# CoderLSF/fast-llama

Measured on AMD Instinct MI355X. Metric: decode tokens/s LLaMA2-7B int8, higher is better.
Workload: dtype int8; 1 GPU; LLaMA2-7B int8 .flm-layout synthetic weights (portable splitmix64 checkpoint, norm weights 1.0), single-stream greedy decode, prompt 9 tokens, positions 14..928, fp32 KV cache, max_seq 1024; parallelism=single-gpu

## Files before the change

### fast-llama_amd/csrc/flm_attn.h

```cpp
#pragma once
#include "flm_math.h"
#include "flm_gemv.h"
#pragma clang fp contract(off)

namespace flm {

struct AttnArgs {
    const float* q;
    const float* kcache;
    const float* vcache;
    float* out;
    const int* pos_ptr;
    const int* halt;
    int hs, max_seq;
    int kv_rows;
    unsigned long long* trace;
    void* oq; float* os; int oqt;
    int G; float* sc_global; unsigned* flag_sc; unsigned epoch; int* err;
    float* out_peer[7]; int n_peer;
    unsigned long long* gout; unsigned long long* gout_peer[7];
    const unsigned long long* qg; const unsigned long long* kg; const unsigned long long* vg;
};

#ifndef FLM_V_LATE_NS
// ... 718 lines not shown
        const int k = tid & 7, p = (tid >> 3) & 63, jh = (tid >> 9) * 4;
        for (int s = 0; s < nt; ++s) {
            float* cur = (s & 1) ? tile1 : tile0;
            park(cur, ring);
            __syncthreads();
            request(rK, s + 1, ring);
            const float* kp = cur + p * rs + k;
            const float* q0 = qs + (jh + 0) * hs + k; const float* q1 = qs + (jh + 1) * hs + k;
            const float* q2 = qs + (jh + 2) * hs + k; const float* q3 = qs + (jh + 3) * hs + k;
            float l0 = 0.f, l1 = 0.f, l2 = 0.f, l3 = 0.f;
#pragma unroll 8
            for (int i = 0; i < hs; i += 8) {
                const float kv = kp[i];
                l0 = __fmaf_rn(kv, q0[i], l0); l1 = __fmaf_rn(kv, q1[i], l1); l2 = __fmaf_rn(kv, q2[i], l2); l3 = __fmaf_rn(kv, q3[i], l3);
            }
            const int t = s * kAttnTile + p;
            auto fold = [&](float l, int j) {
                const int li = __float_as_int(l);
                float tot = __fadd_rn(0.f, l);
                tot = __fadd_rn(tot, __int_as_float(__builtin_amdgcn_update_dpp(0, li, 0x101 , 0xF, 0xF, true)));
                tot = __fadd_rn(tot, __int_as_float(__builtin_amdgcn_update_dpp(0, li, 0x102, 0xF, 0xF, true)));
                tot = __fadd_rn(tot, __int_as_float(__builtin_amdgcn_update_dpp(0, li, 0x103, 0xF, 0xF, true)));
                tot = __fadd_rn(tot, __int_as_float(__builtin_amdgcn_update_dpp(0, li, 0x104, 0xF, 0xF, true)));
                tot = __fadd_rn(tot, __int_as_float(__builtin_amdgcn_update_dpp(0, li, 0x105, 0xF, 0xF, true)));
                tot = __fadd_rn(tot, __int_as_float(__builtin_amdgcn_update_dpp(0, li, 0x106, 0xF, 0xF, true)));
                tot = __fadd_rn(tot, __int_as_float(__builtin_amdgcn_update_dpp(0, li, 0x107, 0xF, 0xF, true)));
                if (k == 0 && j < nq && t < pos0 + i0 + j + 1) sc[j * scs + t] = __fmul_rn(tot, scale);
            };
            fold(l0, jh + 0); fold(l1, jh + 1); fold(l2, jh + 2); fold(l3, jh + 3);
        }
    }
    }
    request(rV, 0, ring);
    __syncthreads();
    if (wave < nq) {
        const int T = pos0 + i0 + wave + 1;
        float* row = sc + wave * scs;
        float m = -INFINITY;
        for (int t = lane; t < T; t += 64) m = fmaxf(m, row[t]);
        m = wave_max(m);
        for (int t = lane; t < T; t += 64) row[t] = expf_ref(__fsub_rn(row[t], m));
        float sum = 0.f;
        if (lane == 0) {
            int t = 0;
            if (T >= 16) {
                const float4* r4 = reinterpret_cast<const float4*>(row);
                float4 a0 = r4[0], a1 = r4[1], a2 = r4[2], a3 = r4[3];
#define FLM_ADD4(q) sum = __fadd_rn(sum, q.x); sum = __fadd_rn(sum, q.y); sum = __fadd_rn(sum, q.z); sum = __fadd_rn(sum, q.w);
                for (; t + 32 <= T; t += 16) {
                    const float4 b0 = r4[t / 4 + 4], b1 = r4[t / 4 + 5], b2 = r4[t / 4 + 6], b3 = r4[t / 4 + 7];
                    FLM_ADD4(a0) FLM_ADD4(a1) FLM_ADD4(a2) FLM_ADD4(a3)
                    a0 = b0; a1 = b1; a2 = b2; a3 = b3;
                }
                FLM_ADD4(a0) FLM_ADD4(a1) FLM_ADD4(a2) FLM_ADD4(a3)
#undef FLM_ADD4
                t += 16;
            }
            for (; t < T; ++t) sum = __fadd_rn(sum, row[t]);
        }
        sum = __uint_as_float(__builtin_amdgcn_readfirstlane(__float_as_uint(sum)));
        for (int t = lane; t < T; t += 64) { const float w = __fdiv_rn(row[t], sum); row[t] = (t > 0 && fabsf(w) <= 1e-15f) ? 0.f : w; }
    }
    const int tpq = hs <= 64 ? 64 : 128;
    const int j = tid / tpq, d = tid - j * tpq;
    const bool mine = j < nq && d < hs;
    const int Tj = pos0 + i0 + j + 1;
    float o = 0.f;
    for (int i = 0; i < nt; ++i) {
        float* cur = (i & 1) ? tile1 : tile0;
        park(cur, ring);
        __syncthreads();
        request(rV, i + 1, ring);
        if (mine) {
            const float* vp = cur + d;
            const float* wp = sc + j * scs + i * kAttnTile;
            int np = Tj - i * kAttnTile; np = np < 0 ? 0 : (np > kAttnTile ? kAttnTile : np);
            int p = 0;
            if (i == 0 && np > 0) { o = __fmul_rn(vp[0], wp[0]); p = 1; }
            const float wl = lane < np ? wp[lane] : 1.f;
            if (__all(wl != 0.f)) {
                for (; p < np && (p & 7); ++p) o = __fmaf_rn(vp[p * rs], wp[p], o);
                for (; p + 8 <= np; p += 8) {
                    const float* vq = vp + p * rs;
                    const float4 wa = *reinterpret_cast<const float4*>(wp + p), wb = *reinterpret_cast<const float4*>(wp + p + 4);
                    const float a0 = vq[0], a1 = vq[rs], a2 = vq[2 * rs], a3 = vq[3 * rs], a4 = vq[4 * rs], a5 = vq[5 * rs], a6 = vq[6 * rs], a7 = vq[7 * rs];
                    o = __fmaf_rn(a0, wa.x, o); o = __fmaf_rn(a1, wa.y, o); o = __fmaf_rn(a2, wa.z, o); o = __fmaf_rn(a3, wa.w, o);
                    o = __fmaf_rn(a4, wb.x, o); o = __fmaf_rn(a5, wb.y, o); o = __fmaf_rn(a6, wb.z, o); o = __fmaf_rn(a7, wb.w, o);
                }
                for (; p < np; ++p) o = __fmaf_rn(vp[p * rs], wp[p], o);
            } else {
                for (; p < np; ++p) { const float w = wp[p]; o = w == 0.f ? o : __fmaf_rn(vp[p * rs], w, o); }
            }
        }
    }
    if (mine) a.out[(size_t)(i0 + j) * row_stride + (size_t)h * hs + d] = o;
}
template <bool PRE>
__global__ void __launch_bounds__(kAttnBlock) k_attn_prefill_mq(const AttnArgs a, int pos0, int row_stride, int B) {
    extern __shared__ __attribute__((aligned(16))) char lds[];
    const int i0 = blockIdx.y * kMqQueries, nq = B - i0 < kMqQueries ? B - i0 : kMqQueries;
    if (a.hs <= 64) attn_prefill_mq<1, PRE>(a, blockIdx.x, lds, pos0, i0, nq, row_stride, B); else attn_prefill_mq<2, PRE>(a, blockIdx.x, lds, pos0, i0, nq, row_stride, B);
}

constexpr int kQkQ = 16;
template <int NS>
__global__ void __launch_bounds__(256) k_qk_mfma(const AttnArgs a, int pos0, int row_stride, int B) {
    typedef float v4f __attribute__((ext_vector_type(4)));
    const int hs = a.hs, tid = threadIdx.x, lane = tid & 63, wave = tid >> 6;
    const int h = blockIdx.x, q0 = blockIdx.y * kQkQ;
    const int Tmax = pos0 + (q0 + kQkQ < B ? q0 + kQkQ : B);
    const int nt = (Tmax + 15) >> 4;
    const float* K = a.kcache + (size_t)h * (a.kv_rows ? a.kv_rows : a.max_seq) * hs;
    const __amdgpu_buffer_rsrc_t rK = __builtin_amdgcn_make_buffer_rsrc(const_cast<float*>(K), 0, Tmax * hs * 4, 0x00020000);
    const float scale = (float)(1.0 / (double)__builtin_sqrtf((float)hs));
    const int li = lane & 15, c = lane >> 4;
    v4f qa[NS][2];
    {
        const float* qp = a.q + (size_t)(q0 + li) * row_stride + (size_t)h * hs;
#pragma unroll
        for (int sp = 0; sp < NS; ++sp) {
            const int e = 8 * (4 * sp + c);
            if (q0 + li < B) { qa[sp][0] = *reinterpret_cast<const v4f*>(qp + e); qa[sp][1] = *reinterpret_cast<const v4f*>(qp + e + 4); }
            else { qa[sp][0] = v4f{0.f, 0.f, 0.f, 0.f}; qa[sp][1] = v4f{0.f, 0.f, 0.f, 0.f}; }
        }
    }
    v4f kb[2][NS][2];
    auto request = [&](int tile, v4f (&r)[NS][2]) {
        const unsigned base = (unsigned)(((tile * 16 + li) * hs + 8 * c) * 4);
#pragma unroll
        for (int sp = 0; sp < NS; ++sp) {
            r[sp][0] = __builtin_bit_cast(v4f, __builtin_amdgcn_raw_buffer_load_b128(rK, (int)(base + sp * 128), 0, 0));
            r[sp][1] = __builtin_bit_cast(v4f, __builtin_amdgcn_raw_buffer_load_b128(rK, (int)(base + sp * 128 + 16), 0, 0));
        }
    };
    auto tile_scores = [&](int tile, const v4f (&kr)[NS][2]) {
        v4f acc[8];
#pragma unroll
        for (int r = 0; r < 8; ++r) acc[r] = v4f{0.f, 0.f, 0.f, 0.f};
#pragma unroll
        for (int sp = 0; sp < NS; ++sp) {
#pragma unroll
            for (int r = 0; r < 8; ++r)
                acc[r] = __builtin_amdgcn_mfma_f32_16x16x4f32(qa[sp][r >> 2][r & 3], kr[sp][r >> 2][r & 3], acc[r], 0, 0, 0);
        }
        const int t = tile * 16 + li;
#pragma unroll
        for (int reg = 0; reg < 4; ++reg) {
            const int q = q0 + 4 * c + reg;
            float tot = __fadd_rn(0.f, acc[0][reg]);
#pragma unroll
            for (int r = 1; r < 8; ++r) tot = __fadd_rn(tot, acc[r][reg]);
            if (q < B && t < pos0 + q + 1) a.sc_global[((size_t)h * B + q) * a.max_seq + t] = __fmul_rn(tot, scale);
        }
    };
    request(wave, kb[0]);
    for (int tile = wave; tile < nt; tile += 8) {
        request(tile + 4, kb[1]);
        tile_scores(tile, kb[0]);
        request(tile + 8, kb[0]);
        if (tile + 4 < nt) tile_scores(tile + 4, kb[1]);
    }
}
constexpr int kPvQ = 16, kPvRing = 4;
__host__ __device__ inline int pv_row_stride(int tmax) { return ((((tmax + 15) & ~15) + 63) & ~63) + 4; }
__host__ inline size_t pv_mfma_lds_bytes(int tmax, int qw = kPvQ) { return ((size_t)qw * pv_row_stride(tmax) + 16) * 4; }
__host__ inline int pv_mfma_queries(int tmax, size_t lds_max) { int qw = kPvQ; while (qw > 1 && pv_mfma_lds_bytes(tmax, qw) > lds_max) qw >>= 1; return qw; }
inline __global__ void __launch_bounds__(256) k_attn_pv_mfma(const AttnArgs a, int pos0, int row_stride, int B, int qw) {
    typedef float v4f __attribute__((ext_vector_type(4)));
    typedef float v2f __attribute__((ext_vector_type(2)));
    extern __shared__ __attribute__((aligned(16))) char lds[];
    const int hs = a.hs, tid = threadIdx.x, lane = tid & 63, wave = tid >> 6;
    const int h = blockIdx.x, q0 = blockIdx.y * qw, nq = B - q0 < qw ? B - q0 : qw;
    const int S = pv_row_stride(pos0 + B);
    float* E = reinterpret_cast<float*>(lds);
    float* sums = E + qw * S;
    const int Tmax = pos0 + q0 + nq, Tp = (Tmax + 15) & ~15, nblk = Tp >> 4;
    {
        const int q = 4 * wave + (lane >> 4), l16 = lane & 15;
        const int Tq = q < nq ? pos0 + q0 + q + 1 : 0;
        const float* src = a.sc_global + ((size_t)h * B + (q0 + (q < nq ? q : 0))) * a.max_seq;
        float* row = E + q * S;
        const int Tr = q < qw ? Tp : 0;
        float m = -INFINITY;
        for (int t = l16 * 4; t < Tr; t += 64) {
            float4 v = make_float4(-INFINITY, -INFINITY, -INFINITY, -INFINITY);
            if (t + 3 < Tq) v = *reinterpret_cast<const float4*>(src + t);
            else { if (t < Tq) v.x = src[t]; if (t + 1 < Tq) v.y = src[t + 1]; if (t + 2 < Tq) v.z = src[t + 2]; }
            *reinterpret_cast<float4*>(row + t) = v;
            m = fmaxf(m, fmaxf(fmaxf(v.x, v.y), fmaxf(v.z, v.w)));
        }
        m = row16_max(m);
        for (int t = l16 * 4; t < Tr; t += 64) {
            float4 v = *reinterpret_cast<const float4*>(row + t);
            v.x = t < Tq ? expf_ref(__fsub_rn(v.x, m)) : 0.f; v.y = t + 1 < Tq ? expf_ref(__fsub_rn(v.y, m)) : 0.f;
            v.z = t + 2 < Tq ? expf_ref(__fsub_rn(v.z, m)) : 0.f; v.w = t + 3 < Tq ? expf_ref(__fsub_rn(v.w, m)) : 0.f;
            *reinterpret_cast<float4*>(row + t) = v;
        }
    }
    __syncthreads();
    if (tid < qw) {
        const float4* r4 = reinterpret_cast<const float4*>(E + tid * S);
        float sum = 0.f;
#pragma unroll 4
        for (int i = 0; i < Tp / 4; ++i) { const float4 v = r4[i]; sum = __fadd_rn(sum, v.x); sum = __fadd_rn(sum, v.y); sum = __fadd_rn(sum, v.z); sum = __fadd_rn(sum, v.w); }
        sums[tid] = sum;
    }
    __syncthreads();
    for (int bidx = tid; bidx < qw * nblk; bidx += 256) {
        const int q = bidx / nblk, bi = bidx - q * nblk;
        float* blk = E + q * S + bi * 16;
        const float sum = sums[q];
        float w[16];
#pragma unroll
        for (int i = 0; i < 4; ++i) { const float4 v = *reinterpret_cast<const float4*>(blk + 4 * i); w[4 * i] = v.x; w[4 * i + 1] = v.y; w[4 * i + 2] = v.z; w[4 * i + 3] = v.w; }
#pragma unroll
        for (int i = 0; i < 16; ++i) {
            const float x = q < nq ? __fdiv_rn(w[i], sum) : 0.f;
            w[i] = (bi * 16 + i > 0 && fabsf(x) <= 1e-15f) ? 0.f : x;
        }
#pragma unroll
        for (int c = 0; c < 4; ++c) *reinterpret_cast<float4*>(blk + 4 * c) = make_float4(w[c], w[4 + c], w[8 + c], w[12 + c]);
    }
    __syncthreads();
    const int li = lane & 15, c = lane >> 4, d0 = 32 * wave + 2 * li;
    if (32 * wave >= hs) return;
    const float* V = a.vcache + (size_t)h * (a.kv_rows ? a.kv_rows : a.max_seq) * hs;
    const __amdgpu_buffer_rsrc_t rV = __builtin_amdgcn_make_buffer_rsrc(const_cast<float*>(V), 0, Tmax * hs * 4, 0x00020000);
    unsigned voff = d0 < hs ? (unsigned)((c * hs + d0) * 4) : 0x80000000u;
    const unsigned vstep = (unsigned)(4 * hs * 4);
    v2f ring[kPvRing][4];
    auto request = [&](v2f (&r)[4]) {
#pragma unroll
        for (int sp = 0; sp < 4; ++sp) { r[sp] = __builtin_bit_cast(v2f, __builtin_amdgcn_raw_buffer_load_b64(rV, (int)voff, 0, 0)); voff += vstep; }
    };
#pragma unroll
    for (int r = 0; r < kPvRing; ++r) request(ring[r]);
    v4f acc0 = {-0.f, -0.f, -0.f, -0.f}, acc1 = {-0.f, -0.f, -0.f, -0.f};
    const float* ap = E + (li < qw ? li : 0) * S + 4 * c;
    for (int b0 = 0; b0 < nblk; b0 += kPvRing) {
#pragma unroll
        for (int r = 0; r < kPvRing; ++r) {
            if (b0 + r < nblk) {
                float4 av = *reinterpret_cast<const float4*>(ap + (b0 + r) * 16);
                if (li >= qw) av = make_float4(0.f, 0.f, 0.f, 0.f);
                acc0 = __builtin_amdgcn_mfma_f32_16x16x4f32(av.x, ring[r][0].x, acc0, 0, 0, 0); acc1 = __builtin_amdgcn_mfma_f32_16x16x4f32(av.x, ring[r][0].y, acc1, 0, 0, 0);
                acc0 = __builtin_amdgcn_mfma_f32_16x16x4f32(av.y, ring[r][1].x, acc0, 0, 0, 0); acc1 = __builtin_amdgcn_mfma_f32_16x16x4f32(av.y, ring[r][1].y, acc1, 0, 0, 0);
                acc0 = __builtin_amdgcn_mfma_f32_16x16x4f32(av.z, ring[r][2].x, acc0, 0, 0, 0); acc1 = __builtin_amdgcn_mfma_f32_16x16x4f32(av.z, ring[r][2].y, acc1, 0, 0, 0);
                acc0 = __builtin_amdgcn_mfma_f32_16x16x4f32(av.w, ring[r][3].x, acc0, 0, 0, 0); acc1 = __builtin_amdgcn_mfma_f32_16x16x4f32(av.w, ring[r][3].y, acc1, 0, 0, 0);
            }
            request(ring[r]);
        }
    }
    if (d0 < hs) {
#pragma unroll
        for (int reg = 0; reg < 4; ++reg) {
            const int q = 4 * c + reg;
            if (q < nq) {
                const size_t idx = (size_t)(q0 + q) * row_stride + (size_t)h * hs + d0;
                if (a.n_peer == 0) *reinterpret_cast<float2*>(a.out + idx) = make_float2(acc0[reg], acc1[reg]);
                else {
                    st_agent(a.out + idx, acc0[reg]); st_agent(a.out + idx + 1, acc1[reg]);
                    for (int i = 0; i < a.n_peer; ++i) {
                        __hip_atomic_store(a.out_peer[i] + idx, acc0[reg], __ATOMIC_RELAXED, __HIP_MEMORY_SCOPE_SYSTEM);
                        __hip_atomic_store(a.out_peer[i] + idx + 1, acc1[reg], __ATOMIC_RELAXED, __HIP_MEMORY_SCOPE_SYSTEM);
                    }
                }
            }
        }
    }
}

template <bool SPLIT>
__global__ void __launch_bounds__(kAttnBlock) k_attn_decode(const AttnArgs a) {
    extern __shared__ __attribute__((aligned(16))) char lds[];
    if (halted(a.halt)) return;
    const int G = SPLIT ? a.G : 1;
    attn_head_any<false, SPLIT>(a, blockIdx.x / G, lds, *a.pos_ptr + 1, a.q, a.out, blockIdx.x % G, G);
}

struct AoTp { unsigned* peer_flags[8]; const unsigned* base; unsigned add; int world, line0, n_lines; };
template <int QT, int XR, bool PREQ, bool SPLIT = false>
__global__ void __launch_bounds__(kGemvBlock, 4) k_attn_o(const AttnArgs aa, const GemvArgs a, const int n_heads, unsigned* flag, const unsigned target_, int* err, const AoTp tp) {
    extern __shared__ __attribute__((aligned(16))) char lds[];
    if (halted(a.halt)) return;
    auto stamp = [&](int k) { if (kAblate && a.trace && threadIdx.x == 0) a.trace[blockIdx.x * 8 + k] = __builtin_amdgcn_s_memtime(); };
    stamp(0);
    const unsigned target = tp.world ? *tp.base + tp.add : target_;
    if ((int)blockIdx.x < n_heads) {
        const int G = SPLIT ? aa.G : 1;
        attn_head_any<false, SPLIT>(aa, blockIdx.x / G, lds, *aa.pos_ptr + 1, aa.q, aa.out, blockIdx.x % G, G);
        stamp(1);
        wait_stores_done();
        __syncthreads();
        if (threadIdx.x == 0) {
            if (tp.world) {
                __atomic_thread_fence(__ATOMIC_RELEASE);
                for (int r = 0; r < tp.world; ++r) __hip_atomic_store(tp.peer_flags[r] + (tp.line0 + blockIdx.x) * kFlagStride, target, __ATOMIC_RELAXED, __HIP_MEMORY_SCOPE_SYSTEM);
            } else __hip_atomic_store(flag + blockIdx.x * kFlagStride, target, __ATOMIC_RELAXED, __HIP_MEMORY_SCOPE_AGENT);
        }
        stamp(4);
        return;
    }
    GemvCtx<QT, EPI_RESIDUAL> g;
    g.init(a, blockIdx.x - n_heads, gridDim.x - n_heads, lds);
    g.issue(kAblate ? a.ablate : 0);
    stamp(1);
    const int n_poll = tp.world ? tp.n_lines : n_heads;
    if ((int)(threadIdx.x & ~63u) < n_poll) {
        const bool mine = (int)threadIdx.x < n_poll;
        if (tp.world) {
            poll_wave<__HIP_MEMORY_SCOPE_SYSTEM, true, 4>(flag + threadIdx.x * kFlagStride, mine, target, err);
            __atomic_thread_fence(__ATOMIC_ACQUIRE);
        } else poll_wave(flag + threadIdx.x * kFlagStride, mine, target, err);
    }
    __syncthreads();
    stamp(2);
    float4 xv[XR > 0 ? XR : 1], nv[XR > 0 ? XR : 1];
    if constexpr (PREQ) {
        gemv_prologue<QT, PRO_NONE, 0, true>(a, lds, xv, nv, [](int) {});
    } else {
        gemv_preload<QT, PRO_QUANT, XR, true>(a, xv, nv);
        gemv_prologue<QT, PRO_QUANT, XR>(a, lds, xv, nv, [](int) {});
    }
    stamp(3);
    g.run(a, lds, [](int) {});
    stamp(4);
}

template <int QT, int XR, bool PREQ, bool SPLIT = false, bool TP = false>
__global__ void __launch_bounds__(kGemvBlock, 4) k_qkv_attn_o(const GemvArgs aq, const AttnArgs aa, const GemvArgs a, const int gridq, const int n_heads, const int grido,
                                                              unsigned* flagq, unsigned* flag, const unsigned target, int* err, const AoTp tp) {
    extern __shared__ __attribute__((aligned(16))) char lds[];
    if constexpr (!TP) { if (halted(a.halt)) return; }
    auto nostamp = [](int) {};
    const unsigned htarget = TP ? *tp.base + tp.add : target;
    if constexpr (TP) { if (aq.xf.world) xchg_fold(aq.xf); }
    if ((int)blockIdx.x < gridq) {
        float4 xq[1], nq[1];
        gemv_preload<QT, PRO_RMSNORM_QUANT, 1, TP>(aq, xq, nq);
        GemvCtx<QT, EPI_ROPE_KV> gq;
        gq.init(aq, blockIdx.x, gridq, lds);
        gemv_prologue<QT, PRO_RMSNORM_QUANT, 1, TP>(aq, lds, xq, nq, [&](int part) { gq.issue(kAblate ? aq.ablate : 0, part); });
        gq.run(aq, lds, nostamp);
        wait_stores_done();
        __syncthreads();
        if (threadIdx.x == 0) __hip_atomic_store(flagq + blockIdx.x * kFlagStride, target, __ATOMIC_RELAXED, __HIP_MEMORY_SCOPE_AGENT);
    }
    if ((int)blockIdx.x < n_heads) {
        const int G = SPLIT ? aa.G : 1, h = blockIdx.x / G;
        if (threadIdx.x < 256) {
            const bool need = qkv_line_needed(threadIdx.x, (unsigned)gridq, (unsigned)aq.rows_per_pass, (unsigned)aa.hs, (unsigned)h, (unsigned)aq.dim, (unsigned)aq.kv_dim);
            poll_wave(flagq + threadIdx.x * kFlagStride, need, target, err);
        }
        __syncthreads();
        attn_head_any<true, SPLIT>(aa, h, lds, *aa.pos_ptr + 1, aa.q, aa.out, blockIdx.x % G, G);
        wait_stores_done();
        __syncthreads();
        if (threadIdx.x == 0) {
            if constexpr (TP) {
                __atomic_thread_fence(__ATOMIC_RELEASE);
                for (int r = 0; r < tp.world; ++r) __hip_atomic_store(tp.peer_flags[r] + (tp.line0 + blockIdx.x) * kFlagStride, htarget, __ATOMIC_RELAXED, __HIP_MEMORY_SCOPE_SYSTEM);
            } else __hip_atomic_store(flag + blockIdx.x * kFlagStride, target, __ATOMIC_RELAXED, __HIP_MEMORY_SCOPE_AGENT);
        }
        return;
    }
    if ((int)blockIdx.x >= n_heads + grido) return;
    GemvCtx<QT, EPI_RESIDUAL> g;
    g.init(a, blockIdx.x - n_heads, grido, lds);
    g.issue(kAblate ? a.ablate : 0);
    const int n_poll = TP ? tp.n_lines : n_heads;
    if ((int)(threadIdx.x & ~63u) < n_poll) {
        const bool mine = (int)threadIdx.x < n_poll;
        if constexpr (TP) {
            poll_wave<__HIP_MEMORY_SCOPE_SYSTEM, true, 4>(flag + threadIdx.x * kFlagStride, mine, htarget, err);
            __atomic_thread_fence(__ATOMIC_ACQUIRE);
        } else poll_wave(flag + threadIdx.x * kFlagStride, mine, htarget, err);
    }
    __syncthreads();
    float4 xv[XR > 0 ? XR : 1], nv[XR > 0 ? XR : 1];
    if constexpr (PREQ) {
        gemv_prologue<QT, PRO_NONE, 0, true>(a, lds, xv, nv, [](int) {});
    } else {
        gemv_preload<QT, PRO_QUANT, XR, true>(a, xv, nv);
        gemv_prologue<QT, PRO_QUANT, XR>(a, lds, xv, nv, [](int) {});
    }
    g.run(a, lds, [](int) {});
}

struct FfnTp { unsigned* peer_flags[8]; const unsigned* base; unsigned add; int world, rank; unsigned long long* counter; };
template <int QT, int XR2, bool TP = false>
__global__ void __launch_bounds__(kGemvBlock, 4) k_ffn(const GemvArgs a13, const GemvArgs a2, const int grid13, const int grid2, unsigned* flag, const unsigned target_, int* err, const FfnTp tp) {
    extern __shared__ __attribute__((aligned(16))) char lds[];
    if constexpr (!TP) { if (halted(a2.halt)) return; }
    auto nostamp = [](int) {};
    const unsigned target = TP ? *tp.base + tp.add : target_;
    if constexpr (TP) { if (a13.xf.world) xchg_fold(a13.xf); }
    if ((int)blockIdx.x < grid13) {
        float4 xv[1], nv[1];
        gemv_preload<QT, PRO_RMSNORM_QUANT, 1, TP>(a13, xv, nv);
        GemvCtx<QT, EPI_SWIGLU> g;
        g.init(a13, blockIdx.x, grid13, lds);
        gemv_prologue<QT, PRO_RMSNORM_QUANT, 1, TP>(a13, lds, xv, nv, [&](int part) { g.issue(kAblate ? a13.ablate : 0, part); });
        g.run(a13, lds, nostamp);
    }
    wait_stores_done();
    __syncthreads();
    if (threadIdx.x == 0) {
        if constexpr (TP) {
            const unsigned long long old = __hip_atomic_fetch_add(tp.counter, 1ull, __ATOMIC_ACQ_REL, __HIP_MEMORY_SCOPE_AGENT);
            if ((old + 1) % gridDim.x == 0) {
                __atomic_thread_fence(__ATOMIC_RELEASE);
                for (int r = 0; r < tp.world; ++r) __hip_atomic_store(tp.peer_flags[r] + tp.rank * kFlagStride, target, __ATOMIC_RELAXED, __HIP_MEMORY_SCOPE_SYSTEM);
            }
        } else __hip_atomic_store(flag + blockIdx.x * kFlagStride, target, __ATOMIC_RELAXED, __HIP_MEMORY_SCOPE_AGENT);
    }
    if ((int)blockIdx.x >= grid2) return;
    GemvCtx<QT, EPI_RESIDUAL> g2;
    g2.init(a2, blockIdx.x, grid2, lds);
    g2.issue(kAblate ? a2.ablate : 0, 1);
    if (threadIdx.x < 256) {
        const bool mine = (int)threadIdx.x < (TP ? tp.world : (int)gridDim.x);
        if constexpr (TP) {
            poll_wave<__HIP_MEMORY_SCOPE_SYSTEM, true, 4>(flag + threadIdx.x * kFlagStride, mine, target, err);
            __atomic_thread_fence(__ATOMIC_ACQUIRE);
        } else poll_wave(flag + threadIdx.x * kFlagStride, mine, target, err);
    }
    __syncthreads();
    float4 xv2[XR2 > 0 ? XR2 : 1], nv2[XR2 > 0 ? XR2 : 1];
    gemv_preload<QT, PRO_QUANT, XR2, true>(a2, xv2, nv2);
    gemv_prologue<QT, PRO_QUANT, XR2, true>(a2, lds, xv2, nv2, [&](int) { g2.issue(kAblate ? a2.ablate : 0, 2); });
    g2.run(a2, lds, nostamp);
}

}
```

### fast-llama_amd/csrc/flm_gemv.h

```cpp
#pragma once
#include "flm_math.h"
#include "flm_wait.h"
#pragma clang fp contract(off)

namespace flm {

struct GemvArgs {
    const void*  W;   const float* sW;
    int n;
    int items;
    int rows_per_pass;
    int cb_shift;
    int ctr_off;
    int nbuf;
    const float* x;
    const float* norm_w;
    const void*  xq; const float* xs;
    float* out;
    float* kcache; float* vcache;
    const float* rope_cos; const float* rope_sin;
    const int* pos_ptr;
    const int* halt;
    int dim; int kv_dim; int max_seq; int hs;
    float* out_peer[7]; int n_peer;
    unsigned long long* gout; unsigned long long* gout_peer[7];
    unsigned long long* gk; unsigned long long* gv;
    struct XchgFold {
        unsigned* local_flags; unsigned* peer_flags[8];
        const unsigned* base; unsigned add;
        int rank, world, slot; int* err;
    } xf;
    void* dbg_xq; float* dbg_xs; float* dbg_xn;
    unsigned long long* trace;
    int ablate;
};

__device__ __forceinline__ void st_result(const GemvArgs& a, unsigned row, float v) {
    st_agent(a.out + row, v);
    for (int i = 0; i < a.n_peer; ++i) __hip_atomic_store(a.out_peer[i] + row, v, __ATOMIC_RELAXED, __HIP_MEMORY_SCOPE_SYSTEM);
}

#ifndef FLM_ABLATE
#define FLM_ABLATE 0
#endif
constexpr bool kAblate = FLM_ABLATE != 0;
constexpr int kStepBlk = 4;

__host__ __device__ inline int chain_bshift(int n) { int s = 2; while ((64 << s) < n / 4) ++s; return s; }
__host__ __device__ inline int chain_strip_floats(int n) { return 64 * ((1 << chain_bshift(n)) + 4); }
struct GemvLds {
    int off_xs, off_red, off_ctr, off_scr;
    int gstride;
    int buf_bytes;
    int total;
};
__host__ __device__ inline GemvLds gemv_lds_layout(int n, int esz, bool norm, int Rm, int RB, bool two, int nbuf = 2) {
    GemvLds L;
    const int sn = n / kGroup, ng = two ? 2 * sn : sn;
    L.off_xs = n * esz;
    L.off_red = L.off_xs + ((sn * 4 + 15) & ~15);
    L.off_ctr = L.off_red + 64;
    L.off_scr = L.off_ctr + 16;
    int g16 = (ng * 8 + 15) / 16; if ((g16 & 1) == 0) ++g16;
    L.gstride = g16 * 16;
    L.buf_bytes = (Rm + RB) * L.gstride;
    int scratch = nbuf * L.buf_bytes + 64;
    const int chain = 4 * chain_strip_floats(n) * 4 + 64;
    if (norm && chain > scratch) scratch = chain;
    L.total = L.off_scr + scratch;
    return L;
}
__device__ __forceinline__ float sq_chain(const float* p, int n4) {
    float l = 0.f;
    int k = 0;
#define FLM_SQ4(v) l = __fmaf_rn(v.x, v.x, l); l = __fmaf_rn(v.y, v.y, l); l = __fmaf_rn(v.z, v.z, l); l = __fmaf_rn(v.w, v.w, l);
#define FLM_RD4(a, b, c, d, base) a = *reinterpret_cast<const float4*>(pp + (base)); b = *reinterpret_cast<const float4*>(pp + (base) + 4); c = *reinterpret_cast<const float4*>(pp + (base) + 8); d = *reinterpret_cast<const float4*>(pp + (base) + 12);
    if (n4 >= 32) {
        const float* pp = p;
        float4 a0, a1, a2, a3, b0, b1, b2, b3;
        FLM_RD4(a0, a1, a2, a3, 0)
#pragma unroll 2
        for (; k + 32 <= n4; k += 32, pp += 32) {
            FLM_RD4(b0, b1, b2, b3, 16)
            __builtin_amdgcn_s_waitcnt(0xC47F);
            __builtin_amdgcn_sched_barrier(0);
            FLM_SQ4(a0) FLM_SQ4(a1) FLM_SQ4(a2) FLM_SQ4(a3)
            __builtin_amdgcn_sched_barrier(0);
            FLM_RD4(a0, a1, a2, a3, 32)
            __builtin_amdgcn_s_waitcnt(0xC47F);
            __builtin_amdgcn_sched_barrier(0);
            FLM_SQ4(b0) FLM_SQ4(b1) FLM_SQ4(b2) FLM_SQ4(b3)
            __builtin_amdgcn_sched_barrier(0);
        }
        if (k + 4 <= n4) { FLM_SQ4(a0) k += 4; } if (k + 4 <= n4) { FLM_SQ4(a1) k += 4; } if (k + 4 <= n4) { FLM_SQ4(a2) k += 4; } if (k + 4 <= n4) { FLM_SQ4(a3) k += 4; }
    }
#undef FLM_RD4
#undef FLM_SQ4
    for (; k < n4; ++k) l = __fmaf_rn(p[k], p[k], l);
    return l;
}

__device__ __forceinline__ double wave_scan_incl_f64(double v) {
#define FLM_SCAN64(ctrl, rmask, bc) { const int lo_ = __builtin_amdgcn_update_dpp(0, __double2loint(v), ctrl, rmask, 0xF, bc), hi_ = __builtin_amdgcn_update_dpp(0, __double2hiint(v), ctrl, rmask, 0xF, bc); v = __dadd_rn(v, __hiloint2double(hi_, lo_)); }
    FLM_SCAN64(0x111 , 0xF, true) FLM_SCAN64(0x112 , 0xF, true)
    FLM_SCAN64(0x114 , 0xF, true) FLM_SCAN64(0x118 , 0xF, true)
    FLM_SCAN64(0x142 , 0xA, false) FLM_SCAN64(0x143 , 0xC, false)
#undef FLM_SCAN64
    return v;
}
__device__ __forceinline__ float wave_scan_incl(float v) {
#define FLM_SCAN_STEP(ctrl, rmask, bc) v = __fadd_rn(v, __int_as_float(__builtin_amdgcn_update_dpp(0, __float_as_int(v), ctrl, rmask, 0xF, bc)));
    FLM_SCAN_STEP(0x111 , 0xF, true) FLM_SCAN_STEP(0x112 , 0xF, true)
    FLM_SCAN_STEP(0x114 , 0xF, true) FLM_SCAN_STEP(0x118 , 0xF, true)
    FLM_SCAN_STEP(0x142 , 0xA, false) FLM_SCAN_STEP(0x143 , 0xC, false)
#undef FLM_SCAN_STEP
    return v;
}
__device__ __forceinline__ double readlane_f64(double v, int l) {
    return __hiloint2double(__builtin_amdgcn_readlane(__double2hiint(v), l), __builtin_amdgcn_readlane(__double2loint(v), l));
}
constexpr int kChainHead = 4;
#ifdef FLM_TRACE_PRO_RT
#define FLM_CHAIN_STAMP(k) if (tr && lane == 0) tr[k] = __builtin_amdgcn_s_memtime();
#else
#define FLM_CHAIN_STAMP(k)
#endif
template <int OP> __device__ __forceinline__ float chain_step(float l, float x) { if constexpr (OP == 0) return __fmaf_rn(x, x, l); else return __fadd_rn(l, x); }
template <int BVR, int OP = 0, int PAD = 4, bool STARTS = false>
__device__ __forceinline__ float chain_spec_t(const float* p, const int bshift, int* rounds_out, unsigned long long* tr = nullptr, const int Brt = 0, float* lane_start = nullptr) {
    const int lane = threadIdx.x & 63, B = BVR ? 4 * BVR : (Brt ? Brt : (1 << bshift)), BV = B >> 2, LS = B + PAD;
    const float4* pl = reinterpret_cast<const float4*>(p + lane * LS);
    float4 xr[BVR ? BVR : 1];
    if constexpr (BVR > 0) {
#pragma unroll
        for (int q = 0; q < BVR; ++q) xr[q] = pl[q];
    }
    auto elem = [&](int q) -> float4 { if constexpr (BVR > 0) return xr[q]; else return pl[q]; };
    FLM_CHAIN_STAMP(0)
#define FLM_SQ4(l, v) l = chain_step<OP>(l, v.x); l = chain_step<OP>(l, v.y); l = chain_step<OP>(l, v.z); l = chain_step<OP>(l, v.w);
    float s = 0.f; unsigned orb = 0u;
#pragma unroll
    for (int q = 0; q < BV; ++q) { const float4 v = elem(q); FLM_SQ4(s, v) orb |= __float_as_uint(v.x) | __float_as_uint(v.y); orb |= __float_as_uint(v.z) | __float_as_uint(v.w); }
    const bool allzero = (orb & 0x7fffffffu) == 0u;
    const float P = __int_as_float(__builtin_amdgcn_update_dpp(0, __float_as_int(wave_scan_incl(s)), 0x138 , 0xF, 0xF, true));
    FLM_CHAIN_STAMP(1)
    float hv;
    [[maybe_unused]] float ls = 0.f;
    {
        float l = 0.f;
#pragma unroll
        for (int L = 0; L < kChainHead; ++L) {
            if constexpr (STARTS) { if (lane == L) ls = l; }
#pragma unroll
            for (int q = 0; q < BV; ++q) { const float4 v = elem(q); FLM_SQ4(l, v) }
            if (L + 1 < kChainHead) l = __int_as_float(__builtin_amdgcn_update_dpp(0, __float_as_int(l), 0x138 , 0xF, 0xF, true));
        }
        hv = __int_as_float(__builtin_amdgcn_readlane(__float_as_int(l), kChainHead - 1));
    }
    FLM_CHAIN_STAMP(2)
    const unsigned eb = __float_as_uint(P) & 0x7f800000u;
    bool valid = lane >= kChainHead && eb >= (27u << 23) && eb <= (250u << 23);
    const unsigned ebv = valid ? eb : 0x3f800000u;
    const float A = __uint_as_float(ebv), u1 = __uint_as_float(ebv - (23u << 23)), top = __fadd_rn(A, A);
    float ca = A, cb = __fadd_rn(A, u1);
#pragma unroll
    for (int q = 0; q < BV; ++q) { const float4 v = elem(q); FLM_SQ4(ca, v) FLM_SQ4(cb, v) }
    float T = __fsub_rn(ca, A);
    const bool tie = __fsub_rn(cb, ca) != u1;
    if (!(T < INFINITY)) valid = false;
    if (!valid) T = 0.f;
    FLM_CHAIN_STAMP(3)
    const unsigned long long live = __ballot(valid && !allzero);
    bool plain = false;
    if (live) {
        const unsigned e0 = (unsigned)__builtin_amdgcn_readlane((int)eb, __ffsll((long long)live) - 1), e1 = (unsigned)__builtin_amdgcn_readlane((int)eb, 63 - __clzll((long long)live));
        plain = e1 < e0 || ((e1 - e0) >> 23) > 26;
    }
    if (plain) {
        float l = 0.f;
        for (int L = 0; L < 64; ++L) { if constexpr (STARTS) { if (lane == L) ls = l; } const float4* r = reinterpret_cast<const float4*>(p + L * LS); for (int q = 0; q < BV; ++q) { const float4 v = r[q]; FLM_SQ4(l, v) } }
        if (rounds_out) *rounds_out = -1;
        if constexpr (STARTS) *lane_start = ls;
        return l;
    }
    const double Td = (double)T, Si = wave_scan_incl_f64(Td), S = __dsub_rn(Si, Td);
    FLM_CHAIN_STAMP(4)
    int rounds = 0;
    const unsigned long long zero_m = __ballot(allzero), good_m = __ballot(valid && !tie);
    unsigned long long done_m = (1ull << kChainHead) - 1ull;
    double bv = (double)hv, Sb = readlane_f64(S, kChainHead);
    float res;
    [[maybe_unused]] int base = kChainHead;
    for (;;) {
        ++rounds;
        if (rounds <= 9) { FLM_CHAIN_STAMP(4 + rounds) }
        const float st = (float)__dadd_rn(bv, __dsub_rn(S, Sb));
        const unsigned long long e_m = __ballot((__float_as_uint(st) & 0x7f800000u) == eb), t_m = __ballot(__fadd_rn(st, T) < top);
        const unsigned long long bad = ~(zero_m | (good_m & e_m & t_m) | done_m);
        if (bad == 0) {
            if constexpr (STARTS) { if (lane >= base) ls = st; }
            res = __uint_as_float((unsigned)__builtin_amdgcn_readlane((int)__float_as_uint((float)__dadd_rn(bv, __dsub_rn(Si, Sb))), 63)); break;
        }
        const int f = __ffsll((long long)bad) - 1;
        if constexpr (STARTS) { if (lane >= base && lane <= f) ls = st; base = f + 1; }
        float l = st;
#pragma unroll
        for (int q = 0; q < BV; ++q) { const float4 v = elem(q); FLM_SQ4(l, v) }
        res = __uint_as_float((unsigned)__builtin_amdgcn_readlane((int)__float_as_uint(l), f));
        if (f == 63) break;
        done_m = (2ull << f) - 1ull; bv = (double)res; Sb = readlane_f64(S, f + 1);
    }
#undef FLM_SQ4
    FLM_CHAIN_STAMP(14)
    if (tr && lane == 0) tr[15] = (unsigned long long)rounds;
    if (rounds_out) *rounds_out = rounds;
    if constexpr (STARTS) *lane_start = ls;
    return res;
}
template <int BVR>
__device__ __forceinline__ float sq_chain_spec_t(const float* p, const int bshift, int* rounds_out, unsigned long long* tr = nullptr) { return chain_spec_t<BVR, 0, 4>(p, bshift, rounds_out, tr); }
__device__ __forceinline__ float sq_chain_spec(const float* p, const int bshift, int* rounds_out = nullptr, unsigned long long* tr = nullptr) {
    return sq_chain_spec_t<0>(p, bshift, rounds_out, tr);
}

template <int QT, int PRO, int XR, bool COH = false>
__device__ __forceinline__ void gemv_preload(const GemvArgs& a, float4 (&xv)[XR > 0 ? XR : 1], float4 (&wv)[XR > 0 ? XR : 1], const float* xsrc = nullptr) {
    if constexpr (PRO == PRO_QUANT || PRO == PRO_RMSNORM_QUANT) {
        typedef float v4f __attribute__((ext_vector_type(4)));
        const __amdgpu_buffer_rsrc_t rx = __builtin_amdgcn_make_buffer_rsrc(const_cast<float*>(xsrc ? xsrc : a.x), 0, a.n * 4, 0x00020000);
        const __amdgpu_buffer_rsrc_t rn = __builtin_amdgcn_make_buffer_rsrc(const_cast<float*>(PRO == PRO_RMSNORM_QUANT ? a.norm_w : a.x), 0, a.n * 4, 0x00020000);
#pragma unroll
        for (int i = 0; i < XR; ++i) {
            const int off = (threadIdx.x * 4 + i * kGemvBlock * 4) * 4;
            const v4f v = __builtin_bit_cast(v4f, __builtin_amdgcn_raw_buffer_load_b128(rx, off, 0, COH ? kAuxCoherent : 0));
            xv[i] = make_float4(v.x, v.y, v.z, v.w);
            if constexpr (PRO == PRO_RMSNORM_QUANT) {
                const v4f u = __builtin_bit_cast(v4f, __builtin_amdgcn_raw_buffer_load_b128(rn, off, 0, 0));
                wv[i] = make_float4(u.x, u.y, u.z, u.w);
            }
        }
    }
}

typedef unsigned v4u_g __attribute__((ext_vector_type(4)));
typedef unsigned long long granule_t;
__device__ __forceinline__ void st_granule(granule_t* g, unsigned tag, float v) {
    __hip_atomic_store(g, ((granule_t)tag << 32) | (granule_t)__float_as_uint(v), __ATOMIC_RELAXED, __HIP_MEMORY_SCOPE_AGENT);
}
__device__ __forceinline__ float ld_granule_value(const granule_t* g) { return __uint_as_float((unsigned)__hip_atomic_load(g, __ATOMIC_RELAXED, __HIP_MEMORY_SCOPE_AGENT)); }
__device__ __forceinline__ void st_result_granule(const GemvArgs& a, unsigned row, unsigned tag, float v) {
    st_granule(a.gout + row, tag, v);
    const granule_t g = ((granule_t)tag << 32) | (granule_t)__float_as_uint(v);
    for (int i = 0; i < a.n_peer; ++i) __hip_atomic_store(a.gout_peer[i] + row, g, __ATOMIC_RELAXED, __HIP_MEMORY_SCOPE_SYSTEM);
}

#ifndef FLM_QUANT_SHARED_RCP
#define FLM_QUANT_SHARED_RCP 1
#endif
template <int QT>
__device__ __forceinline__ void quant_round4(char* xq, float* xs, int e, bool act, const float4& v) {
    using T = QTraits<QT>;
    const float mx = row16_max(fmaxf(fmaxf(fabsf(v.x), fabsf(v.y)), fmaxf(fabsf(v.z), fabsf(v.w))));
    const float sc = __fdiv_rn(mx, T::kF);
    int qq[4];
#if FLM_QUANT_SHARED_RCP
    quant_elems4(v, sc, qq);
#else
    qq[0] = quant_elem(v.x, sc); qq[1] = quant_elem(v.y, sc); qq[2] = quant_elem(v.z, sc); qq[3] = quant_elem(v.w, sc);
#endif
    if (act) {
        const int q0 = qq[0], q1 = qq[1], q2 = qq[2], q3 = qq[3];
        if constexpr (QT == QT_INT8) {
            const uint32_t pk = (uint32_t)(q0 & 0xff) | ((uint32_t)(q1 & 0xff) << 8) | ((uint32_t)(q2 & 0xff) << 16) | ((uint32_t)(q3 & 0xff) << 24);
            *reinterpret_cast<uint32_t*>(xq + e) = pk;
        } else {
            uint2 pk;
            pk.x = (uint32_t)(q0 & 0xffff) | ((uint32_t)(q1 & 0xffff) << 16);
            pk.y = (uint32_t)(q2 & 0xffff) | ((uint32_t)(q3 & 0xffff) << 16);
            *reinterpret_cast<uint2*>(xq + (size_t)e * 2) = pk;
        }
        if ((threadIdx.x & 15) == 0) xs[e / kGroup] = sc;
    }
}

#ifdef FLM_TRACE_PRO_RT
#define FLM_PRO_STAMP(k) if (kAblate && a.trace && (threadIdx.x == 0 || threadIdx.x == 960)) a.trace[blockIdx.x * 16 + (threadIdx.x ? 8 : 0) + (k)] = __builtin_amdgcn_s_memrealtime();
#elif defined(FLM_TRACE_PRO)
#define FLM_PRO_STAMP(k) if (kAblate && a.trace && threadIdx.x == 0) a.trace[blockIdx.x * 8 + (k)] = __builtin_amdgcn_s_memtime();
#else
#define FLM_PRO_STAMP(k)
#endif
template <int QT, int PRO, int XR, bool COH = false, bool LATE = false, class AfterStage>
__device__ __forceinline__ void gemv_prologue(const GemvArgs& a, char* lds, float4 (&xv)[XR > 0 ? XR : 1], float4 (&wv)[XR > 0 ? XR : 1], AfterStage&& after_stage) {
    using T = QTraits<QT>;
    const int n = a.n;
    const int tid = threadIdx.x;
    const GemvLds L = gemv_lds_layout(n, T::kEsz, PRO == PRO_RMSNORM_QUANT, a.rows_per_pass, 64 >> a.cb_shift, false);
    char*  xq = lds;
    float* xs = reinterpret_cast<float*>(lds + L.off_xs);
    float* red = reinterpret_cast<float*>(lds + L.off_red);
    float* scratch = reinterpret_cast<float*>(lds + L.off_scr);

    if constexpr (PRO == PRO_NONE) {
        const int nb16 = n * T::kEsz / 16;
        if constexpr (COH) {
            const __amdgpu_buffer_rsrc_t rq = __builtin_amdgcn_make_buffer_rsrc(const_cast<void*>(a.xq), 0, n * T::kEsz, 0x00020000);
            for (int c = tid; c < nb16; c += kGemvBlock)
                reinterpret_cast<v4i*>(xq)[c] = __builtin_bit_cast(v4i, __builtin_amdgcn_raw_buffer_load_b128(rq, c * 16, 0, kAuxCoherent));
            for (int g = tid; g < n / kGroup; g += kGemvBlock) xs[g] = ld_agent(a.xs + g);
        } else {
            for (int c = tid; c < nb16; c += kGemvBlock)
                reinterpret_cast<int4*>(xq)[c] = reinterpret_cast<const int4*>(a.xq)[c];
            for (int g = tid; g < n / kGroup; g += kGemvBlock) xs[g] = a.xs[g];
        }
        __syncthreads();
        return;
    } else {
        const int rounds = (n + kGemvBlock * 4 - 1) / (kGemvBlock * 4);
        const float4 z4 = make_float4(0.f, 0.f, 0.f, 0.f);
        float r = 1.0f;
#ifdef FLM_TRACE_PRO_RT
        FLM_PRO_STAMP(0)
#endif
        auto ldx = [&](int e) -> float4 {
            if constexpr (COH) {
                typedef float v4f __attribute__((ext_vector_type(4)));
                const __amdgpu_buffer_rsrc_t rx = __builtin_amdgcn_make_buffer_rsrc(const_cast<float*>(a.x), 0, n * 4, 0x00020000);
                const v4f t = __builtin_bit_cast(v4f, __builtin_amdgcn_raw_buffer_load_b128(rx, e * 4, 0, kAuxCoherent));
                return make_float4(t.x, t.y, t.z, t.w);
            } else return *reinterpret_cast<const float4*>(a.x + e);
        };
        if constexpr (PRO == PRO_QUANT) {
            if constexpr (XR > 0) { asm volatile("" :: "v"(xv[XR - 1].w)); }
            FLM_PRO_STAMP(3)
            if constexpr (!LATE) after_stage(0);
            FLM_PRO_STAMP(4)
        }
        if constexpr (PRO == PRO_RMSNORM_QUANT) {
            const int bs = chain_bshift(n), B = 1 << bs, LS = B + 4, CS = 64 * LS, slots = 64 << bs;
            auto stage = [&](int i, const float4& v) {
                const int k = tid + i * kGemvBlock;
                if (k < slots) { const int o = (k >> bs) * LS + (k & (B - 1)); scratch[o] = v.x; scratch[CS + o] = v.y; scratch[2 * CS + o] = v.z; scratch[3 * CS + o] = v.w; }
            };
            const int srounds = (slots + kGemvBlock - 1) / kGemvBlock;
#pragma unroll
            for (int i = 0; i < XR; ++i) { if (i < srounds) stage(i, xv[i]); }
            for (int i = XR; i < srounds; ++i) {
                const int e = tid * 4 + i * kGemvBlock * 4;
                stage(i, e < n ? ldx(e) : z4);
            }
#ifdef FLM_TRACE_PRO_RT
            FLM_PRO_STAMP(1)
#endif
            __syncthreads();
            FLM_PRO_STAMP(3)
            if constexpr (!LATE) {
                if (tid >= 4 * kWave) __builtin_amdgcn_s_sleep(2);
                after_stage(0);
#ifdef FLM_TRACE_PRO2
                FLM_PRO_STAMP(1)
#endif
                if (tid < 4 * kWave && !(kAblate && (a.ablate & 2))) {
                    const float l = sq_chain_spec(scratch + (tid >> 6) * CS, bs);
                    if ((tid & 63) == 0) red[8 + (tid >> 6)] = l;
                }
            } else {
                const int wv = __builtin_amdgcn_readfirstlane(tid >> 6);
                if (wv >= 4) after_stage(0);
                else if (!(kAblate && (a.ablate & 2))) {
#ifdef FLM_TRACE_PRO_RT
                    unsigned long long* tr = (kAblate && a.trace && tid < 64) ? a.trace + 2 * 4096 + blockIdx.x * 16 : nullptr;
#else
                    unsigned long long* tr = nullptr;
#endif
                    const float* cp = scratch + wv * CS;
                    float l;
                    if (bs == 4) l = sq_chain_spec_t<4>(cp, bs, nullptr, tr);
                    else if (bs == 3) l = sq_chain_spec_t<2>(cp, bs, nullptr, tr);
                    else if (bs == 2) l = sq_chain_spec_t<1>(cp, bs, nullptr, tr);
                    else l = sq_chain_spec_t<0>(cp, bs, nullptr, tr);
                    if ((tid & 63) == 0) red[8 + wv] = l;
                }
            }
#ifdef FLM_TRACE_PRO_RT
            FLM_PRO_STAMP(2)
#endif
            FLM_PRO_STAMP(4)
            __syncthreads();
            const float ss = __fadd_rn(__fadd_rn(__fadd_rn(__fadd_rn(0.f, red[8]), red[9]), red[10]), red[11]);
            r = rms_scale(ss, n);
            FLM_PRO_STAMP(5)
        }
        auto round = [&](int i, float4 v, float4 w) {
            const int e = tid * 4 + i * kGemvBlock * 4;
            const bool act = e < n;
            if constexpr (PRO == PRO_RMSNORM_QUANT) {
                v.x = __fmul_rn(__fmul_rn(v.x, w.x), r); v.y = __fmul_rn(__fmul_rn(v.y, w.y), r);
                v.z = __fmul_rn(__fmul_rn(v.z, w.z), r); v.w = __fmul_rn(__fmul_rn(v.w, w.w), r);
            }
            if (act && a.dbg_xn && blockIdx.x == 0) *reinterpret_cast<float4*>(a.dbg_xn + e) = v;
            quant_round4<QT>(xq, xs, e, act, v);
        };
#pragma unroll
        for (int i = 0; i < XR; ++i) { if (i < rounds) round(i, xv[i], wv[i]); }
        for (int i = XR; i < rounds; ++i) {
            const int e = tid * 4 + i * kGemvBlock * 4;
            float4 v = z4, w = z4;
            if (e < n) {
                v = ldx(e);
                if constexpr (PRO == PRO_RMSNORM_QUANT) w = *reinterpret_cast<const float4*>(a.norm_w + e);
            }
            round(i, v, w);
        }
        if constexpr (PRO == PRO_QUANT) {
            FLM_PRO_STAMP(5)
        }
#ifdef FLM_TRACE_PRO_RT
        FLM_PRO_STAMP(6)
#endif
        __syncthreads();
#ifdef FLM_TRACE_PRO_RT
        FLM_PRO_STAMP(7)
#endif
        if (a.dbg_xq && blockIdx.x == 0) {
            const int nb4 = n * T::kEsz / 4;
            for (int c = tid; c < nb4; c += kGemvBlock) reinterpret_cast<uint32_t*>(a.dbg_xq)[c] = reinterpret_cast<uint32_t*>(xq)[c];
            for (int g = tid; g < n / kGroup; g += kGemvBlock) a.dbg_xs[g] = xs[g];
        }
    }
}

typedef unsigned int u32;
typedef unsigned v4u __attribute__((ext_vector_type(4)));

template <int QT, int EPI, bool STASH = false>
struct GemvCtx {
    using T = QTraits<QT>;
    static constexpr u32 LPGS = (T::kEPC == 16) ? 2 : 3;
    static constexpr u32 LPG = 1u << LPGS;
    static constexpr bool TWO = EPI == EPI_SWIGLU;
    static constexpr int H = kStepBlk;
    static constexpr u32 ES = TWO ? 16 : 8;
    static constexpr u32 kOOB = 0x80000000u;

    struct Set { v4i w[H]; float sw; u32 itl, st, xo, nlive; };

    u32 n, lane, wave, rowbytes, sn, cbs, RB, nbc, NBCV, TRm, Rm, RBP, SP, NS, np_wg, npass, gstride, buf_bytes, off_xs, off_scr, ctr_off;
    u32 inv_SP, inv_NBCV;
    u32 lane_woff, lane_xoff, lane_goff;
    u32 lane_j, lane_s2off, lane_sx2off, lane_poff;
    bool leader;
    u32 dW, dS, dT, dummy_st, wg, nwg, nbuf;
    u32 st_base, st_n;
    static constexpr u32 kSlotBytes = H * 1024 + 256;
    __amdgpu_buffer_rsrc_t rW, rS;
    Set setA, setB;
    bool stored;
    const float* resid_src;
    const granule_t* gsrc; bool gron; unsigned gtag;
    u32 nw;

    static __device__ __forceinline__ u32 inv_of(u32 d) { return d > 1 ? 0xFFFFFFFFu / d + 1u : 0u; }
    static __device__ __forceinline__ u32 udiv(u32 x, u32 d, u32 inv) { return d > 1 ? __umulhi(x, inv) : x; }

    __device__ __forceinline__ void init(const GemvArgs& a, u32 wg_, u32 nwg_, char* lds, u32 ctr_slot = 0, u32 st_base_ = 0, u32 st_n_ = 0, bool write_ctr = true) {
        n = a.n; wg = wg_; nwg = nwg_; st_base = st_base_; st_n = st_n_;
        lane = threadIdx.x & 63;
        wave = __builtin_amdgcn_readfirstlane(threadIdx.x >> 6);
        rowbytes = n * T::kEsz; sn = n / kGroup;
        const u32 nchunks = rowbytes / 16;
        cbs = a.cb_shift; RB = 64u >> cbs;
        const u32 CB = 1u << cbs;
        nbc = nchunks >> cbs;
        NBCV = TWO ? 2 * nbc : nbc;
        TRm = (u32)a.items * (EPI == EPI_ROPE_KV ? 2u : 1u);
        Rm = a.rows_per_pass;
        RBP = Rm / RB;
        npass = (TRm + Rm - 1) / Rm;
        np_wg = wg < npass ? (npass - wg + nwg - 1) / nwg : 0;
        SP = ((RBP + H - 1) / H) * NBCV;
        NS = np_wg * SP;
        inv_SP = inv_of(SP); inv_NBCV = inv_of(NBCV);
        nbuf = a.nbuf > 0 ? a.nbuf : 2;
        const GemvLds L = gemv_lds_layout(n, T::kEsz, true, Rm, RB, TWO, nbuf);
        gstride = L.gstride; buf_bytes = L.buf_bytes; off_xs = L.off_xs; off_scr = L.off_scr; ctr_off = a.ctr_off ? (u32)a.ctr_off : (u32)L.off_ctr + 4 * (ctr_slot & 1);
        dW = RB * rowbytes; dS = RB * sn * 4; dT = RB * gstride;
        dummy_st = Rm * gstride;
        const u32 rb = lane >> cbs, cb = lane & (CB - 1);
        lane_woff = rb * rowbytes + cb * 16;
        lane_xoff = cb * 16;
        lane_goff = rb * gstride + (cb >> LPGS) * ES;
        leader = (cb & (LPG - 1)) == 0;
        constexpr u32 GPB = 64u / LPG;
        lane_j = lane / GPB;
        const u32 ll = (lane % GPB) * LPG, rb2 = ll >> cbs, cb2 = ll & (CB - 1);
        lane_s2off = lane_j * dS + (rb2 * sn + (cb2 >> LPGS)) * 4;
        lane_sx2off = (cb2 >> LPGS) * 4;
        lane_poff = lane_j * dT + rb2 * gstride + (cb2 >> LPGS) * ES + ES / 2;
        constexpr int kRsrcFlags = 0x00020000;
        const u32 NM = TWO ? 2u : 1u;
        rW = __builtin_amdgcn_make_buffer_rsrc(const_cast<void*>(a.W), 0, (int)(NM * TRm * rowbytes), kRsrcFlags);
        rS = __builtin_amdgcn_make_buffer_rsrc(const_cast<float*>(a.sW), 0, (int)(NM * TRm * sn * 4), kRsrcFlags);
        stored = false; primedA = primedB = false; resid_src = nullptr; gsrc = nullptr; gron = false; gtag = 0; nw = kWavesPerBlock;
        if (write_ctr && threadIdx.x == 0) *reinterpret_cast<u32*>(lds + ctr_off) = 2 * kWavesPerBlock;
    }

    __device__ __forceinline__ void reset_ctr(char* lds) const { if (threadIdx.x == 0) *reinterpret_cast<u32*>(lds + ctr_off) = 2 * kWavesPerBlock; }

    __device__ __forceinline__ void decode(u32 s, Set& S, u32& wo, u32& so) const {
        if (s >= NS) { S.itl = np_wg; S.st = 0; S.xo = 0; S.nlive = 0; wo = kOOB; so = kOOB; return; }
        const u32 itl = udiv(s, SP, inv_SP), rem = s - itl * SP;
        const u32 q = udiv(rem, NBCV, inv_NBCV), cv = rem - q * NBCV;
        const bool second = TWO && cv >= nbc;
        const u32 cc = second ? cv - nbc : cv, g0 = (cc << cbs) >> LPGS;
        const u32 rb0 = q * H, row0 = (second ? TRm : 0u) + (wg + itl * nwg) * Rm + rb0 * RB;
        wo = row0 * rowbytes + ((cc << cbs) * 16);
        so = (row0 * sn + g0) * 4;
        S.itl = itl; S.xo = cc; S.nlive = RBP - rb0 < (u32)H ? RBP - rb0 : (u32)H;
        S.st = rb0 * RB * gstride + g0 * ES + (second ? 4u : 0u);
    }
    __device__ __forceinline__ void load_step(Set& S, u32 s, int ablate, const char* lds = nullptr) const {
        u32 wo, so;
        decode(s, S, wo, so);
        if constexpr (STASH) {
            const u32 si = s - 2 * kWavesPerBlock;
            if (si < st_n) {
                const char* p = lds + st_base + si * kSlotBytes;
#pragma unroll
                for (int j = 0; j < H; ++j) S.w[j] = *reinterpret_cast<const v4i*>(p + j * 1024 + lane * 16);
                S.sw = *reinterpret_cast<const float*>(p + H * 1024 + lane * 4);
                return;
            }
        }
        u32 nl = S.nlive;
        if (kAblate && (ablate & 4)) { nl = 0; so = kOOB; }
#pragma unroll
        for (int j = 0; j < H; ++j) {
            const u32 woj = (u32)j < nl ? wo + j * dW : kOOB;
            S.w[j] = __builtin_bit_cast(v4i, __builtin_amdgcn_raw_buffer_load_b128(rW, (int)(lane_woff + woj), 0, 2));
        }
        const u32 svo = lane_j < nl ? lane_s2off + so : kOOB;
        S.sw = __uint_as_float(__builtin_amdgcn_raw_buffer_load_b32(rS, (int)svo, 0, 2));
    }
    bool primedA, primedB;
    __device__ __forceinline__ void issue(int ablate, int part = 0) {
        if (part != 2) { load_step(setA, wave < nw ? wave : NS, ablate); primedA = true; }
        if (part != 1) { load_step(setB, wave < nw ? wave + nw : NS, ablate); primedB = true; }
    }

    __device__ __forceinline__ void stash_issue(const char* lds, const u32 w0 = 0) const {
        const u32 lds0 = (u32)(uintptr_t)(__attribute__((address_space(3))) const char*)lds;
        if (wave < w0) return;
        for (u32 i = wave - w0; i < st_n; i += kWavesPerBlock - w0) {
            Set S; u32 wo, so;
            decode(2 * kWavesPerBlock + i, S, wo, so);
            const u32 dst = __builtin_amdgcn_readfirstlane(lds0 + st_base + i * kSlotBytes);
#pragma unroll
            for (int j = 0; j < H; ++j) {
                const u32 woj = (u32)j < S.nlive ? lane_woff + wo + j * dW : kOOB;
                asm volatile("s_mov_b32 m0, %2\n\ts_nop 0\n\tbuffer_load_dwordx4 %0, %1, 0 offen nt lds" :: "v"(woj), "s"(rW), "s"(dst + j * 1024) : "memory", "m0");
            }
            const u32 svo = lane_j < S.nlive ? lane_s2off + so : kOOB;
            asm volatile("s_mov_b32 m0, %2\n\ts_nop 0\n\tbuffer_load_dword %0, %1, 0 offen nt lds" :: "v"(svo), "s"(rS), "s"(dst + H * 1024) : "memory", "m0");
        }
    }
    __device__ __forceinline__ void issue_missing(int ablate) {
        if (!primedA) { load_step(setA, wave < nw ? wave : NS, ablate); primedA = true; }
        if (!primedB) { load_step(setB, wave < nw ? wave + nw : NS, ablate); primedB = true; }
    }

    v4i xa; float sx2; u32 cur_xo;
    __device__ __forceinline__ void reduce_step(const Set& S, char* lds, char* strips, int ablate) {
        const char* xq = lds; const char* xs = lds + off_xs;
        if (S.xo != cur_xo) {
            cur_xo = S.xo;
            xa = *reinterpret_cast<const v4i*>(xq + ((cur_xo << cbs) * 16) + lane_xoff);
            sx2 = *reinterpret_cast<const float*>(xs + (((cur_xo << cbs) >> LPGS) * 4) + lane_sx2off);
        }
        float d[H];
#pragma unroll
        for (int j = 0; j < H; ++j) {
            int t = (kAblate && (ablate & 8)) ? 0 : quad_sum(dot_chunk<QT>(S.w[j], xa));
            if constexpr (LPG == 8) t += __builtin_amdgcn_update_dpp(0, t, 0x104 , 0xF, 0xF, true);
            d[j] = (float)t;
        }
        if (leader) {
#pragma unroll
            for (int j = 0; j < H; ++j) {
                const u32 stj = (u32)j < S.nlive ? S.st + j * dT : dummy_st;
                *reinterpret_cast<float*>(strips + stj + lane_goff) = d[j];
            }
        }
        if (lane_j < S.nlive) *reinterpret_cast<float*>(strips + S.st + lane_poff) = __fmul_rn(S.sw, sx2);
    }

    __device__ __forceinline__ void finish_pass(const GemvArgs& a, u32 pass, u32 it, const char* strips, int pos) {
        const bool chain_wave = wave == (it & (kWavesPerBlock - 1));
        float resid = 0.f, rc = 0.f, rs = 0.f;
        const u32 row = pass * Rm + lane;
        const bool rv = chain_wave && lane < Rm && row < TRm;
        if constexpr (EPI == EPI_RESIDUAL) { if (rv) resid = gsrc ? ld_granule_value(gsrc + row) : ld_agent((resid_src ? resid_src : a.out) + row); }
        if constexpr (EPI == EPI_ROPE_KV) {
            if (rv && row < (u32)(a.dim + a.kv_dim)) {
                const u32 r2 = (row < (u32)a.dim ? row : row - a.dim) & ~1u;
                const u32 dd = r2 % (u32)a.hs;
                rc = a.rope_cos[(size_t)pos * (a.hs / 2) + dd / 2];
                rs = a.rope_sin[(size_t)pos * (a.hs / 2) + dd / 2];
            }
        }
        __syncthreads();
        if (!chain_wave) return;
#ifdef FLM_TRACE_BAR
        if (kAblate && a.trace && threadIdx.x == 0 && it == 0) a.trace[blockIdx.x * 8 + 3] = __builtin_amdgcn_s_memtime();
#endif
        stored = true;
        float acc = 0.f, acc2 = 0.f;
        if (lane < Rm && !(kAblate && (a.ablate & 1))) {
            const char* sp = strips + lane * gstride;
            u32 g = 0;
#define FLM_RD4(r0, r1, r2, r3, ptr) r0 = *reinterpret_cast<const float4*>(ptr); r1 = *reinterpret_cast<const float4*>((ptr) + 16); r2 = *reinterpret_cast<const float4*>((ptr) + 32); r3 = *reinterpret_cast<const float4*>((ptr) + 48);
            if constexpr (TWO) {
                typedef float f2 __attribute__((ext_vector_type(2)));
                f2 ac = {0.f, 0.f};
#define FLM_CH(q) ac = __builtin_elementwise_fma(f2{q.z, q.w}, f2{q.x, q.y}, ac);
                if (sn >= 8) {
                    float4 a0, a1, a2, a3, b0, b1, b2, b3;
                    FLM_RD4(a0, a1, a2, a3, sp)
                    for (; g + 8 <= sn; g += 8) {
                        const char* pn = sp + (g + 4) * 16;
                        FLM_RD4(b0, b1, b2, b3, pn)
                        __builtin_amdgcn_s_waitcnt(0xC47F);
                        __builtin_amdgcn_sched_barrier(0);
                        FLM_CH(a0) FLM_CH(a1) FLM_CH(a2) FLM_CH(a3)
                        __builtin_amdgcn_sched_barrier(0);
                        FLM_RD4(a0, a1, a2, a3, pn + 64)
                        __builtin_amdgcn_s_waitcnt(0xC47F);
                        __builtin_amdgcn_sched_barrier(0);
                        FLM_CH(b0) FLM_CH(b1) FLM_CH(b2) FLM_CH(b3)
                        __builtin_amdgcn_sched_barrier(0);
                    }
                    if (g < sn) { FLM_CH(a0) ++g; } if (g < sn) { FLM_CH(a1) ++g; } if (g < sn) { FLM_CH(a2) ++g; } if (g < sn) { FLM_CH(a3) ++g; }
                }
                for (; g < sn; ++g) { const float4 e = *reinterpret_cast<const float4*>(sp + g * 16); FLM_CH(e) }
#undef FLM_CH
                acc = ac.x; acc2 = ac.y;
            } else {
#define FLM_CH(q) acc = __fmaf_rn(q.y, q.x, acc); acc = __fmaf_rn(q.w, q.z, acc);
                if (sn >= 16) {
                    float4 a0, a1, a2, a3, b0, b1, b2, b3;
                    FLM_RD4(a0, a1, a2, a3, sp)
                    for (; g + 16 <= sn; g += 16) {
                        const char* pn = sp + (g + 8) * 8;
                        FLM_RD4(b0, b1, b2, b3, pn)
                        __builtin_amdgcn_s_waitcnt(0xC47F);
                        __builtin_amdgcn_sched_barrier(0);
                        FLM_CH(a0) FLM_CH(a1) FLM_CH(a2) FLM_CH(a3)
                        __builtin_amdgcn_sched_barrier(0);
                        FLM_RD4(a0, a1, a2, a3, pn + 64)
                        __builtin_amdgcn_s_waitcnt(0xC47F);
                        __builtin_amdgcn_sched_barrier(0);
                        FLM_CH(b0) FLM_CH(b1) FLM_CH(b2) FLM_CH(b3)
                        __builtin_amdgcn_sched_barrier(0);
                    }
                    if (g + 2 <= sn) { FLM_CH(a0) g += 2; } if (g + 2 <= sn) { FLM_CH(a1) g += 2; } if (g + 2 <= sn) { FLM_CH(a2) g += 2; } if (g + 2 <= sn) { FLM_CH(a3) g += 2; }
                }
#undef FLM_CH
                for (; g < sn; ++g) { const float2 e = *reinterpret_cast<const float2*>(sp + g * 8); acc = __fmaf_rn(e.y, e.x, acc); }
            }
#undef FLM_RD4
        }
        if constexpr (EPI == EPI_STORE || EPI == EPI_RESIDUAL) {
            if (rv) {
                if constexpr (EPI == EPI_STORE) st_result(a, row, acc);
                else if (gron) st_result_granule(a, row, gtag, __fadd_rn(resid, acc));
                else st_result(a, row, __fadd_rn(resid, acc));
            }
        } else if constexpr (EPI == EPI_SWIGLU) {
            if (rv) { const float hv = swiglu_elem(acc, acc2); if (gron) st_result_granule(a, row, gtag, hv); else st_result(a, row, hv); }
        } else {
            const float other = __shfl_xor(acc, 1, kWave);
            if (rv && (lane & 1) == 0) {
                const float x0 = acc, x1 = other;
                const u32 hs = a.hs;
                if (row < (u32)(a.dim + a.kv_dim)) {
                    const u32 rr = row < (u32)a.dim ? row : row - a.dim;
                    const u32 h = rr / hs, d = rr - h * hs;
                    float o0, o1;
                    rope_pair(x0, x1, rc, rs, o0, o1);
                    if (row < (u32)a.dim) {
                        if (gron) { st_granule(a.gout + row, gtag, o0); st_granule(a.gout + row + 1, gtag, o1); }
                        else { st_agent(a.out + row, o0); st_agent(a.out + row + 1, o1); }
                    }
                    else {
                        float* kp = a.kcache + ((size_t)h * a.max_seq + pos) * hs + d; st_agent(kp, o0); st_agent(kp + 1, o1);
                        if (gron) { st_granule(a.gk + rr, gtag, o0); st_granule(a.gk + rr + 1, gtag, o1); }
                    }
                } else {
                    const u32 rr = row - a.dim - a.kv_dim;
                    const u32 h = rr / hs, d = rr - h * hs;
                    float* vp = a.vcache + ((size_t)h * a.max_seq + pos) * hs + d; st_agent(vp, x0); st_agent(vp + 1, x1);
                    if (gron) { st_granule(a.gv + rr, gtag, x0); st_granule(a.gv + rr + 1, gtag, x1); }
                }
            }
        }
    }

    template <class Stamp>
    __device__ __forceinline__ void run(const GemvArgs& a, char* lds, Stamp&& stamp) {
        int pos = 0;
        if constexpr (EPI == EPI_ROPE_KV) pos = *a.pos_ptr;
        xa = v4i{0, 0, 0, 0}; sx2 = 0.f; cur_xo = 0xffffffffu;
        u32* ctr = reinterpret_cast<u32*>(lds + ctr_off);
        u32 it = 0;
        bool tr3 = false;
        auto finish_upto = [&](u32 limit) {
            while (it < limit) {
                char* strips = lds + off_scr + (nbuf > 1 ? (it & 1) * buf_bytes : 0u);
#ifdef FLM_TRACE_WAVES
                if (kAblate && a.trace && it == 0 && lane == 0 && wave % 3 == 0) a.trace[blockIdx.x * 8 + 1 + wave / 3] = __builtin_amdgcn_s_memtime();
#elif !defined(FLM_TRACE_PRO)
                if (it == 0) stamp(4);
#endif
                finish_pass(a, wg + it * nwg, it, strips, pos);
#ifndef FLM_TRACE_PRO
                if (it == 0) stamp(5);
#endif
                ++it;
            }
        };
        auto do_set = [&](Set& S) -> bool {
            finish_upto(S.itl);
            if (S.itl >= np_wg) return false;
            reduce_step(S, lds, lds + off_scr + (nbuf > 1 ? (S.itl & 1) * buf_bytes : 0u), a.ablate);
            u32 s = 0;
            if (lane == 0) s = atomicAdd(ctr, 1u);
            load_step(S, __builtin_amdgcn_readfirstlane(s), a.ablate, lds);
#if !defined(FLM_TRACE_PRO) && !defined(FLM_TRACE_BAR)
            if (!tr3) { tr3 = true; stamp(3); }
#endif
            return true;
        };
        if (!primedA) load_step(setA, wave, a.ablate);
        if (!primedB) load_step(setB, wave + kWavesPerBlock, a.ablate);
        while (do_set(setA) && do_set(setB)) {}
    }

    struct AoSrc {
        const unsigned* flags;
        u32 rows, grid;
        unsigned target; int* err;
    };
    struct AoBlock { v4i d; float s; };
    template <int PRO>
    __device__ __forceinline__ AoBlock ao_fetch(const GemvArgs& a, u32 cc) const {
        AoBlock b; b.s = 0.f;
        const u32 CB = 1u << cbs;
        if constexpr (PRO == PRO_NONE) {
            const __amdgpu_buffer_rsrc_t rq = __builtin_amdgcn_make_buffer_rsrc(const_cast<void*>(a.xq), 0, (int)rowbytes, 0x00020000);
            const __amdgpu_buffer_rsrc_t rs = __builtin_amdgcn_make_buffer_rsrc(const_cast<float*>(a.xs), 0, (int)(sn * 4), 0x00020000);
            b.d = __builtin_bit_cast(v4i, __builtin_amdgcn_raw_buffer_load_b128(rq, (int)(lane < CB ? ((cc << cbs) + lane) * 16 : kOOB), 0, kAuxCoherent));
            b.s = __uint_as_float(__builtin_amdgcn_raw_buffer_load_b32(rs, (int)(lane < (CB >> LPGS) ? (((cc << cbs) >> LPGS) + lane) * 4 : kOOB), 0, kAuxCoherent));
        } else {
            const u32 EPB = (16u << cbs) / T::kEsz;
            const __amdgpu_buffer_rsrc_t rx = __builtin_amdgcn_make_buffer_rsrc(const_cast<float*>(a.x), 0, (int)(n * 4), 0x00020000);
            b.d = __builtin_bit_cast(v4i, __builtin_amdgcn_raw_buffer_load_b128(rx, (int)(4 * lane < EPB ? (cc * EPB + 4 * lane) * 4 : kOOB), 0, kAuxCoherent));
        }
        return b;
    }
    template <int PRO>
    __device__ __forceinline__ void ao_place(char* lds, u32 cc, const AoBlock& b) const {
        char* xq = lds; float* xs = reinterpret_cast<float*>(lds + off_xs);
        const u32 CB = 1u << cbs;
        if constexpr (PRO == PRO_NONE) {
            if (lane < CB) *reinterpret_cast<v4i*>(xq + ((cc << cbs) + lane) * 16) = b.d;
            if (lane < (CB >> LPGS)) xs[((cc << cbs) >> LPGS) + lane] = b.s;
        } else {
            const u32 EPB = (16u << cbs) / T::kEsz, e = cc * EPB + 4 * lane;
            typedef float v4f __attribute__((ext_vector_type(4)));
            const v4f t = __builtin_bit_cast(v4f, b.d);
            quant_round4<QT>(xq, xs, (int)e, 4 * lane < EPB && e < n, make_float4(t.x, t.y, t.z, t.w));
        }
    }
    template <int PRO, class Mid, class Stamp>
    __device__ __forceinline__ void run_ao(const GemvArgs& a, char* lds, const AoSrc& src, Mid&& mid, Stamp&& stamp) {
        xa = v4i{0, 0, 0, 0}; sx2 = 0.f; cur_xo = 0xffffffffu;
        char* strips = lds + off_scr;
        const u32 EPB = (16u << cbs) / T::kEsz, inv_rows = inv_of(src.rows);
        const u32 ks = wave < nw ? wave + nw * (lane >> 4) : NS;
        const u32 kq = udiv(ks, NBCV, inv_NBCV), kc = ks - kq * NBCV;
        const u32 e0 = kc * EPB, e1 = e0 + EPB < n ? e0 + EPB : n;
        const u32 p0 = udiv(e0, src.rows, inv_rows), p1 = udiv(e1 - 1, src.rows, inv_rows), pj = p0 + (lane & 15);
        const bool mine = ks < NS && pj <= p1;
        const unsigned* line = src.flags + (pj % src.grid) * kFlagStride;
        u32 pending = 0;
#pragma unroll
        for (u32 k = 0; k < 4; ++k) if (wave < nw && wave + nw * k < NS) pending |= 1u << k;
        const unsigned long long t0 = __builtin_amdgcn_s_memrealtime();
        bool first = true;
        u32 spins = 0;
        while (pending) {
            const unsigned f = mine ? __hip_atomic_load(line, __ATOMIC_RELAXED, __HIP_MEMORY_SCOPE_AGENT) : src.target;
            const unsigned long long okm = __ballot(flag_reached(f, src.target));
            u32 now = 0;
#pragma unroll
            for (u32 k = 0; k < 4; ++k) if (((okm >> (16 * k)) & 0xFFFFull) == 0xFFFFull) now |= 1u << k;
            now &= pending;
            if (!now) {
                const bool late = give_up_local(t0, src.err);
                if (late || ((++spins & 63u) == 0u && __hip_atomic_load(src.err, __ATOMIC_RELAXED, __HIP_MEMORY_SCOPE_AGENT) != 0)) now = pending;
            }
            AoBlock b[4];
#pragma unroll
            for (u32 k = 0; k < 4; ++k) if (now & (1u << k)) b[k] = ao_fetch<PRO>(a, (u32)__builtin_amdgcn_readlane((int)kc, 16 * k));
            if (first) { first = false; mid(); }
#pragma unroll
            for (u32 k = 0; k < 4; ++k) {
                if (now & (1u << k)) {
                    ao_place<PRO>(lds, (u32)__builtin_amdgcn_readlane((int)kc, 16 * k), b[k]);
                    asm volatile("" ::: "memory");
                    cur_xo = 0xffffffffu;
                    if (k == 0) reduce_step(setA, lds, strips, a.ablate);
                    else if (k == 1) reduce_step(setB, lds, strips, a.ablate);
                    else {
                        wait_stores_done();
                        Set S;
                        load_step(S, wave + nw * k, a.ablate, lds);
                        reduce_step(S, lds, strips, a.ablate);
                    }
                }
            }
            if (pending && now == pending) stamp(3);
            pending &= ~now;
        }
        stamp(4);
        if (np_wg) finish_pass(a, wg, 0, strips, 0);
        stamp(5);
    }
};

__device__ __forceinline__ void xchg_fold(const GemvArgs::XchgFold& x) {
    const unsigned e = *x.base + x.add;
    const int r = threadIdx.x;
    if (threadIdx.x < 64) {
        if (blockIdx.x == 0) {
            __atomic_thread_fence(__ATOMIC_RELEASE);
            if (r < x.world) __hip_atomic_store(x.peer_flags[r] + (x.slot * 8 + x.rank) * kFlagStride, e, __ATOMIC_RELAXED, __HIP_MEMORY_SCOPE_SYSTEM);
        }
        poll_wave<__HIP_MEMORY_SCOPE_SYSTEM, true, 4>(x.local_flags + (x.slot * 8 + r) * kFlagStride, r < x.world, e, x.err, XchgAbortLine<GemvArgs::XchgFold>{x, r});
        __atomic_thread_fence(__ATOMIC_ACQUIRE);
    }
    __syncthreads();
}

template <int QT, int PRO, int EPI, int XR, bool COH = false>
__global__ void __launch_bounds__(kGemvBlock, 4) k_gemv(const GemvArgs a) {
    extern __shared__ __attribute__((aligned(16))) char lds[];
    if (halted(a.halt)) return;
    unsigned long long rt0 = 0;
#ifdef FLM_TRACE_WAVES
    auto stamp = [&](int k) { if (kAblate && a.trace && threadIdx.x == 0 && k == 0) a.trace[blockIdx.x * 8 + k] = __builtin_amdgcn_s_memtime(); };
#else
    auto stamp = [&](int k) { if (kAblate && a.trace && threadIdx.x == 0) a.trace[blockIdx.x * 8 + k] = __builtin_amdgcn_s_memtime(); };
#endif
    if (kAblate && a.trace && threadIdx.x == 0) rt0 = __builtin_amdgcn_s_memrealtime();
    stamp(0);
    if (kAblate && (a.ablate & 16)) return;
    if constexpr (COH) { if (a.xf.world) xchg_fold(a.xf); }
    float4 xv[XR > 0 ? XR : 1], nv[XR > 0 ? XR : 1];
    gemv_preload<QT, PRO, XR, COH>(a, xv, nv);
    GemvCtx<QT, EPI> g;
    g.init(a, blockIdx.x, gridDim.x, lds);
    if constexpr (PRO == PRO_NONE) g.issue(kAblate ? a.ablate : 0);
#ifndef FLM_TRACE_PRO2
    stamp(1);
#endif
    gemv_prologue<QT, PRO, XR, COH>(a, lds, xv, nv, [&](int part) { g.issue(kAblate ? a.ablate : 0, part); });
    stamp(2);
    if (kAblate && (a.ablate & 32)) return;
    g.run(a, lds, stamp);
    stamp(6);
    if (kAblate && a.trace && threadIdx.x == 0) {
        const unsigned long long rt1 = __builtin_amdgcn_s_memrealtime();
        a.trace[blockIdx.x * 8 + 7] = rt1 - rt0;
        if (a.ablate & 64) { a.trace[blockIdx.x * 8 + 1] = rt0; a.trace[blockIdx.x * 8 + 2] = rt1; }
    }
}

}
```

### fast-llama_amd/csrc/flm_host.h

```cpp
#pragma once
#include "flm_gpu.h"
#include "flm_kernels.h"
#include "flm_launch.h"

#include <hip/hip_runtime.h>
#include <rccl/rccl.h>

#include <math.h>
#include <stdio.h>
#include <stdlib.h>
#include <string.h>

#include <map>
#include <string>
#include <mutex>
#include <tuple>
#include <vector>

namespace fh {
using namespace flm;
extern thread_local std::string g_last_error;

struct QMat { void* q = nullptr; float* s = nullptr; int rows = 0, cols = 0; float* st = nullptr;  };
struct LayerW {
    QMat qkv, o, w13, w2;
    float* att_norm = nullptr; float* ffn_norm = nullptr;
    unsigned got = 0;
};

enum KClass { KC_EMBED = 0, KC_QKV, KC_ATTN, KC_ATTN_O, KC_FFN13, KC_FFN2, KC_CLS, KC_ARGMAX, KC_ALLREDUCE, KC_ATTN_WO , KC_FFN , KC_QKV_ATTN_WO , KC_LAYER , KC_BACK , KC_LAYERS , KC_TOKEN  };

struct TimedLaunch { int kclass; hipEvent_t e0, e1; };
struct DevMem { void* p = nullptr; ~DevMem() { if (p) hipFree(p); } };
struct EvPair { hipEvent_t e0 = nullptr, e1 = nullptr; ~EvPair() { if (e0) hipEventDestroy(e0); if (e1) hipEventDestroy(e1); } };
enum class TokenForm { Logits, Greedy, Prompt, Sampled, Shaped, ShapedLp, ShapedEnt };
inline bool shaped_form(TokenForm f) { return f == TokenForm::Shaped || f == TokenForm::ShapedLp || f == TokenForm::ShapedEnt; }
using GraphKey = std::tuple<bool, TokenForm, int, int>;


}
using namespace fh;

constexpr size_t kLdsMax = 160 * 1024;
struct flm_ctx {
    flm_model_desc d{};
    int device = 0, rank = 0, world = 1;
    flm_shard_plan plan{};
    int hs = 0, esz = 1, cu_count = 256, cu_total = 256, n_xcd = 8;
    int dim_local = 0, hidden_local = 0, heads_local = 0, vocab_slot = 0;
    int drow_begin = 0, drow_count = 0;
    hipStream_t stream = nullptr;
    ncclComm_t comm = nullptr;

    std::vector<LayerW> layers;
    void* emb = nullptr; float* emb_s = nullptr; int emb_qt = 0; bool got_emb = false;
    float* out_norm = nullptr; bool got_out_norm = false;
    QMat cls; bool got_cls = false;

    float *kcache = nullptr, *vcache = nullptr;
    int kv_rows = 0;
    float *x1 = nullptr, *qbuf = nullptr, *att_out = nullptr, *hd = nullptr;
    float *logits = nullptr;
    float *rope_cos = nullptr, *rope_sin = nullptr;
    DecodeState* state = nullptr; int* prompt_dev = nullptr; int* out_tokens_dev = nullptr;
    int prompt_cap = 0, out_cap = 0;
    char* bounce = nullptr; size_t bounce_bytes = 0; int err_word = 0; bool err_word_fresh = false;
    bool warmed = false;

    bool tuning = false;
    int wg_per_cu = 1; int use_graph = 1; int ablate = 0;
    int graph_chunks = 1;
    int use_mfma = 1;
    int use_prefill = 1;
    int pf_cap = 0;
    bool pf_in_xbuf = false;
    float *pf_x = nullptr, *pf_qkv = nullptr, *pf_q = nullptr, *pf_att = nullptr, *pf_gu = nullptr, *pf_hd = nullptr, *pf_xs = nullptr, *pf_xst = nullptr; void* pf_xq = nullptr;
    int use_prefill_mq = 1;
    int use_pv_mfma = 1;
    int use_qk_mfma = 1;
    float* pf_scores = nullptr;
    int fold_xchg = 1;
    int ranks_on_device = 1;
    int cu_parts = 1;
    bool tp_prefill = false;
    int fuse_attn_o = 1;
    bool st_ready = false;
    int fuse_ffn = 1;
    int fuse_back = 1;
    int fuse_token = 1;
    int tok_nstq = 4, tok_preq = 99 ;
    void* la_dev[2] = {nullptr, nullptr}; bool la_valid[2] = {false, false}, la_ok[2] = {false, false}; flm::BackArgs la_p[2]; int la_grid[2] = {0, 0}, la_r2[2] = {0, 0};
    int fuse_tail = 1;
    void* tail_dev[2] = {nullptr, nullptr}; bool tail_ok[2] = {false, false};
    unsigned* tail_mem = nullptr;
    int fuse_layer = 1;
    int back_nst13 = -1, back_nst13_head = -1, back_nst2 = 0, back_pre13 = 99 , back_pre2 = 16;
    int attn_kpre = 1;
    int back_nwo = 0;
    int gr_edges = 1;
    granule_t* xg = nullptr; size_t x_gran_off = 0;
    int back_ao = 3, back_ao2 = 2;
    int fuse_qkv = 1;
    unsigned* flag_lines = nullptr; int* xwg_err = nullptr;
    void* att_q = nullptr; float* att_qs = nullptr;
    char* xbuf = nullptr; size_t xbuf_bytes = 0, x_flags_off = 0, x_hflags_off = 0; bool xbuf_fine = false;
    int tp_fuse_ffn = 0;
    unsigned long long* ffn_counter = nullptr;
    int tp_fuse_attn = 2;
    int tp_fuse_layers = 1;
    int tp_fence = -1;
    size_t x_tlines_off = 0;
    char* peer[8] = {nullptr}; bool peer_opened[8] = {false}; int p2p = 0;
    bool grp_fold = false, grp_span = false, grp_can_split = false, grp_tpl = false, grp_gr = false ; int grp_tpfa = 0, grp_tpff = 0, grp_split = 0;
    int force_tp = 0;
    int tp_trust_fused = 0;
    unsigned* xepoch = nullptr;
    float* att_sc = nullptr;
    int attn_split = 1;
    unsigned* eng_base = nullptr;
    int resident = 1;
    int fell_back = 0;
    bool fb_active = false; int fb_tokens = 0; std::vector<int> fb_saved;
    int trace_class = -1; unsigned long long* trace = nullptr;
    flm::SampleParams* sparams = nullptr; unsigned long long* sort_buf = nullptr; long long sampled = 0;
    flm::ShapeParams* shape_p = nullptr; float* shape_row = nullptr; long long shaped = 0;
    flm::ShapeParams* shape_stage = nullptr;
    flm::DfaBlock* dfa_blk = nullptr; int* dfa_dev = nullptr;
    std::vector<int32_t> dfa_row, dfa_tok, dfa_nxt; int dfa_state = -1;
    unsigned long long* gen_host = nullptr; unsigned long long* gen_ring_dev = nullptr; const int* gen_cancel_dev = nullptr; int gen_cap = 0;
    int gen_stop = -1; unsigned gen_tag = 0; int gen_max = 0; unsigned gen_seq = 0;
    int gen_rules = 0;
    std::vector<int32_t> gen_ids; int gen_tokens = 0, gen_streamed = 0;
    int* score_tgt = nullptr; flm::ScoreRow* score_dev = nullptr; bool cls_st_ready = false;
    int* spec_hist = nullptr; int* spec_arg = nullptr; flm::SpecOut* spec_res = nullptr;
    int spec_gemm = 0;
    int spec_steps = 0, spec_accepted = 0;
    flm_ctx* draft = nullptr; hipEvent_t draft_ev[2] = {nullptr, nullptr}; int draft_tokens = 0;
    int lp_top_n = -1, lp_source = 0, lp_count = -1;
    flm::LogprobBlock* lp_blk = nullptr; flm::LogprobRec* lp_rec = nullptr; unsigned* lp_tags = nullptr; float* lp_side = nullptr;
    flm::StopBlock* stop_blk = nullptr; flm::StopBlock stop_host{}; int stop_reason = 0, stop_rule = 0;
    flm::EntropyBlock* ent_blk = nullptr; flm_entropy ent{}; int ent_mode = 0; float ent_mu_fetched = 0.0f;
    int* fan_drawn = nullptr; unsigned long long* fan_after = nullptr; flm::FanOut* fan_res = nullptr;
    flm_fan_layout fan_lay{}; int fan_count[FLM_FAN_MAX] = {0}; bool fan_valid = false;
    struct BatchSlot { bool used = false, live = false; int pos = 0, last = 0, n_out = 0, max_tokens = 0, stop = -1, reason = 0; float temp = 0.0f, topp = 0.0f; unsigned long long rng = 0;
                       bool filling = false; const int32_t* prompt = nullptr; int n_prompt = 0, fed = 0; };
    flm_batch_layout batch_lay{}; BatchSlot batch_slot[FLM_BATCH_MAX]; bool batch_open = false; flm::SlotOut* batch_res = nullptr;
    flm::AttnArgs* batch_views = nullptr;
    flm::AttnArgs* seg_views = nullptr;
    std::vector<int32_t> pass_ids;
    int batch_rows = -1;
    int batch_passes = 0;
    int score_rows = 0;
    std::map<GraphKey, hipGraphExec_t> graphs;
    std::vector<TimedLaunch>* timing = nullptr;
    std::vector<void*> owned;
    std::string err;
};
#include "flm_tuning.h"

namespace fh {

#define HIPC(ctx, expr) do { hipError_t e_ = (expr); if (e_ != hipSuccess) { \
    char b_[512]; snprintf(b_, sizeof b_, "%s failed: %s (%s:%d)", #expr, hipGetErrorString(e_), __FILE__, __LINE__); \
    if (ctx) (ctx)->err = b_; g_last_error = b_; return FLM_ERR_HIP; } } while (0)
#define NCCLC(ctx, expr) do { ncclResult_t r_ = (expr); if (r_ != ncclSuccess) { \
    char b_[512]; snprintf(b_, sizeof b_, "%s failed: %s (%s:%d)", #expr, ncclGetErrorString(r_), __FILE__, __LINE__); \
    if (ctx) (ctx)->err = b_; g_last_error = b_; return FLM_ERR_COMM; } } while (0)

int fail(flm_ctx* c, int code, const char* msg);
int esz_of(int qt);
void split_even(int total, int parts, int idx, int* begin, int* count);

struct GemvPlan { int Rm, cb_shift, grid, nbuf; size_t lds; };
GemvPlan gemv_plan(int n, int esz, int rows, bool two, bool pairs, bool norm, int wgs);
inline int plan_gemv(flm_ctx* c, GemvArgs& a, int esz, int pro, int epi, int wgs, GemvPlan& P) {
    const bool TWO = epi == EPI_SWIGLU, PAIRS = epi == EPI_ROPE_KV;
    const int rows = a.items * (PAIRS ? 2 : 1);
    if ((double)rows * a.n * esz * (TWO ? 2 : 1) >= 2147483648.0) return fail(c, FLM_ERR_UNSUPPORTED, "gemv: matrix of 2 GiB or more");
    P = gemv_plan(a.n, esz, rows, TWO, PAIRS, pro == PRO_RMSNORM_QUANT, wgs);
    if (P.lds > kLdsMax) return fail(c, FLM_ERR_UNSUPPORTED, "gemv: activation vector does not fit LDS");
    a.rows_per_pass = P.Rm; a.cb_shift = P.cb_shift; a.nbuf = P.nbuf;
    return FLM_OK;
}
template <int QT, int PRO, int EPI>
int plan_gemv(flm_ctx* c, GemvArgs& a, int wgs, GemvPlan& P) { return plan_gemv(c, a, QTraits<QT>::kEsz, PRO, EPI, wgs, P); }
inline int gemv_rounds(int n) { return (n + kGemvBlock * 4 - 1) / (kGemvBlock * 4); }
inline int rounds_class(int rounds) { return rounds <= 1 ? 1 : 3; }
template <int QT, int PRO, int EPI, bool COH>
int launch_gemv_xr(flm_ctx* c, hipStream_t st, GemvArgs a, int wgs) {
    GemvPlan P;
    int r = plan_gemv<QT, PRO, EPI>(c, a, wgs, P); if (r) return r;
    const int rounds = gemv_rounds(a.n);
    if (PRO == PRO_NONE)   hipLaunchKernelGGL((k_gemv<QT, PRO, EPI, 0, COH>), dim3(P.grid), dim3(kGemvBlock), P.lds, st, a);
    else if (rounds <= 1)  hipLaunchKernelGGL((k_gemv<QT, PRO, EPI, 1, COH>), dim3(P.grid), dim3(kGemvBlock), P.lds, st, a);
    else if (rounds <= 3)  hipLaunchKernelGGL((k_gemv<QT, PRO, EPI, 3, COH>), dim3(P.grid), dim3(kGemvBlock), P.lds, st, a);
    else                   hipLaunchKernelGGL((k_gemv<QT, PRO, EPI, 0, COH>), dim3(P.grid), dim3(kGemvBlock), P.lds, st, a);
    HIPC(c, hipGetLastError());
    return FLM_OK;
}
template <int PRO, int EPI>
int launch_gemv(flm_ctx* c, hipStream_t st, int qt, const GemvArgs& a, int wgs, bool coh = false) {
    if (a.n % kGroup != 0 || a.n <= 0) return fail(c, FLM_ERR_INVALID, "gemv: n must be a positive multiple of 64");
    if (qt != FLM_QT_INT8 && qt != FLM_QT_INT16) return fail(c, FLM_ERR_UNSUPPORTED, "gemv: quant type must be INT8 or INT16");
    if constexpr (PRO != PRO_NONE) {
        if (coh) return qt == FLM_QT_INT8 ? launch_gemv_xr<QT_INT8, PRO, EPI, true>(c, st, a, wgs) : launch_gemv_xr<QT_INT16, PRO, EPI, true>(c, st, a, wgs);
    }
    return qt == FLM_QT_INT8 ? launch_gemv_xr<QT_INT8, PRO, EPI, false>(c, st, a, wgs) : launch_gemv_xr<QT_INT16, PRO, EPI, false>(c, st, a, wgs);
}
inline int gemv_grid(int cu_count, int wg_per_cu, int , int ) { return cu_count * wg_per_cu; }
int quantize_flat(flm_ctx* c, hipStream_t st, int qt, void* q, float* s, const float* x, size_t n);

constexpr int FLM_RETRY = 1;
int xwg_check(flm_ctx* c);

struct Tick {
    flm_ctx* c; hipStream_t st; int kclass; hipEvent_t e0 = nullptr, e1 = nullptr;
    Tick(flm_ctx* c_, hipStream_t st_, int k) : c(c_), st(st_), kclass(k) {
        if (c->timing) { hipEventCreate(&e0); hipEventCreate(&e1); hipEventRecord(e0, st); }
    }
    ~Tick() { if (c->timing) { hipEventRecord(e1, st); c->timing->push_back({kclass, e0, e1}); } }
};

template <class A> void set_peers(flm_ctx* c, A& a, float* p) {
    a.n_peer = 0;
    if (!c->p2p) return;
    const size_t off = (char*)p - c->xbuf;
    for (int r = 0; r < c->world; ++r) if (r != c->rank) a.out_peer[a.n_peer++] = (float*)(c->peer[r] + off);
}
GemvArgs args_qkv(flm_ctx* c, int l);
constexpr int kSplitFrom = 128;
constexpr int kTpLinesPerRank = 256;
int attn_parts(const flm_ctx* c, int T);
AttnArgs args_attn(flm_ctx* c, int l, int G = 1);
GemvArgs args_o(flm_ctx* c, int l);
GemvArgs args_ffn13(flm_ctx* c, int l);
GemvArgs args_ffn2(flm_ctx* c, int l);
GemvArgs args_cls(flm_ctx* c);
void set_fold(flm_ctx* c, GemvArgs& a, int l, int kind);
int plan_layer_qt(flm_ctx* c, int qt, int l, bool with_qkv, int G, LayerArgs& A, BackArgs& p, int& grid, int& r2, TailArgs* tail);
int launch_layer(flm_ctx* c, hipStream_t st, int qt, int l, bool with_qkv, int G = 1);
int layers_prepare(flm_ctx* c, int G);
int launch_layers(flm_ctx* c, hipStream_t st, int l0, int l1, int G, bool tail = false);
enum XKind { XK_ATT = 0, XK_X1 = 1, XK_HD = 2, XK_LOGITS = 3 };
int exchange(flm_ctx* c, hipStream_t st, int kind, float* full, float* mine, int count);
int enqueue_token(flm_ctx* c, hipStream_t st, bool with_cls, TokenForm form, int G);
int launch_logprob_token(flm_ctx* c, hipStream_t st);
const char* shape_fill(const flm_sampling* sp, int vocab, const int32_t* window, int n_window, bool follow, flm::ShapeParams* out, bool* active);
int run_token(flm_ctx* c, bool with_cls, TokenForm form, int T);
inline bool sample_supported(const flm_ctx* c) { return c->d.vocab_size >= 2 && sample_lds_bytes(c->d.vocab_size) <= kLdsMax; }
int set_state(flm_ctx* c, int pos, int tok, int step);
inline bool sharded(const flm_ctx* c) { return c->world > 1 || (c->comm != nullptr && c->force_tp); }
inline bool logprobs_supported(const flm_ctx* c) { return !sharded(c) && sample_supported(c); }
inline bool entropy_supported(const flm_ctx* c) { return !sharded(c) && sample_supported(c) && c->ent_blk != nullptr; }
inline const int* halt_ptr(const flm_ctx* c) { return sharded(c) ? nullptr : &c->state->halt; }

enum Launch { LF_TOKEN = 0, LF_LAYERS, LF_LAYERS_TP, LF_LAYER, LF_QKV_ATTN_O, LF_BACK, LF_ATTN_O, LF_FFN, kLaunchForms };
constexpr int trace_admits(Launch f) { return f == LF_TOKEN || f == LF_LAYERS ? 103 : f == LF_LAYER || f == LF_BACK ? 102 : f == LF_ATTN_O ? 101 : -1; }
inline bool wants_layers(const flm_ctx* c) { return c->fuse_token != 0; }
struct TokenPlan {
    bool opt[kLaunchForms];
    int qkv;
    bool tp, coh, fold, span; int tpfa, tpff;
    bool use[kLaunchForms];
    bool timing; int trace_class;
    bool runs(Launch f) const { return use[f] && !timing && (trace_class < 0 || trace_class == trace_admits(f)); }
};
inline TokenPlan token_plan(const flm_ctx* c, int G) {
    TokenPlan P{};
    bool* o = P.opt;
    o[LF_ATTN_O] = c->fuse_attn_o != 0;
    o[LF_FFN] = c->fuse_ffn != 0;
    P.qkv = o[LF_ATTN_O] ? c->fuse_qkv : 0;
    o[LF_QKV_ATTN_O] = P.qkv >= 2 || (P.qkv && G > 1);
    o[LF_BACK] = c->fuse_back && o[LF_ATTN_O] && o[LF_FFN];
    o[LF_LAYER] = c->fuse_layer && o[LF_BACK];
    o[LF_LAYERS] = wants_layers(c) && o[LF_LAYER];
    o[LF_TOKEN] = c->fuse_tail && o[LF_LAYERS];
    o[LF_LAYERS_TP] = wants_layers(c);
    P.tp = sharded(c); P.coh = P.tp && c->p2p;
    P.fold = P.tp && c->p2p && c->world > 1 && c->grp_fold;
    P.span = P.fold && c->grp_span;
    P.tpfa = P.span ? c->grp_tpfa : 0; P.tpff = P.span ? c->grp_tpff : 0;
    for (int f = 0; f < kLaunchForms; ++f) P.use[f] = !P.tp && o[f];
    P.use[LF_LAYERS_TP] = P.span && c->grp_tpl && o[LF_LAYERS_TP];
    P.use[LF_QKV_ATTN_O] |= P.tpfa >= 2; P.use[LF_ATTN_O] |= P.tpfa != 0; P.use[LF_FFN] |= P.tpff != 0;
    P.timing = c->timing != nullptr; P.trace_class = c->trace_class;
    return P;
}

using VQuant = Variants<Variant<QT_INT8>, Variant<QT_INT16>>;
using VRounds = Variants<Variant<1>, Variant<3>>;
inline int quant_variant(int qt) { return qt == FLM_QT_INT8 ? QT_INT8 : QT_INT16; }
template <class List, class KernelOf> int raise_lds_limit(flm_ctx* c, KernelOf kernel_of) {
    static std::mutex mu; static bool done[64] = {false};
    std::lock_guard<std::mutex> lk(mu);
    if (c->device >= 0 && c->device < 64 && !done[c->device]) {
        std::vector<const void*> fns;
        for_each_variant(List{}, [&](auto v) { fns.push_back((const void*)kernel_of(v)); });
        for (const void* f : fns) HIPC(c, hipFuncSetAttribute(f, hipFuncAttributeMaxDynamicSharedMemorySize, (int)kLdsMax));
        done[c->device] = true;
    }
    return FLM_OK;
}
inline bool ids_in_vocab(const flm_ctx* c, const int32_t* ids, int n) {
    for (int i = 0; i < n; ++i) if (ids[i] < 0 || ids[i] >= c->d.vocab_size) return false;
    return true;
}
struct SpecDraw;
struct Draw {
    float temperature, topp; uint64_t* rng_state;
    TokenForm form;
    flm::ShapeParams block;
    int cstate = -1;
    bool lp = false;
    bool rules = false;
    int ent = 0; float typical_p = 0.0f;
    Draw(float t = 0.0f, float p = 0.0f, uint64_t* st = nullptr, bool sampler = false) { plain(t, p, st, sampler); }
    void plain(float t, float p, uint64_t* st, bool sampler = false) { temperature = t; topp = p; rng_state = st; form = t != 0.0f || sampler ? TokenForm::Sampled : TokenForm::Greedy; }
    void shape_by(int cq, bool armed, int entropy = 0, float tp = 0.0f) {
        form = entropy ? TokenForm::ShapedEnt : armed ? TokenForm::ShapedLp : TokenForm::Shaped; cstate = cq; lp = armed; ent = entropy; typical_p = entropy == 1 ? tp : 0.0f;
    }
    bool mu_moves() const { return ent == 2 && temperature != 0.0f; }
    bool shaped() const { return shaped_form(form); }
    bool coins() const { return form == TokenForm::Sampled || (shaped() && temperature != 0.0f); }
    int arm(flm_ctx* c) const { return arm_with(c, block, coins() ? (unsigned long long)*rng_state : 0ull, cstate, 0); }
    int arm_step(flm_ctx* c, unsigned long long rng, int q, int rec_base, const int32_t* prompt, int n_prompt, const int32_t* drawn, int n_drawn) const;
    int arm_block(flm_ctx* c) const;
    SpecDraw batch(const flm_ctx* c, unsigned long long base, const int* win, int n_win, int q, int rec_base) const;
    int fetch(flm_ctx* c, unsigned long long* after) const;
    void commit(flm_ctx* c, const int32_t* ids, int n, unsigned long long after) const;
    void commit(flm_ctx* c, int n, unsigned long long after, int q_after) const;
private:
    int arm_with(flm_ctx* c, const flm::ShapeParams& blk, unsigned long long rng, int q, int rec_base) const;
};
int check_ready(flm_ctx* c, int n, int pos);
bool model_complete(const flm_ctx* c);
int run_tokens(flm_ctx* c, int pos, int n, TokenForm form);
int maybe_recover(flm_ctx* c, int tokens);
int feed(flm_ctx* c, const int32_t* tokens, int n, int pos, TokenForm last);
int d2h(flm_ctx* c, void* dst, const void* src_dev, size_t bytes);
float* score_stage(const flm_ctx* c, int* chunk);
constexpr int kPrefillMin = 4;
int prefill_batched_qt(flm_ctx* c, int B, int pos, bool all_layers = false, bool skinny = false, const flm::FanDesc* fan = nullptr, int row0 = 0, const flm::SlotDesc* slots = nullptr, const flm::SegDesc* segs = nullptr);
int fan_classify(flm_ctx* c, int row0, int m, float* stage, bool skinny, float temperature, float topp, const flm::FanIn& in);
int launch_sample_fan(flm_ctx* c, hipStream_t st, const float* logits, int ld, int n, int row0, int rows, float temperature, float topp, const flm::FanIn& in,
                      unsigned long long* sort_buf, int* drawn, unsigned long long* after);
int batch_classify(flm_ctx* c, int src_row0, int row0, int m, float* stage, bool skinny, const flm::SlotIn& in);
int launch_attn_slots(flm_ctx* c, hipStream_t st, const flm::AttnArgs& aa, const flm::SlotDesc& f, int heads, int row_stride, flm::AttnArgs* views);
int launch_rope_kv_slots(flm_ctx* c, hipStream_t st, const float* qkv, float* qout, float* kcache, float* vcache, const float* rope_cos, const float* rope_sin, int dim, int hs, int kv_rows, const flm::SlotDesc& f);
const char* seg_check(const flm::SegDesc& f, int B, int max_seq);
int launch_attn_segs(flm_ctx* c, hipStream_t st, const flm::AttnArgs& aa, const flm::SegDesc& f, int heads, int row_stride, flm::AttnArgs* views, bool one_query);
int launch_rope_kv_segs(flm_ctx* c, hipStream_t st, const float* qkv, float* qout, float* kcache, float* vcache, const float* rope_cos, const float* rope_sin, int dim, int hs, int kv_rows, const flm::SegDesc& f, int B);
int launch_attn_fan(flm_ctx* c, hipStream_t st, const flm::AttnArgs& aa, const flm::FanDesc& f, int heads, int row_stride);
int launch_rope_kv_fan(flm_ctx* c, hipStream_t st, const float* qkv, float* qout, float* kcache, float* vcache, const float* rope_cos, const float* rope_sin, int dim, int hs, int kv_rows, const flm::FanDesc& f);
int score_classify(flm_ctx* c, int row0, int m, float* stage);
struct SpecDraw { float temperature, topp; unsigned long long base; const flm::ShapeParams* shape = nullptr; const int* win = nullptr; int n_win = 0; int cstate = -1 ;
                  float typical_p = 0.0f ;
                  int lp_top_n = -1 , lp_source = 0, lp_base = 0; };
int launch_shape_rows(flm_ctx* c, hipStream_t st, const float* logits, int ld, float* out, int ld_out, int n, int row0, int rows, const flm::ShapeParams* p,
                      const int* win, int n_win, const int* drafts, const flm::DfaBlock* dfa = nullptr, int cstate = -1, int* states_out = nullptr);
inline bool stop_installed(const flm_ctx* c) { return c->stop_blk != nullptr && (c->stop_host.n_ids | c->stop_host.n_seqs) != 0; }
int dfa_fold(const flm_ctx* c, int q, const int32_t* ids, int n);
const char* dfa_check(const flm_dfa* dfa, int vocab);
int spec_classify(flm_ctx* c, int row0, int m, float* stage, bool skinny, int* argmax_out, const SpecDraw& draw);
int launch_logprob_rows(flm_ctx* c, hipStream_t st, const float* rows_dev, int ld, int n, int row0, int rows, const int* chosen, int top_n, flm::LogprobRec* rec, int rec_base, int rec_cap);
int launch_entropy_rows(flm_ctx* c, hipStream_t st, const flm::EntropyRowsArgs& a, int rows);
int launch_sample_rows(flm_ctx* c, hipStream_t st, const float* logits, int ld, int n, int row0, int rows, float temperature, float topp, unsigned long long base,
                       unsigned long long* sort_buf, int* out);
int launch_gemm_skinny_store(flm_ctx* c, hipStream_t st, const GemmArgs& g, int force_nb = 0);
int launch_score_rows(flm_ctx* c, hipStream_t st, const float* logits, int ld, int n, const int* targets, flm::ScoreRow* out, int rows);
int launch_gemm_store(flm_ctx* c, hipStream_t st, int qt, const GemmArgs& g, int use_mfma);
void build_rope_table(int hs, int max_seq, std::vector<float>& cs, std::vector<float>& sn);

}
```

### fast-llama_amd/csrc/flm_layer.h

```cpp
#pragma once
#include "flm_math.h"
#include "flm_gemv.h"
#include "flm_attn.h"
#pragma clang fp contract(off)

namespace flm {

struct BackArgs {
    int n_heads;
    int grido, grid13, grid2;
    int gridq;
    unsigned* flag_q;
    unsigned* flag_h;
    unsigned* flag_x;
    unsigned* flag_hd;
    unsigned* flag_x2;
    int nstq, preq;
    unsigned target; int* err;
    const int* halt;
    unsigned st_base;
    int nst13;
    int nst13_head;
    int nst2;
    int pre2;
    int pre13;
    int ao_o;
    int ao_2;
    int r5;
    unsigned kpre_off;
    int nw_o;
    int nst2_ao;
    unsigned long long* trace;
    granule_t* xg_a; granule_t* xg_b; granule_t* xg_att; granule_t* xg_hd; int gr; int gres_off;
    struct Tp {
        int world, rank;
        unsigned* peer[8];
        unsigned off_h, off_x, off_hd, off_x2, off_cls;
        int head_line0;
        int n_heads_all;
        const unsigned* base;
        int abort_off;
        int fence;
    } tp;
};


template <int PRO, int XR, bool TP>
__device__ __forceinline__ void gemv_preload_granules(const GemvArgs& a, float4 (&xv)[XR], float4 (&wv)[XR], const granule_t* g, const unsigned tag, const BackArgs& p) {
    const __amdgpu_buffer_rsrc_t rg = __builtin_amdgcn_make_buffer_rsrc(const_cast<granule_t*>(g), 0, a.n * 8, 0x00020000);
    const int gave_up = __hip_atomic_load(p.err, __ATOMIC_RELAXED, __HIP_MEMORY_SCOPE_AGENT);
    if constexpr (PRO == PRO_RMSNORM_QUANT) {
        const __amdgpu_buffer_rsrc_t rn = __builtin_amdgcn_make_buffer_rsrc(const_cast<float*>(a.norm_w), 0, a.n * 4, 0x00020000);
#pragma unroll
        for (int i = 0; i < XR; ++i) {
            const v4f u = __builtin_bit_cast(v4f, __builtin_amdgcn_raw_buffer_load_b128(rn, (int)((threadIdx.x * 4 + i * kGemvBlock * 4) * 4), 0, 0));
            wv[i] = make_float4(u.x, u.y, u.z, u.w);
        }
    }
    v4u32 A[XR], C[XR]; bool ok[XR];
#pragma unroll
    for (int i = 0; i < XR; ++i) { A[i] = v4u32{0u, 0u, 0u, 0u}; C[i] = A[i]; ok[i] = (int)(threadIdx.x * 4 + i * kGemvBlock * 4) >= a.n; }
    const unsigned long long t0 = __builtin_amdgcn_s_memrealtime();
    unsigned spins = 0;
    while (true) {
        asm volatile("" ::: "memory");
#pragma unroll
        for (int i = 0; i < XR; ++i) {
            if (!ok[i]) granules4_load(rg, (int)((threadIdx.x * 4 + i * kGemvBlock * 4) * 8), A[i], C[i]);
        }
        bool all = true;
#pragma unroll
        for (int i = 0; i < XR; ++i) { if (!ok[i]) ok[i] = granules4_tagged(A[i], C[i], tag); all = all && ok[i]; }
        if (__all(all) || gave_up) break;
        if constexpr (!TP) { if (give_up_local(t0, p.err)) break; }
        else if ((++spins & (TpAbortLine<BackArgs>::kEvery - 1)) == 0u) { if (give_up_ranks(t0, p.err, TpAbortLine<BackArgs>{p})) break; }
    }
#pragma unroll
    for (int i = 0; i < XR; ++i) { const v4f v = granules4_values(A[i], C[i]); xv[i] = make_float4(v.x, v.y, v.z, v.w); }
}

#ifndef FLM_BACK_LATE
#define FLM_BACK_LATE 1
#endif
#ifndef FLM_BACK_LATE2
#define FLM_BACK_LATE2 0
#endif
#ifndef FLM_LAYER_LATEQ
#define FLM_LAYER_LATEQ 1
#endif
template <int QT, int XR2, bool QKV, bool SPLIT, bool PERSIST, int R5 = 0, bool TP = false, int GRM = 0>
__device__ __forceinline__ void layer_body(const GemvArgs& aq, const AttnArgs& aa, const GemvArgs& ao, const GemvArgs& a13, const GemvArgs& a2, const BackArgs& p, char* lds,
                                           const unsigned target, const bool xpoll, const bool xflag, const bool tracing, const float* x0 = nullptr) {
    auto nostamp = [](int) {};
    auto stamp = [&](int k) { if (kAblate && tracing && p.trace && threadIdx.x == 0) p.trace[blockIdx.x * 16 + k] = __builtin_amdgcn_s_memrealtime(); };
    stamp(0);
    constexpr bool gr = PERSIST && GRM == 2;
    constexpr bool gr_hd = gr && (R5 & 2) == 0;
#ifndef FLM_SPLIT_GRQ
#define FLM_SPLIT_GRQ 1
#endif
    constexpr bool gr_q = gr && !TP && QKV && (FLM_SPLIT_GRQ || !SPLIT);
    constexpr bool gr_att = gr && (TP || SPLIT);
    unsigned nst13 = 0;
    if constexpr (QKV) {
        if ((int)blockIdx.x < p.gridq) {
            GemvCtx<QT, EPI_ROPE_KV, PERSIST> gq;
            float4 xq[1], nq[1];
            if (!PERSIST || !xpoll) gemv_preload<QT, PRO_RMSNORM_QUANT, 1, PERSIST>(aq, xq, nq, x0);
            gq.init(aq, blockIdx.x, p.gridq, lds, 0, p.st_base, (PERSIST && xpoll) ? (unsigned)p.nstq : 0u);
            if (gr_q) { gq.gron = true; gq.gtag = target; }
            if constexpr (PERSIST) {
                if (xpoll) {
                    if ((int)gq.wave < p.preq) gq.issue(kAblate ? aq.ablate : 0, 1);
                    gq.stash_issue(lds);
                    if (gr) {
                        gemv_preload_granules<PRO_RMSNORM_QUANT, 1, TP>(aq, xq, nq, p.xg_a, target - 1u, p);
                        wait_stores_done();
                    } else {
                    poll_lines_t<TP>(p.flag_x2, (TP ? p.tp.world : 1) * p.grid2, target - 1u, p);
                    wait_stores_done();
                    __syncthreads();
                    gemv_preload<QT, PRO_RMSNORM_QUANT, 1, true>(aq, xq, nq);
                    }
                }
            }
            if constexpr (SPLIT) {
                if ((int)blockIdx.x < p.n_heads && p.kpre_off) attn_kpre_issue(aa, blockIdx.x / aa.G, blockIdx.x % aa.G, aa.G, *aa.pos_ptr + 1, lds, p.kpre_off);
            }
            gemv_prologue<QT, PRO_RMSNORM_QUANT, 1, PERSIST, FLM_LAYER_LATEQ != 0>(aq, lds, xq, nq, [&](int) { gq.issue_missing(kAblate ? aq.ablate : 0); });
            stamp(12);
            gq.run(aq, lds, nostamp);
            stamp(13);
            if (gr_q) __syncthreads();
            else {
            wait_stores_done();
            __syncthreads();
            if (threadIdx.x == 0) __hip_atomic_store(p.flag_q + blockIdx.x * kFlagStride, target, __ATOMIC_RELAXED, __HIP_MEMORY_SCOPE_AGENT);
            }
            stamp(14);
        }
    }
    if ((int)blockIdx.x < p.n_heads) {
        const int G = SPLIT ? aa.G : 1, hh = blockIdx.x / G;
        auto qwait = [&]() {
            if (threadIdx.x < 256) {
                const bool need = qkv_line_needed(threadIdx.x, (unsigned)p.gridq, (unsigned)aq.rows_per_pass, (unsigned)aa.hs, (unsigned)hh, (unsigned)aq.dim, (unsigned)aq.kv_dim);
                poll_wave(p.flag_q + threadIdx.x * kFlagStride, need, target, p.err);
            }
            __syncthreads();
        };
        if constexpr (QKV) attn_head_any<true, SPLIT, true, gr_q>(aa, hh, lds, *aa.pos_ptr + 1, aa.q, aa.out, blockIdx.x % G, G, qwait, target, gr_att, gr, (SPLIT && p.kpre_off) ? reinterpret_cast<const float*>(lds + p.kpre_off) : nullptr);
        else attn_head_any<false, SPLIT>(aa, hh, lds, *aa.pos_ptr + 1, aa.q, aa.out, blockIdx.x % G, G);
        stamp(1);
        if (gr_att) __syncthreads();
        else {
        wait_stores_done();
        __syncthreads();
        raise_line<TP>(p, p.flag_h, p.tp.off_h, (TP ? (unsigned)p.tp.head_line0 : 0u) + blockIdx.x, target);
        }
        stamp(2);
        if (p.nst13_head > 0 && (int)blockIdx.x < p.grid13) {
            nst13 = (unsigned)p.nst13_head;
            GemvCtx<QT, EPI_SWIGLU, true> t;
            t.init(a13, blockIdx.x, p.grid13, lds, 0, p.st_base, nst13, false);
            t.stash_issue(lds);
        }
    } else if ((int)blockIdx.x >= p.n_heads + p.grido) {
        if (p.nst13 > 0 && (int)blockIdx.x < p.grid13) {
            nst13 = (unsigned)p.nst13;
            GemvCtx<QT, EPI_SWIGLU, true> t;
            t.init(a13, blockIdx.x, p.grid13, lds, 0, p.st_base, nst13, false);
            t.stash_issue(lds);
        }
    } else {
        GemvCtx<QT, EPI_RESIDUAL> g;
        g.init(ao, blockIdx.x - p.n_heads, p.grido, lds);
        const unsigned nwo = (!SPLIT && (R5 & 1) != 0 && p.nw_o > 0 && p.nw_o < kWavesPerBlock) ? (unsigned)p.nw_o : (unsigned)kWavesPerBlock;
        g.nw = nwo;
        g.resid_src = x0;
        if (gr) { g.gsrc = xpoll ? p.xg_a + p.gres_off : nullptr; g.gron = true; g.gtag = target; }
        g.issue(kAblate ? ao.ablate : 0);
        if (p.nst13 > 0 && (int)blockIdx.x < p.grid13) {
            nst13 = (unsigned)p.nst13;
            GemvCtx<QT, EPI_SWIGLU, true> t;
            t.init(a13, blockIdx.x, p.grid13, lds, 0, p.st_base, nst13, false);
            t.stash_issue(lds, nwo < (unsigned)kWavesPerBlock ? nwo : 0u);
        }
        stamp(1);
#ifdef FLM_TRACE_PRO_RT
        if (kAblate && p.trace && threadIdx.x == 960) { wait_stores_done(); p.trace[blockIdx.x * 16 + 15] = __builtin_amdgcn_s_memrealtime(); }
#endif
        if constexpr (!SPLIT && (R5 & 1) != 0) {
            const typename GemvCtx<QT, EPI_RESIDUAL>::AoSrc src{p.flag_h, (unsigned)aa.hs, (unsigned)p.n_heads, target, p.err};
            g.template run_ao<PRO_NONE>(ao, lds, src, []() {}, [&](int k) { if (k == 3) stamp(2); });
        } else if (gr_att) {
            float4 xv[1], nv[1];
            gemv_preload_granules<PRO_QUANT, 1, TP>(ao, xv, nv, p.xg_att, target, p);
            stamp(2);
            gemv_prologue<QT, PRO_QUANT, 1>(ao, lds, xv, nv, [](int) {});
            g.run(ao, lds, nostamp);
        } else {
        poll_lines_t<TP>(p.flag_h, TP ? p.tp.n_heads_all : p.n_heads, target, p);
        __syncthreads();
        stamp(2);
        float4 xv[1], nv[1];
        if constexpr (SPLIT || TP) {
            gemv_preload<QT, PRO_QUANT, 1, true>(ao, xv, nv);
            gemv_prologue<QT, PRO_QUANT, 1>(ao, lds, xv, nv, [](int) {});
        } else gemv_prologue<QT, PRO_NONE, 0, true>(ao, lds, xv, nv, [](int) {});
        g.run(ao, lds, nostamp);
        }
        stamp(3);
        if (gr) __syncthreads();
        else {
        wait_stores_done();
        __syncthreads();
        raise_line<TP>(p, p.flag_x, p.tp.off_x, (TP ? (unsigned)(p.tp.rank * p.grido) : 0u) + (blockIdx.x - p.n_heads), target);
        }
        stamp(4);
    }
    if ((int)blockIdx.x < p.grid13) {
        GemvCtx<QT, EPI_SWIGLU, true> g;
        g.init(a13, blockIdx.x, p.grid13, lds, 0, p.st_base, nst13);
        if (gr_hd) { g.gron = true; g.gtag = target; }
        if ((int)g.wave < p.pre13) g.issue(kAblate ? a13.ablate : 0, 1);
        float4 xv[1], nv[1];
        if (gr) {
            gemv_preload_granules<PRO_RMSNORM_QUANT, 1, TP>(a13, xv, nv, p.xg_b, target, p);
            wait_stores_done();
            stamp(5);
        } else {
        poll_lines_t<TP>(p.flag_x, (TP ? p.tp.world : 1) * p.grido, target, p);
        wait_stores_done();
        __syncthreads();
        stamp(5);
        gemv_preload<QT, PRO_RMSNORM_QUANT, 1, true>(a13, xv, nv);
        }
        gemv_prologue<QT, PRO_RMSNORM_QUANT, 1, true, FLM_BACK_LATE != 0>(a13, lds, xv, nv, [&](int) { g.issue_missing(kAblate ? a13.ablate : 0); });
        stamp(6);
#ifdef FLM_TRACE_PRO_RT
        g.run(a13, lds, [&](int k) { if (kAblate && a13.trace && threadIdx.x == 0 && k >= 3 && k <= 5) a13.trace[3 * 4096 + blockIdx.x * 16 + k] = __builtin_amdgcn_s_memrealtime(); });
#else
        g.run(a13, lds, nostamp);
#endif
        stamp(7);
    } else if (!gr) {
        poll_lines_t<TP>(p.flag_x, (TP ? p.tp.world : 1) * p.grido, target, p);
    }
    if (gr_hd) __syncthreads();
    else {
    wait_stores_done();
    __syncthreads();
    raise_line<TP>(p, p.flag_hd, p.tp.off_hd, (TP ? (unsigned)p.tp.rank * gridDim.x : 0u) + blockIdx.x, target);
    }
    stamp(8);
    if ((int)blockIdx.x < p.grid2) {
    GemvCtx<QT, EPI_RESIDUAL, true> g2;
    if constexpr ((R5 & 2) != 0) {
        g2.init(a2, blockIdx.x, p.grid2, lds, 0, p.st_base, (unsigned)p.nst2_ao);
        if (gr) { g2.gsrc = p.xg_b + p.gres_off; g2.gron = xflag; g2.gtag = target; }
        const typename GemvCtx<QT, EPI_RESIDUAL, true>::AoSrc src{p.flag_hd, (unsigned)a13.rows_per_pass, (unsigned)p.grid13, target, p.err};
        g2.issue(kAblate ? a2.ablate : 0, p.ao_2 == 1 ? 0 : 1);
        if (p.ao_2 != 2) g2.stash_issue(lds);
        g2.template run_ao<PRO_QUANT>(a2, lds, src, [&]() { g2.issue_missing(kAblate ? a2.ablate : 0); if (p.ao_2 == 2) g2.stash_issue(lds); },
                                      [&](int k) { if (k == 3) stamp(9); else if (k == 4) stamp(10); });
        stamp(11);
    } else {
    g2.init(a2, blockIdx.x, p.grid2, lds, 0, p.st_base, (unsigned)p.nst2);
    if (gr) { g2.gsrc = p.xg_b + p.gres_off; g2.gron = xflag; g2.gtag = target; }
    if ((int)g2.wave < p.pre2) g2.issue(kAblate ? a2.ablate : 0, 1);
    g2.stash_issue(lds);
    float4 xv2[XR2 > 0 ? XR2 : 1], nv2[XR2 > 0 ? XR2 : 1];
    if (gr_hd) {
        gemv_preload_granules<PRO_QUANT, (XR2 > 0 ? XR2 : 1), TP>(a2, xv2, nv2, p.xg_hd, target, p);
        wait_stores_done();
        stamp(9);
    } else {
    poll_lines_t<TP>(p.flag_hd, (TP ? p.tp.world : 1) * (int)gridDim.x, target, p);
    wait_stores_done();
    __syncthreads();
    stamp(9);
    gemv_preload<QT, PRO_QUANT, XR2, true>(a2, xv2, nv2);
    }
    gemv_prologue<QT, PRO_QUANT, XR2, true, FLM_BACK_LATE2 == 1>(a2, lds, xv2, nv2, [&](int) { g2.issue_missing(kAblate ? a2.ablate : 0); });
    stamp(10);
    g2.run(a2, lds, nostamp);
    stamp(11);
    }
    }
    if constexpr (PERSIST) {
        if (xflag) {
            if (gr) __syncthreads();
            else {
            wait_stores_done();
            __syncthreads();
            if ((int)blockIdx.x < p.grid2) raise_line<TP>(p, p.flag_x2, p.tp.off_x2, (TP ? (unsigned)(p.tp.rank * p.grid2) : 0u) + blockIdx.x, target);
            }
        }
    }
}

template <int QT, int XR2, bool QKV = false, bool SPLIT = false>
__global__ void __launch_bounds__(kGemvBlock, 4) k_attn_ffn(const GemvArgs aq, const AttnArgs aa, const GemvArgs ao, const GemvArgs a13, const GemvArgs a2, const BackArgs p) {
    extern __shared__ __attribute__((aligned(16))) char lds[];
    if (halted(p.halt)) return;
    layer_body<QT, XR2, QKV, SPLIT, false>(aq, aa, ao, a13, a2, p, lds, p.target, false, false, true);
}

struct LayerArgs { GemvArgs aq, ao, a13, a2; AttnArgs aa; };
struct TailArgs {
    GemvArgs acls;
    const float* emb; const int* tok_ptr; int dim, vocab;
    unsigned* epoch;
    unsigned* flag_cls;
    float* slots;
    int gridc;
    DecodeState* st; int* out_tokens; int out_cap;
};
template <int QT>
__device__ __forceinline__ void tail_phase(const TailArgs& T, const BackArgs& p, char* lds, const unsigned xtarget, const unsigned ctarget, const unsigned next_epoch) {
    auto nostamp = [](int) {};
    if ((int)blockIdx.x < T.gridc) {
        const GemvArgs& a = T.acls;
        GemvCtx<QT, EPI_STORE, true> gc;
        gc.init(a, blockIdx.x, T.gridc, lds, 0, p.st_base, (unsigned)p.nstq);
        if ((int)gc.wave < p.preq) gc.issue(kAblate ? a.ablate : 0, 1);
        gc.stash_issue(lds);
        float4 xq[1], nq[1];
        gemv_preload_granules<PRO_RMSNORM_QUANT, 1, false>(a, xq, nq, p.xg_a, xtarget, p);
        wait_stores_done();
        gemv_prologue<QT, PRO_RMSNORM_QUANT, 1, true, FLM_LAYER_LATEQ != 0>(a, lds, xq, nq, [&](int) { gc.issue_missing(kAblate ? a.ablate : 0); });
        gc.run(a, lds, nostamp);
        wait_stores_done();
        __syncthreads();
        if (threadIdx.x < 64) {
            float best = -INFINITY; int idx = 0x7fffffff;
            for (unsigned it = 0; it < gc.np_wg; ++it) {
                const unsigned row = (gc.wg + it * gc.nwg) * gc.Rm + threadIdx.x;
                if (threadIdx.x < gc.Rm && row < (unsigned)T.vocab) { const float v = ld_agent(a.out + row); if (v > best) { best = v; idx = (int)row; } }
            }
            for (int o = 32; o > 0; o >>= 1) {
                const float ov = __shfl_xor(best, o, kWave); const int oi = __shfl_xor(idx, o, kWave);
                if (ov > best || (ov == best && oi < idx)) { best = ov; idx = oi; }
            }
            if (threadIdx.x == 0) { st_agent(T.slots + 2 * blockIdx.x, best); st_agent(T.slots + 2 * blockIdx.x + 1, __int_as_float(idx)); }
            wait_stores_done();
            if (threadIdx.x == 0) __hip_atomic_store(T.flag_cls + blockIdx.x * kFlagStride, ctarget, __ATOMIC_RELAXED, __HIP_MEMORY_SCOPE_AGENT);
        }
    }
    if (blockIdx.x == 0) {
        poll_lines(T.flag_cls, T.gridc, ctarget, p.err);
        __syncthreads();
        float* bv = reinterpret_cast<float*>(lds); int* bi = reinterpret_cast<int*>(lds) + 16;
        float best = -INFINITY; int idx = 0x7fffffff;
        if ((int)threadIdx.x < T.gridc) { best = ld_agent(T.slots + 2 * threadIdx.x); idx = __float_as_int(ld_agent(T.slots + 2 * threadIdx.x + 1)); }
        for (int o = 32; o > 0; o >>= 1) {
            const float ov = __shfl_xor(best, o, kWave); const int oi = __shfl_xor(idx, o, kWave);
            if (ov > best || (ov == best && oi < idx)) { best = ov; idx = oi; }
        }
        if ((threadIdx.x & 63) == 0) { bv[threadIdx.x >> 6] = best; bi[threadIdx.x >> 6] = idx; }
        __syncthreads();
        if (threadIdx.x == 0) {
            for (int w = 1; w < kWavesPerBlock; ++w) if (bv[w] > best || (bv[w] == best && bi[w] < idx)) { best = bv[w]; idx = bi[w]; }
            if (idx == 0x7fffffff) idx = 0;
            DecodeState* st = T.st;
            if (T.out_tokens && st->step >= 0 && st->step < T.out_cap) T.out_tokens[st->step] = idx;
            const bool halt = gen_last_act(st, st->step, idx, p.err);
            if (!halt) { st->tok = idx; st->pos += 1; }
            st->step += 1;
            *T.epoch = (FLM_WAIT_FORM == 0 && next_epoch >= kEpochWrap) ? kEpochFirst : next_epoch;
        }
    }
}
template <int QT, int XR2, bool SPLIT, int R5 = 0, bool TAIL = false, bool TP = false, bool GRT = false>
__global__ void __launch_bounds__(kGemvBlock, 4) k_layers(const LayerArgs* __restrict__ LA, const BackArgs p, const int l0, const int l1, const TailArgs* __restrict__ TA = nullptr) {
    static_assert(!TP || (R5 == 0 && !TAIL), "the rank-spanning launch carries the all-to-all hand-offs, the classifier is a launch of its own");
    extern __shared__ __attribute__((aligned(16))) char lds[];
    if constexpr (!TP) { if (halted(p.halt)) return; }
    typedef const LayerArgs __attribute__((address_space(4))) CLayerArgs;
    CLayerArgs* LAc = (CLayerArgs*)(unsigned long long)LA;
    unsigned base = 0; const float* x0 = nullptr;
    if constexpr (TAIL) {
        typedef const TailArgs __attribute__((address_space(4))) CTailArgs;
        const TailArgs& T = *(const TailArgs*)((CTailArgs*)(unsigned long long)TA);
        base = *T.epoch;
        x0 = T.emb + (size_t)(*T.tok_ptr) * T.dim;
    }
    if constexpr (TP) base = *p.tp.base;
    for (int l = l0; l < l1; ++l) {
        const LayerArgs& A = *(const LayerArgs*)(LAc + l);
        layer_body<QT, XR2, true, SPLIT, true, R5, TP, (TP ? (GRT ? 2 : 0) : (TAIL ? 2 : 0))>(A.aq, A.aa, A.ao, A.a13, A.a2, p, lds, base + (unsigned)(l + 1), l > l0, TAIL || l + 1 < l1, l == (l1 - l0 > 1 ? l0 + 1 : l0),
                                                   (TAIL && l == l0) ? x0 : nullptr);
    }
    if constexpr (TAIL) {
        typedef const TailArgs __attribute__((address_space(4))) CTailArgs;
        const TailArgs& T = *(const TailArgs*)((CTailArgs*)(unsigned long long)TA);
        tail_phase<QT>(T, p, lds, base + (unsigned)l1, base + (unsigned)l1 + 1u, base + (unsigned)l1 + 2u);
    }
}

}
```

### fast-llama_amd/csrc/flm_layerlaunch.hip

```cpp
#include "flm_host.h"

namespace fh {

template <int QT>
int plan_layer(flm_ctx* c, int l, bool with_qkv, int G, LayerArgs& A, BackArgs& p, int& grid, int& r2, TailArgs* tail) {
    const auto& d = c->d;
    constexpr int esz = QTraits<QT>::kEsz;
    const int all = c->cu_count < 256 ? c->cu_count : 256, parts = c->heads_local * G, wgs_o = all - parts;
    const bool tpl = c->world > 1 && c->p2p && c->grp_tpl && with_qkv && c->x_tlines_off != 0;
    if ((c->world != 1 && !tpl) || (G == 1 && !tpl && c->hs % kGroup != 0) || wgs_o < 8 || parts > 256) return FLM_ERR_UNSUPPORTED;
    if (tpl && (d.n_heads * G > kTpLinesPerRank || all > kTpLinesPerRank)) return FLM_ERR_UNSUPPORTED;
    if (G > 1 && !with_qkv) return FLM_ERR_UNSUPPORTED;
    GemvArgs aq = args_qkv(c, l), ao = args_o(c, l), a13 = args_ffn13(c, l), a2 = args_ffn2(c, l);
    GemvPlan Pq{}, Po, P13, P2;
    int r = plan_gemv<QT, PRO_QUANT, EPI_RESIDUAL>(c, ao, wgs_o, Po); if (r) return r;
    if (with_qkv) {
        r = plan_gemv<QT, PRO_RMSNORM_QUANT, EPI_ROPE_KV>(c, aq, all, Pq); if (r) return r;
        if (gemv_rounds(aq.n) > 1) return FLM_ERR_UNSUPPORTED;
    }
    r = plan_gemv<QT, PRO_RMSNORM_QUANT, EPI_SWIGLU>(c, a13, all, P13); if (r) return r;
    r = plan_gemv<QT, PRO_QUANT, EPI_RESIDUAL>(c, a2, all, P2); if (r) return r;
    r2 = gemv_rounds(a2.n);
    if (gemv_rounds(a13.n) > 1 || r2 > 3) return FLM_ERR_UNSUPPORTED;
    if ((G > 1 || tpl) && gemv_rounds(ao.n) > 1) return FLM_ERR_UNSUPPORTED;
    auto one_pass = [&](GemvArgs& a, GemvPlan& P, bool two, bool norm, int rows_per_item = 1) {
        const int rows = a.items * rows_per_item, npass = (rows + P.Rm - 1) / P.Rm;
        if (npass <= P.grid) { a.nbuf = 1; P.nbuf = 1; P.lds = (size_t)gemv_lds_layout(a.n, esz, norm, P.Rm, 64 >> P.cb_shift, two, 1).total; }
    };
    one_pass(ao, Po, false, false); one_pass(a13, P13, true, true); one_pass(a2, P2, false, false);
    size_t own = Po.lds; if (P13.lds > own) own = P13.lds; if (P2.lds > own) own = P2.lds;
    if (with_qkv) { one_pass(aq, Pq, false, true, 2); if (Pq.lds > kLdsMax) return FLM_ERR_UNSUPPORTED; if (wants_layers(c) && Pq.lds > own) own = Pq.lds; }
    GemvArgs acls{}; GemvPlan Pc{}; bool tail_fits = false;
    if (tail) {
        tail->gridc = 0;
        const bool gr_tail = c->gr_edges && c->xg && d.dim <= 4 * kGemvBlock && d.dim % 4 == 0 && d.hidden_dim % 4 == 0 && (d.max_seq_len <= kSplitFrom || attn_parts(c, d.max_seq_len) > 1);
        if (gr_tail && c->fuse_tail && with_qkv && wants_layers(c) && c->world == 1 && !tpl && c->got_emb && c->emb_qt == 0 && c->got_cls) {
            acls = args_cls(c);
            if (plan_gemv<QT, PRO_RMSNORM_QUANT, EPI_STORE>(c, acls, all, Pc) == FLM_OK && gemv_rounds(acls.n) <= 1 && Pc.grid <= 256 && Pc.lds + 8 * (kStepBlk * 1024 + 256) <= kLdsMax) {
                tail_fits = true; if (Pc.lds > own) own = Pc.lds;
            }
        }
    }
    own = (own + 255) & ~(size_t)255;
    const size_t lds_attn = attn_lds_bytes(d.max_seq_len, c->hs, G > 1);
    if (own > kLdsMax || lds_attn > kLdsMax) return FLM_ERR_UNSUPPORTED;
    const int slot = kStepBlk * 1024 + 256, fit = (int)((kLdsMax - own) / slot);
    auto slots = [&](int want) { int n = want < 0 ? fit : want; if (n > fit) n = fit; if (n > 32) n = 32; return n < 0 ? 0 : n; };
    AttnArgs aa = args_attn(c, l, G);
    if (G == 1 && !tpl) { aa.oq = c->att_q; aa.os = c->att_qs; aa.oqt = QT; ao.xq = c->att_q; ao.xs = c->att_qs; }
    p = BackArgs{};
    p.n_heads = parts; p.grido = Po.grid; p.grid13 = P13.grid; p.grid2 = P2.grid;
    p.flag_h = c->flag_lines; p.flag_hd = c->flag_lines + 512 * 16; p.flag_x = c->flag_lines + 1024 * 16;
    p.gridq = with_qkv ? Pq.grid : 0; p.flag_q = c->flag_lines + 768 * 16;
    p.target = (unsigned)(l + 1); p.err = c->xwg_err; p.halt = tpl ? nullptr : halt_ptr(c);
    p.st_base = (unsigned)own; p.nst13 = slots(c->back_nst13); p.nst13_head = slots(c->back_nst13_head); p.nst2 = slots(c->back_nst2); p.pre13 = c->back_pre13 == 99 ? 16 : c->back_pre13 < 0 ? 0 : c->back_pre13 > 16 ? 16 : c->back_pre13; p.pre2 = c->back_pre2 < 0 ? 0 : c->back_pre2 > 16 ? 16 : c->back_pre2;
    {
        auto steps = [&](const GemvArgs& a, const GemvPlan& P, int rows) { const int RB = 64 >> P.cb_shift, RBP = P.Rm / RB, nbc = (a.n * esz / 16) >> P.cb_shift; return (rows + P.Rm - 1) / P.Rm <= P.grid ? ((RBP + kStepBlk - 1) / kStepBlk) * nbc : 1 << 30; };
        const int epb_o = (16 << Po.cb_shift) / esz, epb_2 = (16 << P2.cb_shift) / esz;
        const int ns_o = steps(ao, Po, ao.items), ns_2 = steps(a2, P2, a2.items);
        p.ao_o = (c->back_ao & 1) && G == 1 && ns_o <= 32 && ao.n < 65536 && epb_o / c->hs + 2 <= 16 ? 1 : 0;
        const int want2 = ns_2 > 32 ? ns_2 - 32 : 0;
        const bool ok2 = (c->back_ao & 2) && want2 <= fit && want2 <= 32 && a2.n < 65536 && epb_2 <= 256 && epb_2 / P13.Rm + 2 <= 16;
        p.ao_2 = ok2 ? (c->back_ao2 >= 1 && c->back_ao2 <= 3 ? c->back_ao2 : 2) : 0;
        p.nst2_ao = ok2 ? want2 : 0;
        p.r5 = ((G > 1 || p.ao_o) && p.ao_2 && with_qkv && !tpl) ? 3 : 0;
        if (!p.r5) { p.ao_o = 0; p.ao_2 = 0; p.nst2_ao = 0; }
        p.nw_o = kWavesPerBlock;
        if (p.ao_o && G == 1) { const int need = (ns_o + 1) / 2, want = c->back_nwo > 0 ? c->back_nwo : (need < 4 ? 4 : need); p.nw_o = (want >= need && want <= kWavesPerBlock - 2) ? want : kWavesPerBlock; }
    }
    if (kAblate && c->trace_class == 102 && l == 0) { p.trace = c->trace; a13.trace = c->trace + 256 * 16; a2.trace = c->trace + 2 * 256 * 16; }
    if (kAblate && c->trace_class == 103) { p.trace = c->trace; if (l == (c->d.n_layers > 1 ? 1 : 0)) { a13.trace = c->trace + 256 * 16; a2.trace = c->trace + 2 * 256 * 16; aa.trace = c->trace + 5 * 4096; } }
    grid = parts + Po.grid; if (P13.grid > grid) grid = P13.grid; if (P2.grid > grid) grid = P2.grid; if (with_qkv && Pq.grid > grid) grid = Pq.grid;
    if (grid > all) return FLM_ERR_UNSUPPORTED;
    p.xg_a = c->xg; p.xg_b = c->xg + d.dim; p.xg_att = c->xg + 2 * (size_t)d.dim; p.xg_hd = c->xg + 3 * (size_t)d.dim; p.gres_off = c->drow_begin;
    p.gr = (c->gr_edges && c->xg && with_qkv && d.dim <= 4 * kGemvBlock && d.dim % 4 == 0 && d.hidden_dim % 4 == 0 && (tpl ? c->grp_gr : (tail != nullptr && tail_fits))) ? 1 : 0;
    if (p.gr && tpl && c->back_pre13 == 99) p.pre13 = 12;
    if (p.gr && !tpl && G == 1 && c->back_pre13 == 99) p.pre13 = 10;
    {
        auto gpeers = [&](unsigned long long* (&peer)[7], size_t off) { int k = 0; for (int r = 0; r < c->world; ++r) if (r != c->rank) peer[k++] = (unsigned long long*)(c->peer[r] + c->x_gran_off) + off; };
        ao.gout = p.xg_b + c->drow_begin; a2.gout = p.xg_a + c->drow_begin; a13.gout = p.xg_hd + c->plan.hidden_begin;
        aa.gout = p.xg_att + (size_t)c->plan.head_begin * c->hs;
        {
            granule_t* gq = c->xg + 3 * (size_t)d.dim + d.hidden_dim;
            aq.gout = gq; aq.gk = gq + d.dim; aq.gv = gq + d.dim + c->dim_local;
            aa.qg = gq; aa.kg = aq.gk; aa.vg = aq.gv;
        }
        if (tpl && p.gr) {
            gpeers(ao.gout_peer, (size_t)d.dim + c->drow_begin); gpeers(a2.gout_peer, (size_t)c->drow_begin); gpeers(a13.gout_peer, 3 * (size_t)d.dim + c->plan.hidden_begin);
            gpeers(aa.gout_peer, 2 * (size_t)d.dim + (size_t)c->plan.head_begin * c->hs);
        }
    }
    p.flag_x2 = c->flag_lines + 1280 * 16; p.nstq = slots(c->tok_nstq);
    {
        const size_t tile2 = (size_t)2 * 64 * attn_row_stride(c->hs) * 4, off = ((size_t)own + (size_t)p.nstq * slot + 255) & ~(size_t)255;
        p.kpre_off = (G > 1 && with_qkv && c->attn_kpre && off >= attn_lds_bytes(d.max_seq_len, c->hs, false) && off + tile2 <= kLdsMax) ? (unsigned)off : 0u;
    }
    p.preq = c->tok_preq == 99 ? (p.gr ? 12 : 16) : c->tok_preq < 0 ? 0 : c->tok_preq > 16 ? 16 : c->tok_preq;
    if (tpl) {
        BackArgs::Tp& t = p.tp;
        t.world = c->world; t.rank = c->rank;
        for (int r = 0; r < c->world; ++r) t.peer[r] = (unsigned*)(c->peer[r] + c->x_tlines_off);
        const unsigned per = (unsigned)c->world * kTpLinesPerRank * 16;
        t.off_h = 0; t.off_x = kTpLinesPerRank * 16; t.off_hd = t.off_x + per; t.off_x2 = t.off_hd + per; t.off_cls = t.off_x2 + per;
        t.head_line0 = c->plan.head_begin * G; t.n_heads_all = d.n_heads * G;
        t.base = c->eng_base; t.fence = c->tp_fence >= 0 ? c->tp_fence : (c->ranks_on_device == c->world ? 0 : 3);
        t.abort_off = (int)(((long long)c->x_flags_off + (long long)kXchgAbortLine * 64 - (long long)c->x_tlines_off) / 4);
        unsigned* mine = t.peer[c->rank];
        p.flag_h = mine + t.off_h; p.flag_x = mine + t.off_x; p.flag_hd = mine + t.off_hd; p.flag_x2 = mine + t.off_x2;
    }
    A.aq = aq; A.ao = ao; A.a13 = a13; A.a2 = a2; A.aa = aa;
    if (tail && tail_fits && Pc.grid <= grid) {
        TailArgs& T = *tail;
        T.acls = acls; T.emb = (const float*)c->emb; T.tok_ptr = &c->state->tok; T.dim = d.dim; T.vocab = c->cls.rows;
        T.epoch = c->tail_mem; T.flag_cls = c->tail_mem + 16; T.slots = (float*)(c->tail_mem + 16 + 256 * 16); T.gridc = Pc.grid;
        T.st = c->state; T.out_tokens = c->out_tokens_dev; T.out_cap = c->out_cap;
    }
    return FLM_OK;
}
int plan_layer_qt(flm_ctx* c, int qt, int l, bool with_qkv, int G, LayerArgs& A, BackArgs& p, int& grid, int& r2, TailArgs* tail) {
    return qt == FLM_QT_INT8 ? plan_layer<QT_INT8>(c, l, with_qkv, G, A, p, grid, r2, tail) : plan_layer<QT_INT16>(c, l, with_qkv, G, A, p, grid, r2, tail);
}

using VAttnFfn = cross_t<VQuant, cross_t<VRounds, Variants<Variant<0, 0>, Variant<1, 0>, Variant<1, 1>>>>;
int launch_layer(flm_ctx* c, hipStream_t st, int qt, int l, bool with_qkv, int G) {
    LayerArgs A; BackArgs p; int grid = 0, r2 = 0;
    int r = plan_layer_qt(c, qt, l, with_qkv, G, A, p, grid, r2, nullptr); if (r) return r;
    auto kernel_of = [](auto v) { using V = decltype(v); return &k_attn_ffn<V::v[0], V::v[1], V::v[2] != 0, V::v[3] != 0>; };
    r = raise_lds_limit<VAttnFfn>(c, kernel_of); if (r) return r;
    const int want[] = {quant_variant(qt), rounds_class(r2), G > 1 || with_qkv, G > 1};
    if (!dispatch(VAttnFfn{}, want, [&](auto v) { hipLaunchKernelGGL(kernel_of(v), dim3(grid), dim3(kGemvBlock), kLdsMax, st, A.aq, A.aa, A.ao, A.a13, A.a2, p); })) return FLM_ERR_UNSUPPORTED;
    HIPC(c, hipGetLastError());
    return FLM_OK;
}

}
```

### fast-llama_amd/csrc/flm_token.hip

```cpp
#include "flm_host.h"

namespace fh {

GemvPlan gemv_plan(int n, int esz, int rows, bool two, bool pairs, bool norm, int wgs) {
    GemvPlan P{};
    const int nchunks = n * esz / 16;
    int cbs = 0; while (cbs < 6 && (nchunks % (2 << cbs)) == 0) ++cbs;
    const int RB = 64 >> cbs;
    const int mult = (pairs && RB < 2) ? 2 : RB;
    const int lds_budget = 150 * 1024;
    int rmax = 64;
    while (rmax > mult && gemv_lds_layout(n, esz, norm, rmax, RB, two).total > lds_budget) rmax -= mult;
    rmax = rmax / mult * mult; if (rmax < mult) rmax = mult;
    if (rows < 1) rows = 1;
    int ppw = (rows + wgs * rmax - 1) / (wgs * rmax);
    if (ppw < 1) ppw = 1;
    int Rm = (rows + wgs * ppw - 1) / (wgs * ppw);
    Rm = (Rm + mult - 1) / mult * mult; if (Rm > rmax) Rm = rmax; if (Rm < mult) Rm = mult;
    const int npass = (rows + Rm - 1) / Rm;
    P.Rm = Rm; P.cb_shift = cbs; P.grid = npass < wgs ? npass : wgs; if (P.grid < 1) P.grid = 1;
    P.nbuf = 2;
    P.lds = (size_t)gemv_lds_layout(n, esz, norm, Rm, RB, two, P.nbuf).total;
    return P;
}

GemvArgs args_qkv(flm_ctx* c, int l) {
    const auto& d = c->d; LayerW& w = c->layers[l];
    const size_t kv_layer = (size_t)c->heads_local * c->kv_rows * c->hs;
    GemvArgs a{}; a.ablate = c->ablate; a.halt = halt_ptr(c);
    a.W = w.qkv.q; a.sW = w.qkv.s; a.n = d.dim; a.items = w.qkv.rows / 2;
    a.x = c->x1; a.norm_w = w.att_norm;
    a.out = c->qbuf; a.kcache = c->kcache + (size_t)l * kv_layer; a.vcache = c->vcache + (size_t)l * kv_layer;
    a.rope_cos = c->rope_cos; a.rope_sin = c->rope_sin; a.pos_ptr = &c->state->pos;
    a.dim = c->dim_local; a.kv_dim = c->dim_local; a.max_seq = c->kv_rows ; a.hs = c->hs;
    return a;
}

int attn_parts(const flm_ctx* c, int T) {
    const int Gfull = c->hs / kSplitDims;
    if (c->world > 1 && c->p2p) {
        if (!c->grp_can_split || c->grp_split == 0) return 1;
        return (c->grp_split >= 2 || T >= kSplitFrom) ? Gfull : 1;
    }
    const bool can = c->hs % kSplitDims == 0 && Gfull >= 2 && c->hs <= 128 && c->d.max_seq_len <= kSplitMaxSeq && c->heads_local * Gfull + 8 <= c->cu_count && c->heads_local * Gfull <= 256;
    if (!can || c->attn_split == 0) return 1;
    return (c->attn_split >= 2 || T >= kSplitFrom) ? Gfull : 1;
}
AttnArgs args_attn(flm_ctx* c, int l, int G) {
    const auto& d = c->d;
    const size_t kv_layer = (size_t)c->heads_local * c->kv_rows * c->hs;
    AttnArgs a{}; a.halt = halt_ptr(c);
    a.q = c->qbuf; a.kcache = c->kcache + (size_t)l * kv_layer; a.vcache = c->vcache + (size_t)l * kv_layer;
    a.out = c->att_out + (size_t)c->plan.head_begin * c->hs; a.pos_ptr = &c->state->pos; a.hs = c->hs; a.max_seq = d.max_seq_len; a.kv_rows = c->kv_rows;
    a.G = G; a.sc_global = c->att_sc; a.flag_sc = c->flag_lines + 256 * 16; a.epoch = (unsigned)(l + 1); a.err = c->xwg_err;
    set_peers(c, a, a.out);
    return a;
}
GemvArgs args_o(flm_ctx* c, int l) {
    LayerW& w = c->layers[l];
    GemvArgs a{}; a.ablate = c->ablate; a.halt = halt_ptr(c);
    a.W = w.o.q; a.sW = w.o.s; a.n = c->d.dim; a.items = c->drow_count;
    a.x = c->att_out; a.out = c->x1 + c->drow_begin;
    set_peers(c, a, a.out);
    return a;
}
GemvArgs args_ffn13(flm_ctx* c, int l) {
    LayerW& w = c->layers[l];
    GemvArgs a{}; a.ablate = c->ablate; a.halt = halt_ptr(c);
    a.W = w.w13.q; a.sW = w.w13.s; a.n = c->d.dim; a.items = c->hidden_local;
    a.x = c->x1; a.norm_w = w.ffn_norm; a.out = c->hd + c->plan.hidden_begin;
    set_peers(c, a, a.out);
    return a;
}
GemvArgs args_ffn2(flm_ctx* c, int l) {
    LayerW& w = c->layers[l];
    GemvArgs a{}; a.ablate = c->ablate; a.halt = halt_ptr(c);
    a.W = w.w2.q; a.sW = w.w2.s; a.n = c->d.hidden_dim; a.items = c->drow_count;
    a.x = c->hd; a.out = c->x1 + c->drow_begin;
    set_peers(c, a, a.out);
    return a;
}
GemvArgs args_cls(flm_ctx* c) {
    GemvArgs a{}; a.ablate = c->ablate; a.halt = halt_ptr(c);
    a.W = c->cls.q; a.sW = c->cls.s; a.n = c->d.dim; a.items = c->cls.rows;
    a.x = c->x1; a.norm_w = c->out_norm; a.out = c->logits + (c->world > 1 ? (size_t)c->rank * c->vocab_slot : 0);
    set_peers(c, a, a.out);
    return a;
}


void set_fold(flm_ctx* c, GemvArgs& a, int l, int kind) {
    a.xf.world = 0;
    if (!(c->world > 1 && c->p2p && c->fold_xchg)) return;
    a.xf.local_flags = (unsigned*)(c->xbuf + c->x_flags_off);
    for (int r = 0; r < c->world; ++r) a.xf.peer_flags[r] = (unsigned*)(c->peer[r] + c->x_flags_off);
    a.xf.base = c->eng_base; a.xf.add = (unsigned)(4 * l + kind + 1);
    a.xf.rank = c->rank; a.xf.world = c->world; a.xf.slot = 4 + (kind == 3 ? 1 : kind); a.xf.err = c->xwg_err;
}

using VAttnO = cross_t<VQuant, Variants<Variant<0, 1, 0>, Variant<1, 0, 0>, Variant<3, 0, 0>, Variant<1, 0, 1>, Variant<3, 0, 1>>>;
using VQkvAttnO = cross_t<VQuant, Variants<Variant<0, 1, 0, 0>, Variant<1, 0, 0, 0>, Variant<3, 0, 0, 0>, Variant<1, 0, 1, 0>, Variant<3, 0, 1, 0>,
                                           Variant<1, 0, 0, 1>, Variant<3, 0, 0, 1>, Variant<1, 0, 1, 1>, Variant<3, 0, 1, 1>>>;
using VFfn = cross_t<VQuant, cross_t<VRounds, Variants<Variant<0>, Variant<1>>>>;

static int launch_attn_o(flm_ctx* c, hipStream_t st, int qt, int l, int G, bool with_qkv) {
    const auto& d = c->d;
    const int qv = quant_variant(qt), parts = c->heads_local * G, all = with_qkv && c->cu_count > 256 ? 256 : c->cu_count, wgs = all - parts;
    if (wgs < 1 || parts > 256) return FLM_ERR_UNSUPPORTED;
    GemvArgs aq = with_qkv ? args_qkv(c, l) : GemvArgs{}, a = args_o(c, l);
    if (!with_qkv && kAblate && c->trace_class == 101 && l == 0) a.trace = c->trace;
    GemvPlan Pq{}, P;
    int r = with_qkv ? plan_gemv(c, aq, c->esz, PRO_RMSNORM_QUANT, EPI_ROPE_KV, all, Pq) : FLM_OK; if (r) return r;
    r = plan_gemv(c, a, c->esz, PRO_QUANT, EPI_RESIDUAL, wgs, P); if (r) return r;
    const int rounds = gemv_rounds(a.n);
    if ((with_qkv && gemv_rounds(aq.n) > 1) || rounds > 3) return FLM_ERR_UNSUPPORTED;
    size_t lds = attn_lds_bytes(d.max_seq_len, c->hs, G > 1); if (P.lds > lds) lds = P.lds; if (Pq.lds > lds) lds = Pq.lds;
    AttnArgs aa = args_attn(c, l, G);
    unsigned* flag = c->flag_lines;
    unsigned* flagq = c->flag_lines + 768 * 16;
    unsigned target = (unsigned)(l + 1);
    const dim3 grid(parts + P.grid > Pq.grid ? parts + P.grid : Pq.grid), block(kGemvBlock);
    AoTp tp{};
    bool preq = false;
    if (c->world > 1) {
        if (d.n_heads * G > 256) return FLM_ERR_UNSUPPORTED;
        if (with_qkv && l > 0) set_fold(c, aq, l - 1, 3);
        tp.world = c->world; tp.line0 = c->plan.head_begin * G; tp.n_lines = d.n_heads * G; tp.base = c->eng_base; tp.add = (unsigned)(4 * l + 1);
        for (int r = 0; r < c->world; ++r) tp.peer_flags[r] = (unsigned*)(c->peer[r] + c->x_hflags_off);
        flag = (unsigned*)(c->xbuf + c->x_hflags_off); if (!with_qkv) target = 0u;
    } else if (c->hs % kGroup == 0 && G == 1) {
        preq = true; aa.oq = c->att_q; aa.os = c->att_qs; aa.oqt = qv; a.xq = c->att_q; a.xs = c->att_qs;
    }
    const int want[] = {qv, preq ? 0 : rounds_class(rounds), preq, G > 1, c->world > 1};
    const int want_o[] = {want[0], want[1], want[2], want[3]};
    const bool found = with_qkv
        ? dispatch(VQkvAttnO{}, want, [&](auto v) { using V = decltype(v);
              hipLaunchKernelGGL((k_qkv_attn_o<V::v[0], V::v[1], V::v[2] != 0, V::v[3] != 0, V::v[4] != 0>), grid, block, lds, st, aq, aa, a, Pq.grid, parts, P.grid, flagq, flag, target, c->xwg_err, tp); })
        : dispatch(VAttnO{}, want_o, [&](auto v) { using V = decltype(v);
              hipLaunchKernelGGL((k_attn_o<V::v[0], V::v[1], V::v[2] != 0, V::v[3] != 0>), grid, block, lds, st, aa, a, parts, flag, target, c->xwg_err, tp); });
    if (!found) return FLM_ERR_UNSUPPORTED;
    HIPC(c, hipGetLastError());
    return FLM_OK;
}

static int launch_ffn(flm_ctx* c, hipStream_t st, int qt, int l) {
    GemvArgs a13 = args_ffn13(c, l), a2 = args_ffn2(c, l);
    const int qv = quant_variant(qt), wgs = c->cu_count < 256 ? c->cu_count : 256;
    GemvPlan P13, P2;
    int r = plan_gemv(c, a13, c->esz, PRO_RMSNORM_QUANT, EPI_SWIGLU, wgs, P13); if (r) return r;
    r = plan_gemv(c, a2, c->esz, PRO_QUANT, EPI_RESIDUAL, wgs, P2); if (r) return r;
    const int r2 = gemv_rounds(a2.n);
    if (gemv_rounds(a13.n) > 1 || r2 > 3) return FLM_ERR_UNSUPPORTED;
    const size_t lds = P13.lds > P2.lds ? P13.lds : P2.lds;
    const int grid = P13.grid > P2.grid ? P13.grid : P2.grid;
    unsigned* flag = c->flag_lines + 512 * 16;
    unsigned target = (unsigned)(l + 1);
    FfnTp tp{};
    if (c->world > 1) {
        set_fold(c, a13, l, 1);
        tp.world = c->world; tp.rank = c->rank; tp.base = c->eng_base; tp.add = (unsigned)(4 * l + 3); tp.counter = c->ffn_counter;
        for (int r = 0; r < c->world; ++r) tp.peer_flags[r] = (unsigned*)(c->peer[r] + c->x_hflags_off) + 256 * 16;
        flag = (unsigned*)(c->xbuf + c->x_hflags_off) + 256 * 16; target = 0u;
    }
    const int want[] = {qv, rounds_class(r2), c->world > 1};
    if (!dispatch(VFfn{}, want, [&](auto v) { using V = decltype(v);
            hipLaunchKernelGGL((k_ffn<V::v[0], V::v[1], V::v[2] != 0>), dim3(grid), dim3(kGemvBlock), lds, st, a13, a2, P13.grid, P2.grid, flag, target, c->xwg_err, tp); }))
        return FLM_ERR_UNSUPPORTED;
    HIPC(c, hipGetLastError());
    return FLM_OK;
}

static int launch_embed(flm_ctx* c, hipStream_t st) {
    const int dim = c->d.dim;
    hipLaunchKernelGGL(k_embed, dim3((dim + 255) / 256), dim3(256), 0, st, c->x1, (const void*)c->emb, (const float*)c->emb_s, c->emb_qt, dim, (const int*)&c->state->tok, c->flag_lines, c->eng_base, c->ffn_counter, halt_ptr(c));
    HIPC(c, hipGetLastError());
    return FLM_OK;
}
static int launch_attn_decode(flm_ctx* c, hipStream_t st, int l, int G, bool trace) {
    AttnArgs aa = args_attn(c, l, G); if (trace) aa.trace = c->trace;
    hipLaunchKernelGGL(G > 1 ? k_attn_decode<true> : k_attn_decode<false>, dim3(c->heads_local * (G > 1 ? G : 1)), dim3(kAttnBlock), attn_lds_bytes(c->d.max_seq_len, c->hs, G > 1), st, aa);
    HIPC(c, hipGetLastError());
    return FLM_OK;
}
static SampleArgs args_sample(flm_ctx* c, const float* row) {
    SampleArgs sa{};
    sa.logits = row; sa.n = c->d.vocab_size; sa.sp = c->sparams; sa.st = c->state; sa.out_tokens = c->out_tokens_dev; sa.out_cap = c->out_cap; sa.advance = 1; sa.sort_buf = c->sort_buf; sa.err = c->xwg_err;
    return sa;
}
static int launch_argmax_advance(flm_ctx* c, hipStream_t st, const float* row) {
    hipLaunchKernelGGL(k_argmax_advance, dim3(1), dim3(1024), 0, st, row, c->d.vocab_size, c->state, c->out_tokens_dev, 1, c->out_cap, (const int*)c->xwg_err);
    HIPC(c, hipGetLastError());
    return FLM_OK;
}

int exchange(flm_ctx* c, hipStream_t st, int kind, float* full, float* mine, int count) {
    Tick t(c, st, KC_ALLREDUCE);
    if (c->p2p) {
        XchgArgs x{};
        x.local_flags = (unsigned*)(c->xbuf + c->x_flags_off);
        for (int r = 0; r < c->world; ++r) x.peer_flags[r] = (unsigned*)(c->peer[r] + c->x_flags_off);
        x.epoch = c->xepoch + kind; x.err = c->xwg_err; x.rank = c->rank; x.world = c->world; x.kind = kind;
        hipLaunchKernelGGL(k_xchg, dim3(1), dim3(64), 0, st, x);
        HIPC(c, hipGetLastError());
        return FLM_OK;
    }
    if (!c->comm) return fail(c, FLM_ERR_STATE, "tensor parallel: neither flm_p2p_import was called nor an RCCL id was given");
    NCCLC(c, ncclAllGather(mine, full, count, ncclFloat, c->comm, st));
    return FLM_OK;
}

int launch_logprob_token(flm_ctx* c, hipStream_t st) {
    if (!logprobs_supported(c) || !c->lp_rec) return fail(c, FLM_ERR_UNSUPPORTED, "logprobs: one GPU, a vocabulary within the sampler's LDS bound");
    LogprobArgs la{};
    la.raw = c->logits; la.shaped = c->shape_row; la.n = c->d.vocab_size; la.blk = c->lp_blk; la.st = c->state; la.out_tokens = c->out_tokens_dev; la.out_cap = c->out_cap;
    la.rec = c->lp_rec; la.tags = c->lp_tags; la.rec_cap = c->d.max_seq_len;
    hipLaunchKernelGGL(k_logprob_token, dim3(1), dim3(kSampleBlock), logprob_lds_bytes(c->d.vocab_size), st, la);
    HIPC(c, hipGetLastError());
    return FLM_OK;
}
static int enqueue_draw(flm_ctx* c, hipStream_t st, TokenForm form, bool tp) {
    const auto& d = c->d;
    if (form == TokenForm::Logits) return FLM_OK;
    const bool shaped = shaped_form(form);
    const float* row = c->logits;
    if (shaped) {
        if (tp) return fail(c, FLM_ERR_UNSUPPORTED, "shaped token: one GPU only");
        ShapeArgs ha{};
        ha.logits = c->logits; ha.out = c->shape_row; ha.n = d.vocab_size; ha.p = c->shape_p; ha.st = c->state; ha.out_tokens = c->out_tokens_dev; ha.out_cap = c->out_cap; ha.dfa = c->dfa_blk;
        hipLaunchKernelGGL(k_shape_logits, dim3(1), dim3(kSampleBlock), 0, st, ha);
        HIPC(c, hipGetLastError());
        row = c->shape_row;
    }
    if (form == TokenForm::Sampled && !sample_supported(c)) return fail(c, FLM_ERR_UNSUPPORTED, "device sampler: vocabulary too large for one workgroup's LDS");
    {
        Tick t(c, st, KC_ARGMAX);
        if ((shaped || form == TokenForm::Sampled) && sample_supported(c)) {
            SampleArgs sa = args_sample(c, row);
            if (shaped) sa.stop = c->stop_blk;
            if (form == TokenForm::ShapedEnt) {
                if (!c->ent_blk) return fail(c, FLM_ERR_UNSUPPORTED, "entropy token: no device block");
                hipLaunchKernelGGL(k_entropy_advance, dim3(1), dim3(kSampleBlock), sample_lds_bytes(d.vocab_size), st, EntropyArgs{sa, c->ent_blk});
            } else {
                hipLaunchKernelGGL(k_sample_advance, dim3(1), dim3(kSampleBlock), sample_lds_bytes(d.vocab_size), st, sa);
            }
            HIPC(c, hipGetLastError());
        } else {
            if (form == TokenForm::ShapedEnt) return fail(c, FLM_ERR_UNSUPPORTED, "entropy token: vocabulary too large for one workgroup's LDS");
            const int r = launch_argmax_advance(c, st, row); if (r) return r;
        }
    }
    if (form == TokenForm::ShapedLp) return launch_logprob_token(c, st);
    return FLM_OK;
}

int enqueue_token(flm_ctx* c, hipStream_t st, bool with_cls, TokenForm form, int G) {
    const auto& d = c->d;
    const int qt = d.quant_type, hs = c->hs, L = d.n_layers;
    const TokenPlan P = token_plan(c, G);
    const bool tp = P.tp, coh = P.coh, fold = P.fold;
    if (with_cls && form == TokenForm::Greedy && P.runs(LF_TOKEN)) {
        const int r = launch_layers(c, st, 0, L, G, true);
        if (r != FLM_ERR_UNSUPPORTED) return r;
    }
    int r;
    { Tick t(c, st, KC_EMBED); r = launch_embed(c, st); if (r) return r; }
    const int wgs = gemv_grid(c->cu_count, c->wg_per_cu, 0, 0);
    auto traced = [&](GemvArgs a, int kc, int l) { if (kAblate && c->trace_class == kc && l == 0) a.trace = c->trace; return a; };
    auto folded = [&](GemvArgs a, int l, int kind) { if (fold && l >= 0) set_fold(c, a, l, kind); return a; };
    if (P.runs(LF_LAYERS)) {
        r = launch_layers(c, st, 0, L, G);
        if (r == FLM_OK) goto layers_done; else if (r != FLM_ERR_UNSUPPORTED) return r;
    }
    if (P.runs(LF_LAYERS_TP)) {
        r = launch_layers(c, st, 0, L, G);
        if (r == FLM_OK) {
            if (!with_cls) { r = exchange(c, st, XK_X1, c->x1, c->x1 + c->drow_begin, c->drow_count); if (r) return r; }
            goto layers_done;
        } else if (r != FLM_ERR_UNSUPPORTED) return r;
    }
    for (int l = 0; l < L; ++l) {
        bool fused = false;
        if (P.runs(LF_LAYER)) {
            r = launch_layer(c, st, qt, l, true, G);
            if (r == FLM_OK) continue; else if (r != FLM_ERR_UNSUPPORTED) return r;
        }
        if (P.runs(LF_QKV_ATTN_O)) {
            r = launch_attn_o(c, st, qt, l, G, true);
            if (r == FLM_OK) fused = true; else if (r != FLM_ERR_UNSUPPORTED) return r;
        }
        if (!fused) {
            Tick t(c, st, KC_QKV);
            r = launch_gemv<PRO_RMSNORM_QUANT, EPI_ROPE_KV>(c, st, qt, folded(traced(args_qkv(c, l), KC_QKV, l), l - 1, 3), wgs, coh); if (r) return r;
        }
        if (!fused && P.runs(LF_BACK) && G == 1) {
            r = launch_layer(c, st, qt, l, false);
            if (r == FLM_OK) continue; else if (r != FLM_ERR_UNSUPPORTED) return r;
        }
        if (!fused && P.runs(LF_ATTN_O)) {
            r = launch_attn_o(c, st, qt, l, G, false);
            if (r == FLM_OK) fused = true; else if (r != FLM_ERR_UNSUPPORTED) return r;
        }
        if (!fused) { Tick t(c, st, KC_ATTN); r = launch_attn_decode(c, st, l, G, kAblate && c->trace_class == KC_ATTN && l == 0); if (r) return r; }
        if (tp && !fold) { r = exchange(c, st, XK_ATT, c->att_out, c->att_out + (size_t)c->plan.head_begin * hs, c->dim_local); if (r) return r; }
        if (!fused) {
            Tick t(c, st, KC_ATTN_O);
            r = launch_gemv<PRO_QUANT, EPI_RESIDUAL>(c, st, qt, folded(traced(args_o(c, l), KC_ATTN_O, l), l, 0), wgs, coh); if (r) return r;
        }
        if (tp && !fold) { r = exchange(c, st, XK_X1, c->x1, c->x1 + c->drow_begin, c->drow_count); if (r) return r; }
        if (P.runs(LF_FFN)) {
            r = launch_ffn(c, st, qt, l);
            if (r == FLM_OK) {
                if (tp && l == L - 1 && !with_cls) { r = exchange(c, st, XK_X1, c->x1, c->x1 + c->drow_begin, c->drow_count); if (r) return r; }
                continue;
            } else if (r != FLM_ERR_UNSUPPORTED) return r;
        }
        {
            Tick t(c, st, KC_FFN13);
            r = launch_gemv<PRO_RMSNORM_QUANT, EPI_SWIGLU>(c, st, qt, folded(traced(args_ffn13(c, l), KC_FFN13, l), l, 1), wgs, coh); if (r) return r;
        }
        if (tp && !fold) { r = exchange(c, st, XK_HD, c->hd, c->hd + c->plan.hidden_begin, c->hidden_local); if (r) return r; }
        {
            Tick t(c, st, KC_FFN2);
            r = launch_gemv<PRO_QUANT, EPI_RESIDUAL>(c, st, qt, folded(traced(args_ffn2(c, l), KC_FFN2, l), l, 2), wgs, coh); if (r) return r;
        }
        if (tp && (!fold || (l == L - 1 && !with_cls))) { r = exchange(c, st, XK_X1, c->x1, c->x1 + c->drow_begin, c->drow_count); if (r) return r; }
    }
layers_done:
// ... 128 lines not shown
```

Baseline: 555.0 tokens/s.

## Precompute GEMV geometry on host and read it from kernel args

Moves the per-block GEMV geometry setup (LDS layout, pass counts, reciprocal divisors, buffer resource sizes) into a host-computed GemvGeom struct stored in the kernel arguments. Device init now loads these values instead of computing them, optionally pinned to scalar constant address space, and k_attn_ffn reads its argument blocks straight from the kernarg segment. The aim is to cut per-layer setup latency from integer divisions and layout arithmetic. In exchange the argument structs grow by 128 bytes each, and every host path must fill the geometry consistently.

```diff
diff --git a/fast-llama_amd/csrc/flm_attn.h b/fast-llama_amd/csrc/flm_attn.h
--- a/fast-llama_amd/csrc/flm_attn.h
+++ b/fast-llama_amd/csrc/flm_attn.h
@@ -1044,7 +1044,7 @@
         return;
     }
     GemvCtx<QT, EPI_RESIDUAL> g;
-    g.init(a, blockIdx.x - n_heads, gridDim.x - n_heads, lds);
+    g.init(a, blockIdx.x - n_heads, lds);
     g.issue(kAblate ? a.ablate : 0);
     stamp(1);
     const int n_poll = tp.world ? tp.n_lines : n_heads;
@@ -1081,7 +1081,7 @@
         float4 xq[1], nq[1];
         gemv_preload<QT, PRO_RMSNORM_QUANT, 1, TP>(aq, xq, nq);
         GemvCtx<QT, EPI_ROPE_KV> gq;
-        gq.init(aq, blockIdx.x, gridq, lds);
+        gq.init(aq, blockIdx.x, lds);
         gemv_prologue<QT, PRO_RMSNORM_QUANT, 1, TP>(aq, lds, xq, nq, [&](int part) { gq.issue(kAblate ? aq.ablate : 0, part); });
         gq.run(aq, lds, nostamp);
         wait_stores_done();
@@ -1108,7 +1108,7 @@
     }
     if ((int)blockIdx.x >= n_heads + grido) return;
     GemvCtx<QT, EPI_RESIDUAL> g;
-    g.init(a, blockIdx.x - n_heads, grido, lds);
+    g.init(a, blockIdx.x - n_heads, lds);
     g.issue(kAblate ? a.ablate : 0);
     const int n_poll = TP ? tp.n_lines : n_heads;
     if ((int)(threadIdx.x & ~63u) < n_poll) {
@@ -1141,7 +1141,7 @@
         float4 xv[1], nv[1];
         gemv_preload<QT, PRO_RMSNORM_QUANT, 1, TP>(a13, xv, nv);
         GemvCtx<QT, EPI_SWIGLU> g;
-        g.init(a13, blockIdx.x, grid13, lds);
+        g.init(a13, blockIdx.x, lds);
         gemv_prologue<QT, PRO_RMSNORM_QUANT, 1, TP>(a13, lds, xv, nv, [&](int part) { g.issue(kAblate ? a13.ablate : 0, part); });
         g.run(a13, lds, nostamp);
     }
@@ -1158,7 +1158,7 @@
     }
     if ((int)blockIdx.x >= grid2) return;
     GemvCtx<QT, EPI_RESIDUAL> g2;
-    g2.init(a2, blockIdx.x, grid2, lds);
+    g2.init(a2, blockIdx.x, lds);
     g2.issue(kAblate ? a2.ablate : 0, 1);
     if (threadIdx.x < 256) {
         const bool mine = (int)threadIdx.x < (TP ? tp.world : (int)gridDim.x);
diff --git a/fast-llama_amd/csrc/flm_gemv.h b/fast-llama_amd/csrc/flm_gemv.h
--- a/fast-llama_amd/csrc/flm_gemv.h
+++ b/fast-llama_amd/csrc/flm_gemv.h
@@ -1,6 +1,7 @@
 #pragma once
 #include "flm_math.h"
 #include "flm_wait.h"
+#include "flm_geom.h"
 #pragma clang fp contract(off)
 
 namespace flm {
@@ -32,6 +33,7 @@
     } xf;
     void* dbg_xq; float* dbg_xs; float* dbg_xn;
     unsigned long long* trace;
+    GemvGeom geom;
     int ablate;
 };
 
@@ -44,32 +46,8 @@
 #define FLM_ABLATE 0
 #endif
 constexpr bool kAblate = FLM_ABLATE != 0;
-constexpr int kStepBlk = 4;
-
-__host__ __device__ inline int chain_bshift(int n) { int s = 2; while ((64 << s) < n / 4) ++s; return s; }
-__host__ __device__ inline int chain_strip_floats(int n) { return 64 * ((1 << chain_bshift(n)) + 4); }
-struct GemvLds {
-    int off_xs, off_red, off_ctr, off_scr;
-    int gstride;
-    int buf_bytes;
-    int total;
-};
-__host__ __device__ inline GemvLds gemv_lds_layout(int n, int esz, bool norm, int Rm, int RB, bool two, int nbuf = 2) {
-    GemvLds L;
-    const int sn = n / kGroup, ng = two ? 2 * sn : sn;
-    L.off_xs = n * esz;
-    L.off_red = L.off_xs + ((sn * 4 + 15) & ~15);
-    L.off_ctr = L.off_red + 64;
-    L.off_scr = L.off_ctr + 16;
-    int g16 = (ng * 8 + 15) / 16; if ((g16 & 1) == 0) ++g16;
-    L.gstride = g16 * 16;
-    L.buf_bytes = (Rm + RB) * L.gstride;
-    int scratch = nbuf * L.buf_bytes + 64;
-    const int chain = 4 * chain_strip_floats(n) * 4 + 64;
-    if (norm && chain > scratch) scratch = chain;
-    L.total = L.off_scr + scratch;
-    return L;
-}
+
+static_assert(kGeomGroup == kGroup, "flm_geom.h states the quantization group on its own");
 __device__ __forceinline__ float sq_chain(const float* p, int n4) {
     float l = 0.f;
     int k = 0;
@@ -460,32 +438,28 @@
     const granule_t* gsrc; bool gron; unsigned gtag;
     u32 nw;
 
-    static __device__ __forceinline__ u32 inv_of(u32 d) { return d > 1 ? 0xFFFFFFFFu / d + 1u : 0u; }
     static __device__ __forceinline__ u32 udiv(u32 x, u32 d, u32 inv) { return d > 1 ? __umulhi(x, inv) : x; }
 
-    __device__ __forceinline__ void init(const GemvArgs& a, u32 wg_, u32 nwg_, char* lds, u32 ctr_slot = 0, u32 st_base_ = 0, u32 st_n_ = 0, bool write_ctr = true) {
-        n = a.n; wg = wg_; nwg = nwg_; st_base = st_base_; st_n = st_n_;
+    template <bool PIN = false>
+    __device__ __forceinline__ void init(const GemvArgs& a, u32 wg_, char* lds, u32 st_base_ = 0, u32 st_n_ = 0, bool write_ctr = true) {
+        const GemvGeom* Gp = &a.geom;
+        if constexpr (PIN) {
+            typedef const GemvGeom __attribute__((address_space(4))) CGeom;
+            unsigned long long ga = (unsigned long long)Gp;
+            asm volatile("" : "+s"(ga));
+            Gp = (const GemvGeom*)((CGeom*)ga);
+        }
+        const GemvGeom& G = *Gp;
+        wg = wg_; st_base = st_base_; st_n = st_n_;
         lane = threadIdx.x & 63;
         wave = __builtin_amdgcn_readfirstlane(threadIdx.x >> 6);
-        rowbytes = n * T::kEsz; sn = n / kGroup;
-        const u32 nchunks = rowbytes / 16;
-        cbs = a.cb_shift; RB = 64u >> cbs;
+        n = G.n; rowbytes = G.rowbytes; sn = G.sn; cbs = G.cbs; RB = G.RB; nbc = G.nbc; NBCV = G.NBCV; TRm = G.TRm; Rm = G.Rm; RBP = G.RBP; SP = G.SP; npass = G.npass;
+        inv_SP = G.inv_SP; inv_NBCV = G.inv_NBCV; nwg = G.nwg; nbuf = G.nbuf;
+        gstride = G.gstride; buf_bytes = G.buf_bytes; off_xs = G.off_xs; off_scr = G.off_scr; ctr_off = G.ctr_off;
+        dW = G.dW; dS = G.dS; dT = G.dT; dummy_st = G.dummy_st;
+        np_wg = G.np_q + (wg < G.np_rem ? 1u : 0u);
+        NS = np_wg * SP;
         const u32 CB = 1u << cbs;
-        nbc = nchunks >> cbs;
-        NBCV = TWO ? 2 * nbc : nbc;
-        TRm = (u32)a.items * (EPI == EPI_ROPE_KV ? 2u : 1u);
-        Rm = a.rows_per_pass;
-        RBP = Rm / RB;
-        npass = (TRm + Rm - 1) / Rm;
-        np_wg = wg < npass ? (npass - wg + nwg - 1) / nwg : 0;
-        SP = ((RBP + H - 1) / H) * NBCV;
-        NS = np_wg * SP;
-        inv_SP = inv_of(SP); inv_NBCV = inv_of(NBCV);
-        nbuf = a.nbuf > 0 ? a.nbuf : 2;
-        const GemvLds L = gemv_lds_layout(n, T::kEsz, true, Rm, RB, TWO, nbuf);
-        gstride = L.gstride; buf_bytes = L.buf_bytes; off_xs = L.off_xs; off_scr = L.off_scr; ctr_off = a.ctr_off ? (u32)a.ctr_off : (u32)L.off_ctr + 4 * (ctr_slot & 1);
-        dW = RB * rowbytes; dS = RB * sn * 4; dT = RB * gstride;
-        dummy_st = Rm * gstride;
         const u32 rb = lane >> cbs, cb = lane & (CB - 1);
         lane_woff = rb * rowbytes + cb * 16;
         lane_xoff = cb * 16;
@@ -498,9 +472,8 @@
         lane_sx2off = (cb2 >> LPGS) * 4;
         lane_poff = lane_j * dT + rb2 * gstride + (cb2 >> LPGS) * ES + ES / 2;
         constexpr int kRsrcFlags = 0x00020000;
-        const u32 NM = TWO ? 2u : 1u;
-        rW = __builtin_amdgcn_make_buffer_rsrc(const_cast<void*>(a.W), 0, (int)(NM * TRm * rowbytes), kRsrcFlags);
-        rS = __builtin_amdgcn_make_buffer_rsrc(const_cast<float*>(a.sW), 0, (int)(NM * TRm * sn * 4), kRsrcFlags);
+        rW = __builtin_amdgcn_make_buffer_rsrc(const_cast<void*>(a.W), 0, (int)G.wbytes, kRsrcFlags);
+        rS = __builtin_amdgcn_make_buffer_rsrc(const_cast<float*>(a.sW), 0, (int)G.sbytes, kRsrcFlags);
         stored = false; primedA = primedB = false; resid_src = nullptr; gsrc = nullptr; gron = false; gtag = 0; nw = kWavesPerBlock;
         if (write_ctr && threadIdx.x == 0) *reinterpret_cast<u32*>(lds + ctr_off) = 2 * kWavesPerBlock;
     }
@@ -747,7 +720,7 @@
 
     struct AoSrc {
         const unsigned* flags;
-        u32 rows, grid;
+        u32 rows, inv_rows, grid;
         unsigned target; int* err;
     };
     struct AoBlock { v4i d; float s; };
@@ -785,7 +758,7 @@
     __device__ __forceinline__ void run_ao(const GemvArgs& a, char* lds, const AoSrc& src, Mid&& mid, Stamp&& stamp) {
         xa = v4i{0, 0, 0, 0}; sx2 = 0.f; cur_xo = 0xffffffffu;
         char* strips = lds + off_scr;
-        const u32 EPB = (16u << cbs) / T::kEsz, inv_rows = inv_of(src.rows);
+        const u32 EPB = (16u << cbs) / T::kEsz, inv_rows = src.inv_rows;
         const u32 ks = wave < nw ? wave + nw * (lane >> 4) : NS;
         const u32 kq = udiv(ks, NBCV, inv_NBCV), kc = ks - kq * NBCV;
         const u32 e0 = kc * EPB, e1 = e0 + EPB < n ? e0 + EPB : n;
@@ -869,7 +842,7 @@
     float4 xv[XR > 0 ? XR : 1], nv[XR > 0 ? XR : 1];
     gemv_preload<QT, PRO, XR, COH>(a, xv, nv);
     GemvCtx<QT, EPI> g;
-    g.init(a, blockIdx.x, gridDim.x, lds);
+    g.init(a, blockIdx.x, lds);
     if constexpr (PRO == PRO_NONE) g.issue(kAblate ? a.ablate : 0);
 #ifndef FLM_TRACE_PRO2
     stamp(1);
diff --git a/fast-llama_amd/csrc/flm_geom.h b/fast-llama_amd/csrc/flm_geom.h
--- /dev/null
+++ b/fast-llama_amd/csrc/flm_geom.h
@@ -0,0 +1,110 @@
+#pragma once
+#include <stddef.h>
+#include <stdint.h>
+
+#if defined(__HIPCC__) || defined(__CUDACC__)
+#define FLM_GEOM_HD __host__ __device__
+#else
+#define FLM_GEOM_HD
+#endif
+
+namespace flm {
+
+constexpr int kGeomGroup = 64;
+constexpr int kStepBlk = 4;
+
+FLM_GEOM_HD inline int chain_bshift(int n) { int s = 2; while ((64 << s) < n / 4) ++s; return s; }
+FLM_GEOM_HD inline int chain_strip_floats(int n) { return 64 * ((1 << chain_bshift(n)) + 4); }
+struct GemvLds {
+    int off_xs, off_red, off_ctr, off_scr;
+    int gstride;
+    int buf_bytes;
+    int total;
+};
+FLM_GEOM_HD inline GemvLds gemv_lds_layout(int n, int esz, bool norm, int Rm, int RB, bool two, int nbuf = 2) {
+    GemvLds L;
+    const int sn = n / kGeomGroup, ng = two ? 2 * sn : sn;
+    L.off_xs = n * esz;
+    L.off_red = L.off_xs + ((sn * 4 + 15) & ~15);
+    L.off_ctr = L.off_red + 64;
+    L.off_scr = L.off_ctr + 16;
+    int g16 = (ng * 8 + 15) / 16; if ((g16 & 1) == 0) ++g16;
+    L.gstride = g16 * 16;
+    L.buf_bytes = (Rm + RB) * L.gstride;
+    int scratch = nbuf * L.buf_bytes + 64;
+    const int chain = 4 * chain_strip_floats(n) * 4 + 64;
+    if (norm && chain > scratch) scratch = chain;
+    L.total = L.off_scr + scratch;
+    return L;
+}
+
+struct GemvPlan { int Rm, cb_shift, grid, nbuf; size_t lds; };
+inline GemvPlan gemv_plan(int n, int esz, int rows, bool two, bool pairs, bool norm, int wgs) {
+    GemvPlan P{};
+    const int nchunks = n * esz / 16;
+    int cbs = 0; while (cbs < 6 && (nchunks % (2 << cbs)) == 0) ++cbs;
+    const int RB = 64 >> cbs;
+    const int mult = (pairs && RB < 2) ? 2 : RB;
+    const int lds_budget = 150 * 1024;
+    int rmax = 64;
+    while (rmax > mult && gemv_lds_layout(n, esz, norm, rmax, RB, two).total > lds_budget) rmax -= mult;
+    rmax = rmax / mult * mult; if (rmax < mult) rmax = mult;
+    if (rows < 1) rows = 1;
+    int ppw = (rows + wgs * rmax - 1) / (wgs * rmax);
+    if (ppw < 1) ppw = 1;
+    int Rm = (rows + wgs * ppw - 1) / (wgs * ppw);
+    Rm = (Rm + mult - 1) / mult * mult; if (Rm > rmax) Rm = rmax; if (Rm < mult) Rm = mult;
+    const int npass = (rows + Rm - 1) / Rm;
+    P.Rm = Rm; P.cb_shift = cbs; P.grid = npass < wgs ? npass : wgs; if (P.grid < 1) P.grid = 1;
+    P.nbuf = 2;
+    P.lds = (size_t)gemv_lds_layout(n, esz, norm, Rm, RB, two, P.nbuf).total;
+    return P;
+}
+
+FLM_GEOM_HD inline uint32_t gemv_inv_of(uint32_t d) { return d > 1 ? 0xFFFFFFFFu / d + 1u : 0u; }
+
+struct alignas(16) GemvGeom {
+    uint32_t n, rowbytes, sn, cbs;
+    uint32_t RB, nbc, NBCV, TRm;
+    uint32_t Rm, RBP, SP, npass;
+    uint32_t inv_SP, inv_NBCV;
+    uint32_t np_q, np_rem;
+    uint32_t nwg, nbuf;
+    uint32_t gstride, buf_bytes, off_xs, off_scr, ctr_off;
+    uint32_t dW, dS, dT, dummy_st;
+    uint32_t wbytes, sbytes;
+    uint32_t src_rows, inv_src_rows;
+    uint32_t pad_;
+};
+static_assert(sizeof(GemvGeom) == 128, "GemvGeom: 32 dwords");
+
+FLM_GEOM_HD inline GemvGeom gemv_geom(int n, int esz, int items, int Rm, int cb_shift, int nbuf, int ctr_off, bool TWO, bool PAIRS, int nwg) {
+    GemvGeom g;
+    const uint32_t H = (uint32_t)kStepBlk;
+    g.n = (uint32_t)n; g.rowbytes = g.n * (uint32_t)esz; g.sn = g.n / (uint32_t)kGeomGroup;
+    const uint32_t nchunks = g.rowbytes / 16;
+    g.cbs = (uint32_t)cb_shift; g.RB = 64u >> g.cbs;
+    g.nbc = nchunks >> g.cbs;
+    g.NBCV = TWO ? 2 * g.nbc : g.nbc;
+    g.TRm = (uint32_t)items * (PAIRS ? 2u : 1u);
+    g.Rm = (uint32_t)Rm;
+    g.RBP = g.Rm / g.RB;
+    g.npass = (g.TRm + g.Rm - 1) / g.Rm;
+    g.SP = ((g.RBP + H - 1) / H) * g.NBCV;
+    g.inv_SP = gemv_inv_of(g.SP); g.inv_NBCV = gemv_inv_of(g.NBCV);
+    g.nwg = nwg > 0 ? (uint32_t)nwg : 1u;
+    g.np_q = g.npass / g.nwg; g.np_rem = g.npass % g.nwg;
+    g.nbuf = nbuf > 0 ? (uint32_t)nbuf : 2u;
+    const GemvLds L = gemv_lds_layout(n, esz, true, Rm, (int)g.RB, TWO, (int)g.nbuf);
+    g.gstride = (uint32_t)L.gstride; g.buf_bytes = (uint32_t)L.buf_bytes; g.off_xs = (uint32_t)L.off_xs; g.off_scr = (uint32_t)L.off_scr;
+    g.ctr_off = ctr_off ? (uint32_t)ctr_off : (uint32_t)L.off_ctr;
+    g.dW = g.RB * g.rowbytes; g.dS = g.RB * g.sn * 4; g.dT = g.RB * g.gstride;
+    g.dummy_st = g.Rm * g.gstride;
+    const uint32_t NM = TWO ? 2u : 1u;
+    g.wbytes = NM * g.TRm * g.rowbytes; g.sbytes = NM * g.TRm * g.sn * 4;
+    g.src_rows = 0; g.inv_src_rows = 0; g.pad_ = 0;
+    return g;
+}
+FLM_GEOM_HD inline void gemv_geom_src(GemvGeom& g, uint32_t rows) { g.src_rows = rows; g.inv_src_rows = gemv_inv_of(rows); }
+
+}
diff --git a/fast-llama_amd/csrc/flm_host.h b/fast-llama_amd/csrc/flm_host.h
--- a/fast-llama_amd/csrc/flm_host.h
+++ b/fast-llama_amd/csrc/flm_host.h
@@ -171,8 +171,9 @@
 int esz_of(int qt);
 void split_even(int total, int parts, int idx, int* begin, int* count);
 
-struct GemvPlan { int Rm, cb_shift, grid, nbuf; size_t lds; };
-GemvPlan gemv_plan(int n, int esz, int rows, bool two, bool pairs, bool norm, int wgs);
+inline void fill_geom(GemvArgs& a, int esz, int epi, int grid) {
+    a.geom = gemv_geom(a.n, esz, a.items, a.rows_per_pass, a.cb_shift, a.nbuf, a.ctr_off, epi == EPI_SWIGLU, epi == EPI_ROPE_KV, grid);
+}
 inline int plan_gemv(flm_ctx* c, GemvArgs& a, int esz, int pro, int epi, int wgs, GemvPlan& P) {
     const bool TWO = epi == EPI_SWIGLU, PAIRS = epi == EPI_ROPE_KV;
     const int rows = a.items * (PAIRS ? 2 : 1);
@@ -180,6 +181,7 @@
     P = gemv_plan(a.n, esz, rows, TWO, PAIRS, pro == PRO_RMSNORM_QUANT, wgs);
     if (P.lds > kLdsMax) return fail(c, FLM_ERR_UNSUPPORTED, "gemv: activation vector does not fit LDS");
     a.rows_per_pass = P.Rm; a.cb_shift = P.cb_shift; a.nbuf = P.nbuf;
+    fill_geom(a, esz, epi, P.grid);
     return FLM_OK;
 }
 template <int QT, int PRO, int EPI>
diff --git a/fast-llama_amd/csrc/flm_layer.h b/fast-llama_amd/csrc/flm_layer.h
--- a/fast-llama_amd/csrc/flm_layer.h
+++ b/fast-llama_amd/csrc/flm_layer.h
@@ -92,7 +92,17 @@
 __device__ __forceinline__ void layer_body(const GemvArgs& aq, const AttnArgs& aa, const GemvArgs& ao, const GemvArgs& a13, const GemvArgs& a2, const BackArgs& p, char* lds,
                                            const unsigned target, const bool xpoll, const bool xflag, const bool tracing, const float* x0 = nullptr) {
     auto nostamp = [](int) {};
+#ifdef FLM_TRACE_SETUP
+    auto stamp = [](int) {};
+    auto sstamp = [&](int e, int s, int waves = 3) {
+        __builtin_amdgcn_sched_barrier(0);
+        if (kAblate && tracing && p.trace && ((threadIdx.x == 0 && (waves & 1)) || (threadIdx.x == 960 && (waves & 2)))) p.trace[blockIdx.x * 16 + 4 * e + (threadIdx.x ? 2 : 0) + s] = __builtin_amdgcn_s_memrealtime();
+        __builtin_amdgcn_sched_barrier(0);
+    };
+#else
     auto stamp = [&](int k) { if (kAblate && tracing && p.trace && threadIdx.x == 0) p.trace[blockIdx.x * 16 + k] = __builtin_amdgcn_s_memrealtime(); };
+    auto sstamp = [](int, int, int = 3) {};
+#endif
     stamp(0);
     constexpr bool gr = PERSIST && GRM == 2;
     constexpr bool gr_hd = gr && (R5 & 2) == 0;
@@ -107,12 +117,14 @@
             GemvCtx<QT, EPI_ROPE_KV, PERSIST> gq;
             float4 xq[1], nq[1];
             if (!PERSIST || !xpoll) gemv_preload<QT, PRO_RMSNORM_QUANT, 1, PERSIST>(aq, xq, nq, x0);
-            gq.init(aq, blockIdx.x, p.gridq, lds, 0, p.st_base, (PERSIST && xpoll) ? (unsigned)p.nstq : 0u);
+            sstamp(3, 0);
+            gq.template init<true>(aq, blockIdx.x, lds, p.st_base, (PERSIST && xpoll) ? (unsigned)p.nstq : 0u);
             if (gr_q) { gq.gron = true; gq.gtag = target; }
             if constexpr (PERSIST) {
                 if (xpoll) {
                     if ((int)gq.wave < p.preq) gq.issue(kAblate ? aq.ablate : 0, 1);
                     gq.stash_issue(lds);
+                    sstamp(3, 1);
                     if (gr) {
                         gemv_preload_granules<PRO_RMSNORM_QUANT, 1, TP>(aq, xq, nq, p.xg_a, target - 1u, p);
                         wait_stores_done();
@@ -162,36 +174,39 @@
         if (p.nst13_head > 0 && (int)blockIdx.x < p.grid13) {
             nst13 = (unsigned)p.nst13_head;
             GemvCtx<QT, EPI_SWIGLU, true> t;
-            t.init(a13, blockIdx.x, p.grid13, lds, 0, p.st_base, nst13, false);
+            t.template init<true>(a13, blockIdx.x, lds, p.st_base, nst13, false);
             t.stash_issue(lds);
         }
     } else if ((int)blockIdx.x >= p.n_heads + p.grido) {
         if (p.nst13 > 0 && (int)blockIdx.x < p.grid13) {
             nst13 = (unsigned)p.nst13;
             GemvCtx<QT, EPI_SWIGLU, true> t;
-            t.init(a13, blockIdx.x, p.grid13, lds, 0, p.st_base, nst13, false);
+            t.template init<true>(a13, blockIdx.x, lds, p.st_base, nst13, false);
             t.stash_issue(lds);
         }
     } else {
         GemvCtx<QT, EPI_RESIDUAL> g;
-        g.init(ao, blockIdx.x - p.n_heads, p.grido, lds);
+        sstamp(0, 0);
+        g.template init<true>(ao, blockIdx.x - p.n_heads, lds);
         const unsigned nwo = (!SPLIT && (R5 & 1) != 0 && p.nw_o > 0 && p.nw_o < kWavesPerBlock) ? (unsigned)p.nw_o : (unsigned)kWavesPerBlock;
         g.nw = nwo;
         g.resid_src = x0;
         if (gr) { g.gsrc = xpoll ? p.xg_a + p.gres_off : nullptr; g.gron = true; g.gtag = target; }
         g.issue(kAblate ? ao.ablate : 0);
+        sstamp(0, 1, 1);
         if (p.nst13 > 0 && (int)blockIdx.x < p.grid13) {
             nst13 = (unsigned)p.nst13;
             GemvCtx<QT, EPI_SWIGLU, true> t;
-            t.init(a13, blockIdx.x, p.grid13, lds, 0, p.st_base, nst13, false);
+            t.template init<true>(a13, blockIdx.x, lds, p.st_base, nst13, false);
             t.stash_issue(lds, nwo < (unsigned)kWavesPerBlock ? nwo : 0u);
         }
         stamp(1);
+        sstamp(0, 1, 2);
 #ifdef FLM_TRACE_PRO_RT
         if (kAblate && p.trace && threadIdx.x == 960) { wait_stores_done(); p.trace[blockIdx.x * 16 + 15] = __builtin_amdgcn_s_memrealtime(); }
 #endif
         if constexpr (!SPLIT && (R5 & 1) != 0) {
-            const typename GemvCtx<QT, EPI_RESIDUAL>::AoSrc src{p.flag_h, (unsigned)aa.hs, (unsigned)p.n_heads, target, p.err};
+            const typename GemvCtx<QT, EPI_RESIDUAL>::AoSrc src{p.flag_h, ao.geom.src_rows, ao.geom.inv_src_rows, (unsigned)p.n_heads, target, p.err};
             g.template run_ao<PRO_NONE>(ao, lds, src, []() {}, [&](int k) { if (k == 3) stamp(2); });
         } else if (gr_att) {
             float4 xv[1], nv[1];
@@ -221,9 +236,11 @@
     }
     if ((int)blockIdx.x < p.grid13) {
         GemvCtx<QT, EPI_SWIGLU, true> g;
-        g.init(a13, blockIdx.x, p.grid13, lds, 0, p.st_base, nst13);
+        sstamp(1, 0);
+        g.template init<true>(a13, blockIdx.x, lds, p.st_base, nst13);
         if (gr_hd) { g.gron = true; g.gtag = target; }
         if ((int)g.wave < p.pre13) g.issue(kAblate ? a13.ablate : 0, 1);
+        sstamp(1, 1);
         float4 xv[1], nv[1];
         if (gr) {
             gemv_preload_granules<PRO_RMSNORM_QUANT, 1, TP>(a13, xv, nv, p.xg_b, target, p);
@@ -256,20 +273,23 @@
     stamp(8);
     if ((int)blockIdx.x < p.grid2) {
     GemvCtx<QT, EPI_RESIDUAL, true> g2;
+    sstamp(2, 0);
     if constexpr ((R5 & 2) != 0) {
-        g2.init(a2, blockIdx.x, p.grid2, lds, 0, p.st_base, (unsigned)p.nst2_ao);
+        g2.template init<true>(a2, blockIdx.x, lds, p.st_base, (unsigned)p.nst2_ao);
         if (gr) { g2.gsrc = p.xg_b + p.gres_off; g2.gron = xflag; g2.gtag = target; }
-        const typename GemvCtx<QT, EPI_RESIDUAL, true>::AoSrc src{p.flag_hd, (unsigned)a13.rows_per_pass, (unsigned)p.grid13, target, p.err};
+        const typename GemvCtx<QT, EPI_RESIDUAL, true>::AoSrc src{p.flag_hd, a2.geom.src_rows, a2.geom.inv_src_rows, (unsigned)p.grid13, target, p.err};
         g2.issue(kAblate ? a2.ablate : 0, p.ao_2 == 1 ? 0 : 1);
         if (p.ao_2 != 2) g2.stash_issue(lds);
+        sstamp(2, 1);
         g2.template run_ao<PRO_QUANT>(a2, lds, src, [&]() { g2.issue_missing(kAblate ? a2.ablate : 0); if (p.ao_2 == 2) g2.stash_issue(lds); },
                                       [&](int k) { if (k == 3) stamp(9); else if (k == 4) stamp(10); });
         stamp(11);
     } else {
-    g2.init(a2, blockIdx.x, p.grid2, lds, 0, p.st_base, (unsigned)p.nst2);
+    g2.template init<true>(a2, blockIdx.x, lds, p.st_base, (unsigned)p.nst2);
     if (gr) { g2.gsrc = p.xg_b + p.gres_off; g2.gron = xflag; g2.gtag = target; }
     if ((int)g2.wave < p.pre2) g2.issue(kAblate ? a2.ablate : 0, 1);
     g2.stash_issue(lds);
+    sstamp(2, 1);
     float4 xv2[XR2 > 0 ? XR2 : 1], nv2[XR2 > 0 ? XR2 : 1];
     if (gr_hd) {
         gemv_preload_granules<PRO_QUANT, (XR2 > 0 ? XR2 : 1), TP>(a2, xv2, nv2, p.xg_hd, target, p);
@@ -300,11 +320,15 @@
     }
 }
 
+struct AttnFfnKargs { GemvArgs aq; AttnArgs aa; GemvArgs ao, a13, a2; BackArgs p; };
+static_assert(sizeof(AttnFfnKargs) <= 4096, "k_attn_ffn: five argument blocks by value must fit the kernel-argument segment");
 template <int QT, int XR2, bool QKV = false, bool SPLIT = false>
 __global__ void __launch_bounds__(kGemvBlock, 4) k_attn_ffn(const GemvArgs aq, const AttnArgs aa, const GemvArgs ao, const GemvArgs a13, const GemvArgs a2, const BackArgs p) {
     extern __shared__ __attribute__((aligned(16))) char lds[];
-    if (halted(p.halt)) return;
-    layer_body<QT, XR2, QKV, SPLIT, false>(aq, aa, ao, a13, a2, p, lds, p.target, false, false, true);
+    typedef const AttnFfnKargs __attribute__((address_space(4))) CKargs;
+    const AttnFfnKargs& K = *(const AttnFfnKargs*)((CKargs*)__builtin_amdgcn_kernarg_segment_ptr());
+    if (halted(K.p.halt)) return;
+    layer_body<QT, XR2, QKV, SPLIT, false>(K.aq, K.aa, K.ao, K.a13, K.a2, K.p, lds, K.p.target, false, false, true);
 }
 
 struct LayerArgs { GemvArgs aq, ao, a13, a2; AttnArgs aa; };
@@ -323,7 +347,7 @@
     if ((int)blockIdx.x < T.gridc) {
         const GemvArgs& a = T.acls;
         GemvCtx<QT, EPI_STORE, true> gc;
-        gc.init(a, blockIdx.x, T.gridc, lds, 0, p.st_base, (unsigned)p.nstq);
+        gc.template init<true>(a, blockIdx.x, lds, p.st_base, (unsigned)p.nstq);
         if ((int)gc.wave < p.preq) gc.issue(kAblate ? a.ablate : 0, 1);
         gc.stash_issue(lds);
         float4 xq[1], nq[1];
diff --git a/fast-llama_amd/csrc/flm_layerlaunch.hip b/fast-llama_amd/csrc/flm_layerlaunch.hip
--- a/fast-llama_amd/csrc/flm_layerlaunch.hip
+++ b/fast-llama_amd/csrc/flm_layerlaunch.hip
@@ -25,9 +25,13 @@
     if ((G > 1 || tpl) && gemv_rounds(ao.n) > 1) return FLM_ERR_UNSUPPORTED;
     auto one_pass = [&](GemvArgs& a, GemvPlan& P, bool two, bool norm, int rows_per_item = 1) {
         const int rows = a.items * rows_per_item, npass = (rows + P.Rm - 1) / P.Rm;
-        if (npass <= P.grid) { a.nbuf = 1; P.nbuf = 1; P.lds = (size_t)gemv_lds_layout(a.n, esz, norm, P.Rm, 64 >> P.cb_shift, two, 1).total; }
+        if (npass <= P.grid) {
+            a.nbuf = 1; P.nbuf = 1; P.lds = (size_t)gemv_lds_layout(a.n, esz, norm, P.Rm, 64 >> P.cb_shift, two, 1).total;
+            fill_geom(a, esz, two ? EPI_SWIGLU : rows_per_item == 2 ? EPI_ROPE_KV : EPI_RESIDUAL, P.grid);
+        }
     };
     one_pass(ao, Po, false, false); one_pass(a13, P13, true, true); one_pass(a2, P2, false, false);
+    gemv_geom_src(ao.geom, (uint32_t)c->hs); gemv_geom_src(a2.geom, (uint32_t)P13.Rm);
     size_t own = Po.lds; if (P13.lds > own) own = P13.lds; if (P2.lds > own) own = P2.lds;
     if (with_qkv) { one_pass(aq, Pq, false, true, 2); if (Pq.lds > kLdsMax) return FLM_ERR_UNSUPPORTED; if (wants_layers(c) && Pq.lds > own) own = Pq.lds; }
     GemvArgs acls{}; GemvPlan Pc{}; bool tail_fits = false;
@@ -65,6 +69,7 @@
         p.nst2_ao = ok2 ? want2 : 0;
         p.r5 = ((G > 1 || p.ao_o) && p.ao_2 && with_qkv && !tpl) ? 3 : 0;
         if (!p.r5) { p.ao_o = 0; p.ao_2 = 0; p.nst2_ao = 0; }
+        if (p.r5 && (ao.geom.src_rows != (uint32_t)c->hs || a2.geom.src_rows != (uint32_t)P13.Rm)) return fail(c, FLM_ERR_STATE, "plan_layer: arrival-order hand-off without its producers' geometry");
         p.nw_o = kWavesPerBlock;
         if (p.ao_o && G == 1) { const int need = (ns_o + 1) / 2, want = c->back_nwo > 0 ? c->back_nwo : (need < 4 ? 4 : need); p.nw_o = (want >= need && want <= kWavesPerBlock - 2) ? want : kWavesPerBlock; }
     }
diff --git a/fast-llama_amd/csrc/flm_token.hip b/fast-llama_amd/csrc/flm_token.hip
--- a/fast-llama_amd/csrc/flm_token.hip
+++ b/fast-llama_amd/csrc/flm_token.hip
@@ -2,27 +2,6 @@
 
 namespace fh {
 
-GemvPlan gemv_plan(int n, int esz, int rows, bool two, bool pairs, bool norm, int wgs) {
-    GemvPlan P{};
-    const int nchunks = n * esz / 16;
-    int cbs = 0; while (cbs < 6 && (nchunks % (2 << cbs)) == 0) ++cbs;
-    const int RB = 64 >> cbs;
-    const int mult = (pairs && RB < 2) ? 2 : RB;
-    const int lds_budget = 150 * 1024;
-    int rmax = 64;
-    while (rmax > mult && gemv_lds_layout(n, esz, norm, rmax, RB, two).total > lds_budget) rmax -= mult;
-    rmax = rmax / mult * mult; if (rmax < mult) rmax = mult;
-    if (rows < 1) rows = 1;
-    int ppw = (rows + wgs * rmax - 1) / (wgs * rmax);
-    if (ppw < 1) ppw = 1;
-    int Rm = (rows + wgs * ppw - 1) / (wgs * ppw);
-    Rm = (Rm + mult - 1) / mult * mult; if (Rm > rmax) Rm = rmax; if (Rm < mult) Rm = mult;
-    const int npass = (rows + Rm - 1) / Rm;
-    P.Rm = Rm; P.cb_shift = cbs; P.grid = npass < wgs ? npass : wgs; if (P.grid < 1) P.grid = 1;
-    P.nbuf = 2;
-    P.lds = (size_t)gemv_lds_layout(n, esz, norm, Rm, RB, two, P.nbuf).total;
-    return P;
-}
 
 GemvArgs args_qkv(flm_ctx* c, int l) {
     const auto& d = c->d; LayerW& w = c->layers[l];
```

Result: no change. 560.4 tokens/s (median of 6 runs) (+1.0%).
